# ffreyer/MonteCarlo.jl

Measured on AMD Instinct MI355X. Metric: DQMC sweeps/sec, 16x16 Hubbard beta=8 dtau=0.1; achieved % fp64 MFMA roofline, higher is better.
Workload: dtype f64

## Files before the change

### include/dqmc_hip.h

```cpp
#ifndef DQMC_HIP_H
#define DQMC_HIP_H
#include <stddef.h>
#include <stdint.h>

#ifdef __cplusplus
extern "C" {
#endif

typedef struct dqmc_handle dqmc_handle;

typedef enum {
    DQMC_OK = 0,
    DQMC_ERR_INVALID = -1,
    DQMC_ERR_HIP = -2,
    DQMC_ERR_NO_DEVICE = -3,
    DQMC_ERR_STATE = -4,
    DQMC_ERR_RNG = -5
} dqmc_status;

enum { DQMC_ATTRACTIVE = 0, DQMC_REPULSIVE = 1 };

typedef struct {
    int32_t n_sites;
    int32_t model_kind;
    int32_t slices;
    int32_t safe_mult;
    int32_t n_walkers;
    int32_t device_id;
    int32_t check_propagation_error;
    int32_t check_sign_problem;
    double delta_tau;
    double U;
    const double *eT;
    const double *eTinv;
    const double *eT2;
    const double *eTinv2;
} dqmc_params;

typedef struct {
    double max, min, sum;
    int64_t count;
} dqmc_magstats;

typedef struct {
    int64_t prop_local, acc_local;
    dqmc_magstats imaginary_probability;
    dqmc_magstats negative_probability;
    dqmc_magstats propagation_error;
} dqmc_stats;

int dqmc_create(const dqmc_params *p, dqmc_handle **out);
int dqmc_destroy(dqmc_handle *h);
const char *dqmc_last_error(const dqmc_handle *h);
int dqmc_device_count(void);

int dqmc_set_conf(dqmc_handle *h, int32_t walker, const int8_t *conf);
int dqmc_get_conf(dqmc_handle *h, int32_t walker, int8_t *conf);
int dqmc_get_conf_bits(dqmc_handle *h, int32_t walker, uint64_t *chunks);
int dqmc_set_conf_bits(dqmc_handle *h, int32_t walker, const uint64_t *chunks);
int dqmc_set_uniforms(dqmc_handle *h, int32_t walker, const double *u, size_t n);
int dqmc_seed(dqmc_handle *h, int32_t walker, uint64_t seed);
int dqmc_uniforms_used(dqmc_handle *h, int32_t walker, uint64_t *used);
int dqmc_get_state(dqmc_handle *h, int32_t *current_slice, int32_t *direction);

int dqmc_prepare(dqmc_handle *h);
int dqmc_build_stack(dqmc_handle *h);
int dqmc_propagate(dqmc_handle *h);
int dqmc_sweep_spatial(dqmc_handle *h);
int dqmc_update(dqmc_handle *h);
int dqmc_sweep(dqmc_handle *h, int32_t n_sweeps);
int dqmc_update_until_measure(dqmc_handle *h, int32_t *n_updates);
int dqmc_synchronize(dqmc_handle *h);

int dqmc_get_greens_eff(dqmc_handle *h, int32_t walker, double *out);
int dqmc_set_greens_eff(dqmc_handle *h, int32_t walker, const double *in);
int dqmc_get_greens(dqmc_handle *h, int32_t walker, double *out);
int dqmc_calculate_greens_at(dqmc_handle *h, int32_t walker, int32_t slice, double *out);
int dqmc_replay_greens(dqmc_handle *h, int32_t slice);
int dqmc_wrap_greens(dqmc_handle *h, int32_t slice, int32_t direction);

int dqmc_get_stats(dqmc_handle *h, int32_t walker, dqmc_stats *out);

int dqmc_accumulate_greens(dqmc_handle *h);
int dqmc_accumulator_size(dqmc_handle *h, size_t *n_doubles);
int dqmc_reset_accumulators(dqmc_handle *h);
int dqmc_get_accumulators(dqmc_handle *h, double *host_out);
int dqmc_export_accumulators(dqmc_handle *h, void *device_out);

int dqmc_set_pair_directions(dqmc_handle *h, const int32_t *dir_of, int32_t n_dirs);
int dqmc_accumulate_correlations(dqmc_handle *h);
int dqmc_correlations_size(dqmc_handle *h, size_t *n_doubles);
int dqmc_get_correlations(dqmc_handle *h, double *host_out);
int dqmc_export_correlations(dqmc_handle *h, void *device_out);

int dqmc_set_local_targets(dqmc_handle *h, const int32_t *trg_of, int32_t K);
int dqmc_accumulate_pairing(dqmc_handle *h);
int dqmc_pairing_size(dqmc_handle *h, size_t *n_doubles);
int dqmc_get_pairing(dqmc_handle *h, double *host_out);
int dqmc_export_pairing(dqmc_handle *h, void *device_out);

int dqmc_ut_build_stack(dqmc_handle *h);
int dqmc_ut_get_stack(dqmc_handle *h, int32_t w, int32_t which, int32_t idx, double *U, double *D, double *T);
int dqmc_ut_greens(dqmc_handle *h, int32_t slice1, int32_t slice2, int32_t effective);
int dqmc_ut_get(dqmc_handle *h, int32_t w, int32_t which, double *host_out);
int dqmc_ut_export(dqmc_handle *h, int32_t which, void *device_out );
int dqmc_greens_iterator_begin(dqmc_handle *h, int32_t l, int32_t recalculate);
int dqmc_greens_iterator_next(dqmc_handle *h, int32_t *k);
int dqmc_combined_iterator_begin(dqmc_handle *h, int32_t recalculate);
int dqmc_combined_iterator_next(dqmc_handle *h, int32_t *l);

int dqmc_accumulate_susceptibilities(dqmc_handle *h, int32_t recalculate);
int dqmc_susceptibilities_size(dqmc_handle *h, size_t *n_doubles);
int dqmc_get_susceptibilities(dqmc_handle *h, double *host_out);
int dqmc_export_susceptibilities(dqmc_handle *h, void *device_out);

int dqmc_set_current_targets(dqmc_handle *h, const int32_t *trg_of, int32_t K, const double *T);
int dqmc_current_targets_fast_path(dqmc_handle *h, int32_t *fast);

enum { DQMC_BIN_GREENS = 0, DQMC_BIN_CORRELATIONS = 1, DQMC_BIN_PAIRING = 2, DQMC_BIN_SUSCEPTIBILITIES = 3,
       DQMC_BIN_USER = 4 };
int dqmc_binner_enable(dqmc_handle *h, int32_t which, int64_t capacity);
int dqmc_binner_size(dqmc_handle *h, int32_t which, size_t *n_elements, int32_t *n_levels, int64_t *n_pushed);
int dqmc_binner_reliable_level(dqmc_handle *h, int32_t which, int32_t *level);
int dqmc_binner_get_level(dqmc_handle *h, int32_t which, int32_t walker, int32_t level,
                          double *x_sum, double *x2_sum, int64_t *count);
int dqmc_binner_finish(dqmc_handle *h, int32_t which, int32_t level,
                       double *mean, double *std_error, double *std_error_walkers, double *tau);
int dqmc_binner_export_moments(dqmc_handle *h, int32_t which, int32_t level, void *device_out);
int dqmc_binner_user_create(dqmc_handle *h, int64_t n_elements, int64_t capacity);
int dqmc_binner_user_push(dqmc_handle *h, const double *device_samples);

typedef struct dqmc_comm dqmc_comm;
int dqmc_comm_unique_id(void *id128);
int dqmc_comm_init(const void *id128, int32_t nranks, int32_t rank, int32_t device_id, dqmc_comm **out);
int dqmc_comm_destroy(dqmc_comm *c);
int dqmc_reduce(dqmc_handle *h, dqmc_comm *comm);
int dqmc_reduce_size(dqmc_handle *h, size_t *n_doubles );
int dqmc_reduce_export(dqmc_handle *h, double *host_out);
int dqmc_reduce_import(dqmc_handle *h, const double *host_in);
enum { DQMC_RED_GREENS = 0, DQMC_RED_CORRELATIONS = 1, DQMC_RED_PAIRING = 2, DQMC_RED_SUSCEPTIBILITIES = 3 };
int dqmc_get_reduced(dqmc_handle *h, int32_t which, double *host_out);
int dqmc_get_reduced_stats(dqmc_handle *h, dqmc_stats *out);

int dqmc_vmul(int32_t device_id, int32_t n, int32_t batch, int32_t transa, int32_t transb,
              const double *A, const double *B, double *C);
int dqmc_udt_pivot(int32_t device_id, int32_t n, int32_t batch, double *U, double *D, double *T,
                   int64_t *pivot, int32_t apply_pivot);
int dqmc_rdivp(int32_t device_id, int32_t n, int32_t batch, double *A, const double *T,
               const int64_t *pivot);
int dqmc_calculate_greens(int32_t device_id, int32_t n, int32_t batch, const double *Ul,
                          const double *Dl, const double *Tl, const double *Ur, const double *Dr,
                          const double *Tr, double *G);

int dqmc_set_checkerboard(dqmc_handle *h, int32_t kmax, int32_t n_mats, const double *vals, const int32_t *cols,
                          const double *mu, const double *mu_inv, const int32_t *seqs, const int32_t *lens);

int dqmc_qr_fallbacks(dqmc_handle *h, int64_t *count);
int dqmc_kron_hopping(dqmc_handle *h, int32_t *on);
int dqmc_set_triangular_factors(dqmc_handle *h, const double *f);
int dqmc_udt_one_launch_sites(dqmc_handle *h, int32_t *mask);
int dqmc_device_errors(dqmc_handle *h, int32_t *word);
const char *dqmc_build_commit(void);
const char *dqmc_build_source_hash(void);

typedef struct dqmc_mc_handle dqmc_mc_handle;

typedef struct {
    int32_t n_sites;
    int32_t z;
    int32_t n_walkers;
    int32_t device_id;
    int32_t n_bonds;
    int32_t series_capacity;
    const int64_t *neighs;
    const int64_t *bonds;
} dqmc_mc_params;

typedef struct {
    int64_t energy;
    int64_t magnetization;
    double sum_E, sum_E2, sum_absM, sum_M2;
    int64_t n_meas;
    int64_t prop_local, acc_local;
    uint64_t uniforms_used;
    int64_t n_series;
} dqmc_mc_stats;

int dqmc_mc_create(const dqmc_mc_params *p, dqmc_mc_handle **out);
int dqmc_mc_destroy(dqmc_mc_handle *h);
const char *dqmc_mc_last_error(const dqmc_mc_handle *h);
int dqmc_mc_set_beta(dqmc_mc_handle *h, int32_t walker, double beta);
int dqmc_mc_seed(dqmc_mc_handle *h, int32_t walker, uint64_t seed);
int dqmc_mc_rand_conf(dqmc_mc_handle *h, int32_t walker);
int dqmc_mc_set_conf(dqmc_mc_handle *h, int32_t walker, const int8_t *conf);
int dqmc_mc_get_conf(dqmc_mc_handle *h, int32_t walker, int8_t *conf);
int dqmc_mc_get_conf_bits(dqmc_mc_handle *h, int32_t walker, uint64_t *chunks);
int dqmc_mc_sweep(dqmc_mc_handle *h, int32_t n_sweeps, int64_t first_sweep_index, int64_t thermalization,
                  int32_t measure_rate);
int dqmc_mc_get_stats(dqmc_mc_handle *h, int32_t walker, dqmc_mc_stats *out);
int dqmc_mc_get_series(dqmc_mc_handle *h, int32_t walker, int32_t *energy, int32_t *abs_magnetization,
                       int64_t *n_recorded);
int dqmc_mc_reset_accumulators(dqmc_mc_handle *h);
int dqmc_mc_set_global_rate(dqmc_mc_handle *h, int32_t rate);
int dqmc_mc_global_move(dqmc_mc_handle *h, int32_t walker);
typedef struct {
    int64_t prop_global, acc_global, sum_cluster_size;
    uint64_t moves_drawn;
} dqmc_mc_global_stats;
int dqmc_mc_get_global_stats(dqmc_mc_handle *h, int32_t walker, dqmc_mc_global_stats *out);
int dqmc_mc_synchronize(dqmc_mc_handle *h);

int dqmc_mc_binner_enable(dqmc_mc_handle *h, int64_t capacity);
int dqmc_mc_binner_size(dqmc_mc_handle *h, int32_t *n_levels, int64_t *n_pushed);
int dqmc_mc_binner_reliable_level(dqmc_mc_handle *h, int32_t *level);
int dqmc_mc_binner_get_level(dqmc_mc_handle *h, int32_t walker, int32_t level,
                             double x_sum[4], double x2_sum[4], double xy_sum[2], int64_t *count);
typedef struct {
    double mean[4];
    double varN[4];
    double varN0[4];
    double tau[4];
    double covN[2];
    int64_t count;
    int32_t level;
} dqmc_mc_binned;
int dqmc_mc_binner_finish(dqmc_mc_handle *h, int32_t walker, int32_t level, dqmc_mc_binned *out);

enum { DQMC_K_GEMM = 0, DQMC_K_QR = 1, DQMC_K_TRSM = 2, DQMC_K_SWEEP = 3, DQMC_K_MISC = 4, DQMC_K_FLUSH = 5,
       DQMC_K_COUNT = 6 };
int dqmc_timing_enable(dqmc_handle *h, int32_t on);
int dqmc_timing_get(dqmc_handle *h, double *ms , int64_t *launches );
int dqmc_mfma_f64_peak(int32_t device_id, int32_t iters, double *tflops);

#ifdef __cplusplus
}
#endif
#endif
```

### montecarlo.jl_amd/_lib.py

```python
import ctypes as C
import os

_HERE = os.path.dirname(os.path.abspath(__file__))
LIB_PATH = os.environ.get("DQMC_HIP_LIB") or os.path.join(_HERE, "libdqmc_hip.so")
HEADER_PATH = os.path.join(os.path.dirname(_HERE), "include", "dqmc_hip.h")

OK, ERR_INVALID, ERR_HIP, ERR_NO_DEVICE, ERR_STATE, ERR_RNG = 0, -1, -2, -3, -4, -5
ATTRACTIVE, REPULSIVE = 0, 1
BIN_SECTIONS = ("greens", "correlations", "pairing", "susceptibilities", "user")
K_FAMILIES = ("gemm", "qr", "trsm", "sweep", "misc", "flush")


class DQMCError(RuntimeError):
    def __init__(self, code, msg):
        super().__init__("libdqmc_hip error %d: %s" % (code, msg))
        self.code = code


class Params(C.Structure):
    _fields_ = [
        ("n_sites", C.c_int32), ("model_kind", C.c_int32), ("slices", C.c_int32), ("safe_mult", C.c_int32),
        ("n_walkers", C.c_int32), ("device_id", C.c_int32), ("check_propagation_error", C.c_int32),
        ("check_sign_problem", C.c_int32), ("delta_tau", C.c_double), ("U", C.c_double),
        ("eT", C.POINTER(C.c_double)), ("eTinv", C.POINTER(C.c_double)), ("eT2", C.POINTER(C.c_double)),
        ("eTinv2", C.POINTER(C.c_double)),
    ]


class MagStats(C.Structure):
    _fields_ = [("max", C.c_double), ("min", C.c_double), ("sum", C.c_double), ("count", C.c_int64)]


class Stats(C.Structure):
    _fields_ = [("prop_local", C.c_int64), ("acc_local", C.c_int64), ("imaginary_probability", MagStats),
                ("negative_probability", MagStats), ("propagation_error", MagStats)]


class McParams(C.Structure):
    _fields_ = [("n_sites", C.c_int32), ("z", C.c_int32), ("n_walkers", C.c_int32), ("device_id", C.c_int32),
                ("n_bonds", C.c_int32), ("series_capacity", C.c_int32), ("neighs", C.POINTER(C.c_int64)),
                ("bonds", C.POINTER(C.c_int64))]


class McStats(C.Structure):
    _fields_ = [("energy", C.c_int64), ("magnetization", C.c_int64), ("sum_E", C.c_double), ("sum_E2", C.c_double),
                ("sum_absM", C.c_double), ("sum_M2", C.c_double), ("n_meas", C.c_int64), ("prop_local", C.c_int64),
                ("acc_local", C.c_int64), ("uniforms_used", C.c_uint64), ("n_series", C.c_int64)]


class McGlobalStats(C.Structure):
    _fields_ = [("prop_global", C.c_int64), ("acc_global", C.c_int64), ("sum_cluster_size", C.c_int64),
                ("moves_drawn", C.c_uint64)]


class McBinned(C.Structure):
    _fields_ = [("mean", C.c_double * 4), ("varN", C.c_double * 4), ("varN0", C.c_double * 4), ("tau", C.c_double * 4),
                ("covN", C.c_double * 2), ("count", C.c_int64), ("level", C.c_int32)]


_dp = C.POINTER(C.c_double)
_i64p = C.POINTER(C.c_int64)
_H = C.c_void_p

SIGNATURES = {
    "dqmc_create": (C.c_int, [C.POINTER(Params), C.POINTER(_H)]),
    "dqmc_destroy": (C.c_int, [_H]),
    "dqmc_last_error": (C.c_char_p, [_H]),
    "dqmc_device_count": (C.c_int, []),
    "dqmc_set_conf": (C.c_int, [_H, C.c_int32, C.c_void_p]),
    "dqmc_get_conf": (C.c_int, [_H, C.c_int32, C.c_void_p]),
    "dqmc_get_conf_bits": (C.c_int, [_H, C.c_int32, C.POINTER(C.c_uint64)]),
    "dqmc_set_conf_bits": (C.c_int, [_H, C.c_int32, C.POINTER(C.c_uint64)]),
    "dqmc_set_uniforms": (C.c_int, [_H, C.c_int32, _dp, C.c_size_t]),
    "dqmc_seed": (C.c_int, [_H, C.c_int32, C.c_uint64]),
    "dqmc_uniforms_used": (C.c_int, [_H, C.c_int32, C.POINTER(C.c_uint64)]),
    "dqmc_get_state": (C.c_int, [_H, C.POINTER(C.c_int32), C.POINTER(C.c_int32)]),
    "dqmc_prepare": (C.c_int, [_H]),
    "dqmc_build_stack": (C.c_int, [_H]),
    "dqmc_propagate": (C.c_int, [_H]),
    "dqmc_sweep_spatial": (C.c_int, [_H]),
    "dqmc_update": (C.c_int, [_H]),
    "dqmc_sweep": (C.c_int, [_H, C.c_int32]),
    "dqmc_update_until_measure": (C.c_int, [_H, C.POINTER(C.c_int32)]),
    "dqmc_synchronize": (C.c_int, [_H]),
    "dqmc_get_greens_eff": (C.c_int, [_H, C.c_int32, _dp]),
    "dqmc_set_greens_eff": (C.c_int, [_H, C.c_int32, _dp]),
    "dqmc_get_greens": (C.c_int, [_H, C.c_int32, _dp]),
    "dqmc_calculate_greens_at": (C.c_int, [_H, C.c_int32, C.c_int32, _dp]),
    "dqmc_replay_greens": (C.c_int, [_H, C.c_int32]),
    "dqmc_wrap_greens": (C.c_int, [_H, C.c_int32, C.c_int32]),
    "dqmc_get_stats": (C.c_int, [_H, C.c_int32, C.POINTER(Stats)]),
    "dqmc_accumulate_greens": (C.c_int, [_H]),
    "dqmc_accumulator_size": (C.c_int, [_H, C.POINTER(C.c_size_t)]),
    "dqmc_reset_accumulators": (C.c_int, [_H]),
    "dqmc_get_accumulators": (C.c_int, [_H, _dp]),
    "dqmc_export_accumulators": (C.c_int, [_H, C.c_void_p]),
    "dqmc_set_pair_directions": (C.c_int, [_H, C.POINTER(C.c_int32), C.c_int32]),
    "dqmc_accumulate_correlations": (C.c_int, [_H]),
    "dqmc_correlations_size": (C.c_int, [_H, C.POINTER(C.c_size_t)]),
    "dqmc_get_correlations": (C.c_int, [_H, _dp]),
    "dqmc_export_correlations": (C.c_int, [_H, C.c_void_p]),
    "dqmc_set_local_targets": (C.c_int, [_H, C.POINTER(C.c_int32), C.c_int32]),
    "dqmc_accumulate_pairing": (C.c_int, [_H]),
    "dqmc_pairing_size": (C.c_int, [_H, C.POINTER(C.c_size_t)]),
    "dqmc_get_pairing": (C.c_int, [_H, _dp]),
    "dqmc_export_pairing": (C.c_int, [_H, C.c_void_p]),
    "dqmc_ut_build_stack": (C.c_int, [_H]),
    "dqmc_ut_get_stack": (C.c_int, [_H, C.c_int32, C.c_int32, C.c_int32, _dp, _dp, _dp]),
    "dqmc_ut_greens": (C.c_int, [_H, C.c_int32, C.c_int32, C.c_int32]),
    "dqmc_ut_get": (C.c_int, [_H, C.c_int32, C.c_int32, _dp]),
    "dqmc_ut_export": (C.c_int, [_H, C.c_int32, C.c_void_p]),
    "dqmc_greens_iterator_begin": (C.c_int, [_H, C.c_int32, C.c_int32]),
    "dqmc_greens_iterator_next": (C.c_int, [_H, C.POINTER(C.c_int32)]),
    "dqmc_combined_iterator_begin": (C.c_int, [_H, C.c_int32]),
    "dqmc_combined_iterator_next": (C.c_int, [_H, C.POINTER(C.c_int32)]),
    "dqmc_accumulate_susceptibilities": (C.c_int, [_H, C.c_int32]),
    "dqmc_set_current_targets": (C.c_int, [_H, C.POINTER(C.c_int32), C.c_int32, C.POINTER(C.c_double)]),
    "dqmc_current_targets_fast_path": (C.c_int, [_H, C.POINTER(C.c_int32)]),
    "dqmc_susceptibilities_size": (C.c_int, [_H, C.POINTER(C.c_size_t)]),
    "dqmc_get_susceptibilities": (C.c_int, [_H, _dp]),
    "dqmc_export_susceptibilities": (C.c_int, [_H, C.c_void_p]),
    "dqmc_binner_enable": (C.c_int, [_H, C.c_int32, C.c_int64]),
    "dqmc_binner_size": (C.c_int, [_H, C.c_int32, C.POINTER(C.c_size_t), C.POINTER(C.c_int32), _i64p]),
    "dqmc_binner_reliable_level": (C.c_int, [_H, C.c_int32, C.POINTER(C.c_int32)]),
    "dqmc_binner_get_level": (C.c_int, [_H, C.c_int32, C.c_int32, C.c_int32, _dp, _dp, _i64p]),
    "dqmc_binner_finish": (C.c_int, [_H, C.c_int32, C.c_int32, _dp, _dp, _dp, _dp]),
    "dqmc_binner_export_moments": (C.c_int, [_H, C.c_int32, C.c_int32, C.c_void_p]),
    "dqmc_binner_user_create": (C.c_int, [_H, C.c_int64, C.c_int64]),
    "dqmc_binner_user_push": (C.c_int, [_H, C.c_void_p]),
    "dqmc_comm_unique_id": (C.c_int, [C.c_void_p]),
    "dqmc_comm_init": (C.c_int, [C.c_void_p, C.c_int32, C.c_int32, C.c_int32, C.POINTER(_H)]),
    "dqmc_comm_destroy": (C.c_int, [_H]),
    "dqmc_reduce": (C.c_int, [_H, _H]),
    "dqmc_reduce_size": (C.c_int, [_H, C.POINTER(C.c_size_t)]),
    "dqmc_reduce_export": (C.c_int, [_H, _dp]),
    "dqmc_reduce_import": (C.c_int, [_H, _dp]),
    "dqmc_get_reduced": (C.c_int, [_H, C.c_int32, _dp]),
    "dqmc_get_reduced_stats": (C.c_int, [_H, C.POINTER(Stats)]),
    "dqmc_vmul": (C.c_int, [C.c_int32, C.c_int32, C.c_int32, C.c_int32, C.c_int32, _dp, _dp, _dp]),
    "dqmc_udt_pivot": (C.c_int, [C.c_int32, C.c_int32, C.c_int32, _dp, _dp, _dp, _i64p, C.c_int32]),
    "dqmc_rdivp": (C.c_int, [C.c_int32, C.c_int32, C.c_int32, _dp, _dp, _i64p]),
    "dqmc_calculate_greens": (C.c_int, [C.c_int32, C.c_int32, C.c_int32, _dp, _dp, _dp, _dp, _dp, _dp, _dp]),
    "dqmc_set_checkerboard": (C.c_int, [_H, C.c_int32, C.c_int32, _dp, C.POINTER(C.c_int32), _dp, _dp,
                              C.POINTER(C.c_int32), C.POINTER(C.c_int32)]),
    "dqmc_qr_fallbacks": (C.c_int, [_H, C.POINTER(C.c_int64)]),
    "dqmc_kron_hopping": (C.c_int, [_H, C.POINTER(C.c_int32)]),
    "dqmc_set_triangular_factors": (C.c_int, [_H, _dp]),
    "dqmc_device_errors": (C.c_int, [_H, C.POINTER(C.c_int32)]),
    "dqmc_udt_one_launch_sites": (C.c_int, [_H, C.POINTER(C.c_int32)]),
    "dqmc_build_commit": (C.c_char_p, []),
    "dqmc_build_source_hash": (C.c_char_p, []),
    "dqmc_mc_create": (C.c_int, [C.POINTER(McParams), C.POINTER(_H)]),
    "dqmc_mc_destroy": (C.c_int, [_H]),
    "dqmc_mc_last_error": (C.c_char_p, [_H]),
    "dqmc_mc_set_beta": (C.c_int, [_H, C.c_int32, C.c_double]),
    "dqmc_mc_seed": (C.c_int, [_H, C.c_int32, C.c_uint64]),
    "dqmc_mc_rand_conf": (C.c_int, [_H, C.c_int32]),
    "dqmc_mc_set_conf": (C.c_int, [_H, C.c_int32, C.c_void_p]),
    "dqmc_mc_get_conf": (C.c_int, [_H, C.c_int32, C.c_void_p]),
    "dqmc_mc_get_conf_bits": (C.c_int, [_H, C.c_int32, C.POINTER(C.c_uint64)]),
    "dqmc_mc_sweep": (C.c_int, [_H, C.c_int32, C.c_int64, C.c_int64, C.c_int32]),
    "dqmc_mc_get_stats": (C.c_int, [_H, C.c_int32, C.POINTER(McStats)]),
    "dqmc_mc_get_series": (C.c_int, [_H, C.c_int32, C.POINTER(C.c_int32), C.POINTER(C.c_int32),
                           C.POINTER(C.c_int64)]),
    "dqmc_mc_reset_accumulators": (C.c_int, [_H]),
    "dqmc_mc_set_global_rate": (C.c_int, [_H, C.c_int32]),
    "dqmc_mc_global_move": (C.c_int, [_H, C.c_int32]),
    "dqmc_mc_get_global_stats": (C.c_int, [_H, C.c_int32, C.POINTER(McGlobalStats)]),
    "dqmc_mc_synchronize": (C.c_int, [_H]),
    "dqmc_mc_binner_enable": (C.c_int, [_H, C.c_int64]),
    "dqmc_mc_binner_size": (C.c_int, [_H, C.POINTER(C.c_int32), _i64p]),
    "dqmc_mc_binner_reliable_level": (C.c_int, [_H, C.POINTER(C.c_int32)]),
    "dqmc_mc_binner_get_level": (C.c_int, [_H, C.c_int32, C.c_int32, _dp, _dp, _dp, _i64p]),
    "dqmc_mc_binner_finish": (C.c_int, [_H, C.c_int32, C.c_int32, C.POINTER(McBinned)]),
    "dqmc_timing_enable": (C.c_int, [_H, C.c_int32]),
    "dqmc_timing_get": (C.c_int, [_H, _dp, _i64p]),
    "dqmc_mfma_f64_peak": (C.c_int, [C.c_int32, C.c_int32, _dp]),
}

_lib = None


def lib():
    global _lib
    if _lib is None:
        if not os.path.exists(LIB_PATH):
            raise ImportError(
                "libdqmc_hip.so not found at %s — build it with __graft_entry__.build() "
                "(hipcc --offload-arch=gfx950); there is no CPU fallback." % LIB_PATH)
        L = C.CDLL(LIB_PATH)
        for name, (res, args) in SIGNATURES.items():
            f = getattr(L, name)
            f.restype = res
            f.argtypes = args
        _lib = L
    return _lib


def check(rc, handle=None):
    if rc != 0:
        msg = lib().dqmc_last_error(handle)
        raise DQMCError(rc, msg.decode() if msg else "")


def dptr(a):
    return a.ctypes.data_as(_dp)


def i64ptr(a):
    return a.ctypes.data_as(_i64p)
```

### montecarlo.jl_amd/csrc/engine.cpp

```cpp
#include <hip/hip_runtime.h>

#include <algorithm>
#include <cmath>
#include <cstdio>
#include <cstdlib>
#include <cstring>
#include <string>
#include <vector>

#include "../../include/dqmc_hip.h"
#include "kernels.h"
#include <rccl/rccl.h>

using namespace dqmc;

struct dqmc_comm {
    ncclComm_t comm = nullptr;
    int nranks = 1, rank = 0, device = 0;
};

static thread_local std::string g_create_error;

struct UTStack;

struct dqmc_handle {
    dqmc_params p{};
    int n = 0, nb = 1, N = 0, M = 0, s = 0, K = 0, W = 0, units = 0;
    long nn = 0;
    double lambda = 0, epl = 0, eml = 0;
    SweepConsts sc{};
    hipStream_t stream = nullptr;
    KernelSwitches sw;
    double *eT = nullptr, *eTinv = nullptr, *eT2 = nullptr, *eTinv2 = nullptr;
    double *eT2T = nullptr;
    bool slab = false;
    bool kron = false, tri = false;
    double *kron_f = nullptr;
    int kron_fa = 0, kron_fb = 0;
    int8_t *conf = nullptr;
    double *u_stack = nullptr, *t_stack = nullptr, *d_stack = nullptr;
    std::vector<double *> su, sd, st;
    double *Ul = nullptr, *Ur = nullptr, *Tl = nullptr, *Tr = nullptr, *greens = nullptr, *greens_temp = nullptr;
    double *tmp1 = nullptr, *tmp2 = nullptr, *bufA = nullptr, *bufB = nullptr;
    struct QrSet {
        double *V = nullptr, *W = nullptr, *S = nullptr, *tau = nullptr, *winv = nullptr, *ts = nullptr;
        int *pivot = nullptr;
    } qs[1];
    double *&qrV = qs[0].V, *&qrW = qs[0].W, *&qrS = qs[0].S, *&trsm_w = qs[0].winv, *&trsm_s = qs[0].ts, *&tau = qs[0].tau;
    int *&pivot = qs[0].pivot;
    double *Dl = nullptr, *Dr = nullptr;
    hipStream_t cur = nullptr;
    double *greens_alt = nullptr, *lu_img = nullptr;
    bool sweep_fused = true;
    struct PendingFlush {
        const double *G = nullptr;
        const double *img = nullptr;
        int site0 = 0;
    } pf;
    unsigned *wrap_cnt = nullptr;
    unsigned wrap_launches = 0;
    int wrap_blocks[2] = {0, 0};
    WalkerRng *rng = nullptr;
    DevStats *stats = nullptr;
    unsigned long long *pc_scratch = nullptr;
    std::vector<double *> uniforms;
    double *acc = nullptr;
    size_t acc_n = 0;
    int n_dirs = 0;
    int *dir_ptr = nullptr, *pair_src = nullptr, *pair_trg = nullptr;
    double *corr_per_walker = nullptr, *corr_acc = nullptr;
    int K_loc = 0;
    int *trg_of = nullptr;
    size_t pc_n = 0;
    double *pc_per_walker = nullptr, *pc_acc = nullptr;
    int K_cc = 0;
    std::vector<int> cc_trg_h;
    std::vector<double> cc_T;
    CCPlan cc;
    size_t corr_n = 0;
    int current_slice = 0, direction = 0;
    bool prepared = false;
    long long conf_version = 0;
    UTStack *ut = nullptr;
    std::string err;
    bool timing = false;
    struct Ev { hipEvent_t a, b; int fam; };
    std::vector<Ev> pending;
    std::vector<hipEvent_t> pool;
    double fam_ms[DQMC_K_COUNT] = {0};
    long long fam_n[DQMC_K_COUNT] = {0};
    std::vector<void *> allocs;
    QrCoopWorkspace qr_ws;
    int qrb_sites = 0;
    struct {
        bool on = false;
        int kmax = 0, n_mats = 0;
        double *vals = nullptr, *mu = nullptr, *mu_inv = nullptr;
        int *cols = nullptr;
        int seq[7][32];
        int len[7] = {0, 0, 0, 0, 0, 0, 0};
    } cb;
    double *red_buf = nullptr;
    size_t red_cap = 0;
    dqmc_stats red_stats{};
    bool red_valid = false;
    size_t red_sizes[4] = {0, 0, 0, 0};
    struct Binner {
        bool on = false;
        int E = 0, L = 0;
        int64_t cap = 0, T = 0;
        double *xs = nullptr, *x2 = nullptr, *c = nullptr, *out = nullptr;
    } bin[5];
};

#define HIPCHK(expr)                                                                                   \
    do {                                                                                               \
        hipError_t e_ = (expr);                                                                        \
        if (e_ != hipSuccess) {                                                                        \
            h->err = std::string(#expr) + ": " + hipGetErrorString(e_);                                \
            return DQMC_ERR_HIP;                                                                       \
        }                                                                                              \
    } while (0)
#define CHK(expr)                \
    do {                         \
        int rc_ = (expr);        \
        if (rc_ != 0) return rc_; \
    } while (0)

static int fail(dqmc_handle *h, int code, const std::string &msg)
{
    if (h) h->err = msg;
    else g_create_error = msg;
    return code;
}

template <typename T>
static int dalloc(dqmc_handle *h, T **p, size_t count, bool zero = true)
{
    void *q = nullptr;
    HIPCHK(hipMalloc(&q, (count ? count : 1) * sizeof(T)));
    h->allocs.push_back(q);
    if (zero) HIPCHK(hipMemsetAsync(q, 0, (count ? count : 1) * sizeof(T), h->stream));
    *p = (T *)q;
    return 0;
}

static int timing_drain(dqmc_handle *h)
{
    if (h->pending.empty()) return 0;
    HIPCHK(hipStreamSynchronize(h->stream));
    for (auto &e : h->pending) {
        float ms = 0.f;
        HIPCHK(hipEventElapsedTime(&ms, e.a, e.b));
        h->fam_ms[e.fam] += ms;
        h->fam_n[e.fam] += 1;
        h->pool.push_back(e.a);
        h->pool.push_back(e.b);
    }
    h->pending.clear();
    return 0;
}
struct Timed {
    dqmc_handle *h;
    int fam;
    hipEvent_t a = nullptr, b = nullptr;
    Timed(dqmc_handle *h_, int fam_) : h(h_), fam(fam_)
    {
        if (!h->timing) return;
        auto get = [&]() {
            hipEvent_t e;
            if (!h->pool.empty()) { e = h->pool.back(); h->pool.pop_back(); }
            else (void)hipEventCreate(&e);
            return e;
        };
        a = get();
        b = get();
        (void)hipEventRecord(a, h->cur);
    }
    ~Timed()
    {
        if (!h->timing) return;
        (void)hipEventRecord(b, h->cur);
        h->pending.push_back({a, b, fam});
        if (h->pending.size() >= 2048) (void)timing_drain(h);
    }
};

static GemmArgs gemm_base(dqmc_handle *h, MatRef A, int tA, MatRef B, int tB, double *C)
{
    GemmArgs g{};
    g.M = g.N = g.K = h->n;
    g.n_units = h->units;
    g.nb = h->nb;
    g.A = A;
    g.B = B;
    g.C = C;
    g.strideC = h->nn;
    g.ldc = h->n;
    g.transA = tA;
    g.transB = tB;
    g.kscale = g.colscale = g.rowscale = g.adddiag = vs_none();
    g.row_first = 0;
    g.alpha = 1.0;
    g.ident = 0.0;
    g.beta = 0;
    g.tri = 0;
// ... 616 lines not shown
        g.rowscale = vs_conf(h, l, -1);
        CHK(run_gemm(h, g));
        g = gemm_base(h, U_(h, h->tmp1), 0, C_(h, h->eT2), 0, gf);
        g.colscale = vs_conf(h, l, +1);
        CHK(run_gemm(h, g));
    } else {
        const int l = curr_slice;
        GemmArgs g = gemm_base(h, C_(h, h->eT2), 0, U_(h, gf), 0, h->tmp1);
        g.kscale = vs_conf(h, l, +1);
        CHK(run_gemm(h, g));
        g = gemm_base(h, U_(h, h->tmp1), 0, C_(h, h->eTinv2), 0, gf);
        g.kscale = vs_conf(h, l, -1);
        CHK(run_gemm(h, g));
    }
    return 0;
}

static int reset_slot(dqmc_handle *h, int slot)
{
    const int sp = h->K + 1;
    CHK(set_identity(h, uslot(h, sp)));
    CHK(set_ones(h, dslot(h, sp)));
    CHK(set_identity(h, tslot(h, sp)));
    slot_swap_spare(h, slot);
    return 0;
}
static int prop_check(dqmc_handle *h)
{
    Timed t(h, DQMC_K_MISC);
    HIPCHK(launch_prop_check(h->n, h->nb, h->W, h->greens_temp, h->greens, h->nn, h->stats, h->pc_scratch, h->cur));
    return 0;
}

static int init_stack(dqmc_handle *h)
{
    CHK(set_identity(h, h->Ul)); CHK(set_identity(h, h->Ur));
    CHK(set_identity(h, h->Tl)); CHK(set_identity(h, h->Tr));
    CHK(set_ones(h, h->Dl)); CHK(set_ones(h, h->Dr));
    h->current_slice = 0;
    h->direction = 0;
    return 0;
}
static int build_stack(dqmc_handle *h)
{
    CHK(reset_slot(h, 0));
    for (int i = 1; i <= h->K; ++i) CHK(add_slice_sequence_left(h, i));
    h->current_slice = h->M + 1;
    h->direction = -1;
    return 0;
}

static int propagate(dqmc_handle *h)
{
    const int M = h->M, s = h->s;
    if (h->direction == 1) {
        if (h->current_slice % s == 0) {
            h->current_slice += 1;
            if (h->current_slice == 1) {
                const Udt R = slot_ref(h, 0);
                CHK(reset_slot(h, 0));
                discard_pending_flush(h);
                CHK(calculate_greens_src(h, h->greens, slot_ref(h, 0), R));
            } else if (1 < h->current_slice && h->current_slice <= M) {
                const int idx = (h->current_slice - 1) / s;
                const Udt R = slot_ref(h, idx);
                const bool wt = h->p.check_propagation_error != 0, wt_slab = wt && oop_wrap(h);
                CHK(add_slice_sequence_left(h, idx, wt_slab));
                const Udt L = slot_ref(h, idx);
                if (wt && !wt_slab) {
                    CHK(materialize_pending_flush(h));
                    CHK(copy_mat(h, h->greens_temp, h->greens));
                    CHK(wrap_greens(h, &h->greens_temp, h->current_slice - 1, 1));
                }
                if (wt_slab) {
                    std::swap(h->greens, h->greens_alt);
                    CHK(calculate_greens_src(h, h->greens, L, R));
                    CHK(prop_check(h));
                    return 0;
                }
                discard_pending_flush(h);
                CHK(calculate_greens_src(h, h->greens, L, R));
                if (h->p.check_propagation_error) CHK(prop_check(h));
            } else {
                CHK(add_slice_sequence_left(h, h->K));
                h->direction = -1;
                h->current_slice = M + 1;
                CHK(propagate(h));
            }
        } else {
            CHK(wrap_greens(h, &h->greens, h->current_slice, 1));
            h->current_slice += 1;
        }
    } else {
        if ((h->current_slice - 1) % s == 0) {
            h->current_slice -= 1;
            if (h->current_slice == M) {
                const Udt L = slot_ref(h, h->K);
                CHK(reset_slot(h, h->K));
                discard_pending_flush(h);
                CHK(calculate_greens_src(h, h->greens, L, slot_ref(h, h->K)));
                CHK(wrap_greens(h, &h->greens, h->current_slice + 1, -1));
            } else if (0 < h->current_slice && h->current_slice < M) {
                const int idx = h->current_slice / s + 1;
                const Udt L = slot_ref(h, idx - 1);
                CHK(add_slice_sequence_right(h, idx));
                const Udt R = slot_ref(h, idx - 1);
                if (h->p.check_propagation_error) {
                    CHK(materialize_pending_flush(h));
                    std::swap(h->greens_temp, h->greens);
                }
                discard_pending_flush(h);
                CHK(calculate_greens_src(h, h->greens, L, R));
                if (h->p.check_propagation_error) CHK(prop_check(h));
                CHK(wrap_greens(h, &h->greens, h->current_slice + 1, -1));
            } else {
                CHK(add_slice_sequence_right(h, 1));
                h->direction = 1;
                h->current_slice = 0;
                CHK(propagate(h));
            }
        } else {
            CHK(wrap_greens(h, &h->greens, h->current_slice, -1));
            h->current_slice -= 1;
        }
    }
    return 0;
}

static int sweep_spatial_launches(dqmc_handle *h);
static int sweep_spatial(dqmc_handle *h)
{
    const int l = h->current_slice;
    if (l < 1 || l > h->M) return fail(h, DQMC_ERR_STATE, "sweep_spatial: current_slice outside 1..slices");
    CHK(sweep_spatial_launches(h));
    return 0;
}
static int sweep_spatial_launches(dqmc_handle *h)
{
    const int l = h->current_slice;
    int8_t *cslice = h->conf + (long)(l - 1) * h->N;
    h->conf_version++;
    CHK(materialize_pending_flush(h));
    double *cur = h->greens, *alt = h->greens_alt;
    const size_t istr = (size_t)h->units * sweep_lu_image_doubles();

    const long cstr = (long)h->N * h->M;
    hipEvent_t a, b;
    if (h->sweep_fused && h->n % 64 == 0 && h->N >= 128) {
        const int nc = h->N / 64;
        timing_events(h, &a, &b);
        HIPCHK(launch_sweep_lu(h->n, h->nb, h->W, cur, h->nn, cslice, cstr, 0, 64, h->lu_img, h->sc, h->rng, h->stats,
                               h->p.check_sign_problem, h->qr_ws.errflag, h->cur, a, b));
        CHK(timing_push(h, a, b, DQMC_K_SWEEP));
        for (int c = 1; c < nc; ++c) {
            timing_events(h, &a, &b);
            HIPCHK(launch_sweep_fused(h->n, h->nb, h->W, cur, alt, h->nn, cslice, cstr, 64 * c, 64 * (c - 1),
                                      h->lu_img + (size_t)(c & 1) * istr, h->lu_img + (size_t)((c - 1) & 1) * istr, h->sc,
                                      h->rng, h->stats, h->p.check_sign_problem, h->qr_ws.errflag, h->cur, a, b));
            CHK(timing_push(h, a, b, DQMC_K_SWEEP));
            std::swap(cur, alt);
        }
        const double *img_last = h->lu_img + (size_t)((nc - 1) & 1) * istr;
        if (fold_wrap_flush(h)) {
            h->pf = dqmc_handle::PendingFlush{cur, img_last, 64 * (nc - 1)};
        } else {
            timing_events(h, &a, &b);
            HIPCHK(launch_sweep_flush_lu(h->n, h->units, cur, alt, h->nn, 64 * (nc - 1), 64, img_last, h->sw, h->cur, a, b));
            CHK(timing_push(h, a, b, DQMC_K_FLUSH));
            std::swap(cur, alt);
        }
        if (cur != h->greens) std::swap(h->greens, h->greens_alt);
        return 0;
    }
    for (int site0 = 0; site0 < h->N; site0 += 64) {
        const int ns = std::min(64, h->N - site0);
        timing_events(h, &a, &b);
        HIPCHK(launch_sweep_lu(h->n, h->nb, h->W, cur, h->nn, cslice, cstr, site0, ns, h->lu_img, h->sc,
                               h->rng, h->stats, h->p.check_sign_problem, h->qr_ws.errflag, h->cur, a, b));
        CHK(timing_push(h, a, b, DQMC_K_SWEEP));
        timing_events(h, &a, &b);
        HIPCHK(launch_sweep_flush_lu(h->n, h->units, cur, alt, h->nn, site0, ns, h->lu_img, h->sw, h->cur, a, b));
        CHK(timing_push(h, a, b, DQMC_K_FLUSH));
        std::swap(cur, alt);
    }
    if (cur != h->greens) std::swap(h->greens, h->greens_alt);
    return 0;
}

extern "C" {

const char *dqmc_last_error(const dqmc_handle *h) { return h ? h->err.c_str() : g_create_error.c_str(); }

int dqmc_device_count(void)
{
    int c = 0;
    if (hipGetDeviceCount(&c) != hipSuccess) return 0;
    return c;
}

int dqmc_create(const dqmc_params *p, dqmc_handle **out)
{
    if (!p || !out) return fail(nullptr, DQMC_ERR_INVALID, "dqmc_create: null argument");
    *out = nullptr;
    if (p->n_sites < 1 || p->slices < 1 || p->safe_mult < 1 || p->n_walkers < 1)
        return fail(nullptr, DQMC_ERR_INVALID, "dqmc_create: n_sites, slices, safe_mult, n_walkers must be >= 1");
    if (p->slices % p->safe_mult != 0)
        return fail(nullptr, DQMC_ERR_INVALID, "dqmc_create: slices must be divisible by safe_mult");
    if (p->model_kind != DQMC_ATTRACTIVE && p->model_kind != DQMC_REPULSIVE)
        return fail(nullptr, DQMC_ERR_INVALID, "dqmc_create: unknown model_kind");
    if (!p->eT || !p->eTinv || !p->eT2 || !p->eTinv2)
        return fail(nullptr, DQMC_ERR_INVALID, "dqmc_create: hopping exponentials missing");
    if (!(p->U >= 0.0)) return fail(nullptr, DQMC_ERR_INVALID, "dqmc_create: U must be positive");
    const int nb = p->model_kind == DQMC_REPULSIVE ? 2 : 1;
    if (p->n_sites > 1024) return fail(nullptr, DQMC_ERR_INVALID, "dqmc_create: n_sites exceeds 1024 (unsupported)");
    int ndev = 0;
    if (hipGetDeviceCount(&ndev) != hipSuccess || ndev == 0)
        return fail(nullptr, DQMC_ERR_NO_DEVICE, "dqmc_create: no HIP device visible");
    if (p->device_id < 0 || p->device_id >= ndev)
        return fail(nullptr, DQMC_ERR_INVALID, "dqmc_create: device_id out of range");

    dqmc_handle *h = new dqmc_handle();
    read_kernel_switches(h);
    h->p = *p;
    h->p.eT = h->p.eTinv = h->p.eT2 = h->p.eTinv2 = nullptr;
    h->N = h->n = p->n_sites;
    h->nb = nb;
    h->M = p->slices;
    h->s = p->safe_mult;
    h->K = h->M / h->s;
    h->W = p->n_walkers;
    h->units = h->W * h->nb;
    h->nn = (long)h->n * h->n;
    h->sweep_fused = false;
    if (!h->sw.sweep_split && h->n % 64 == 0) {
        hipDeviceProp_t prop;
        if (hipGetDeviceProperties(&prop, p->device_id) == hipSuccess) {
            const int ncp = (h->n % 256 == 0) ? 2 : 1, nt = (h->n % 128 == 0) ? 8 : 4;
            const int flush_blocks = ((h->units + 7) / 8) * 8 * (h->n / 64) * (h->n / (16 * nt * ncp));
            h->sweep_fused = h->W + flush_blocks <= prop.multiProcessorCount;
        }
    }
    h->lambda = std::acosh(std::exp(0.5 * p->U * p->delta_tau));
    h->epl = std::exp(h->lambda);
    h->eml = std::exp(-h->lambda);
    for (int ci = 0; ci < 2; ++ci) {
        const double c = ci ? 1.0 : -1.0;
        const double dE = -2.0 * h->lambda * c;
        h->sc.gamma[ci] = std::exp(dE) - 1.0;
        h->sc.ebos[ci] = std::exp(-dE);
        h->sc.dup[ci] = std::exp(dE) - 1.0;
        h->sc.ddn[ci] = std::exp(-dE) - 1.0;
    }
    auto bail = [&](int rc) {
        g_create_error = h->err;
        dqmc_destroy(h);
        return rc;
    };
#define CCHK(expr)                     \
    do {                               \
        int rc__ = (expr);             \
        if (rc__ != 0) return bail(rc__); \
    } while (0)
#define CHIP(expr)                                                        \
    do {                                                                  \
        hipError_t e__ = (expr);                                          \
        if (e__ != hipSuccess) {                                          \
            h->err = std::string(#expr) + ": " + hipGetErrorString(e__);  \
            return bail(DQMC_ERR_HIP);                                    \
        }                                                                 \
    } while (0)
    CHIP(hipSetDevice(p->device_id));
    CHIP(hipStreamCreate(&h->stream));
    h->cur = h->stream;
    const size_t cn = (size_t)nb * h->nn, un = (size_t)h->units * h->nn, uv = (size_t)h->units * h->n;
    CCHK(dalloc(h, &h->eT, cn)); CCHK(dalloc(h, &h->eTinv, cn));
    CCHK(dalloc(h, &h->eT2, cn)); CCHK(dalloc(h, &h->eTinv2, cn));
    CHIP(hipMemcpy(h->eT, p->eT, cn * sizeof(double), hipMemcpyHostToDevice));
    CHIP(hipMemcpy(h->eTinv, p->eTinv, cn * sizeof(double), hipMemcpyHostToDevice));
    CHIP(hipMemcpy(h->eT2, p->eT2, cn * sizeof(double), hipMemcpyHostToDevice));
    CHIP(hipMemcpy(h->eTinv2, p->eTinv2, cn * sizeof(double), hipMemcpyHostToDevice));
    if (h->n == 256 && !h->sw.no_slab) {
        std::vector<double> tr(cn);
        for (int b = 0; b < nb; ++b)
            for (int j = 0; j < h->n; ++j)
                for (int i = 0; i < h->n; ++i) tr[(size_t)b * h->nn + j + (size_t)h->n * i] = p->eT2[(size_t)b * h->nn + i + (size_t)h->n * j];
        CCHK(dalloc(h, &h->eT2T, cn));
        CHIP(hipMemcpy(h->eT2T, tr.data(), cn * sizeof(double), hipMemcpyHostToDevice));
        h->slab = true;
    }
    if (h->slab && !h->sw.no_kron) {
        std::vector<double> f((size_t)4 * 2 * nb * 256);
        bool ok = true;
        for (int m = 0; m < 2 && ok; ++m)
            for (int b = 0; b < nb && ok; ++b) {
                double *fx = f.data() + ((size_t)m * 2 * nb + b) * 256, *fy = fx + (size_t)nb * 256;
                double *tx = f.data() + ((size_t)(m + 2) * 2 * nb + b) * 256, *ty = tx + (size_t)nb * 256;
                ok = kron_factor((m ? p->eTinv2 : p->eT2) + (size_t)b * h->nn, fx, fy);
                for (int j = 0; j < 16; ++j)
                    for (int i = 0; i < 16; ++i) {
                        tx[i + 16 * j] = fx[j + 16 * i];
                        ty[i + 16 * j] = fy[j + 16 * i];
                    }
            }
        if (ok) {
            CCHK(dalloc(h, &h->kron_f, f.size()));
            CHIP(hipMemcpy(h->kron_f, f.data(), f.size() * sizeof(double), hipMemcpyHostToDevice));
            h->kron = true;
            h->kron_fa = h->kron_fb = 256;
        }
    }
    if (h->n == 512 && !h->sw.no_kron) {
        const size_t per = (size_t)nb * (4096 + 256);
        std::vector<double> f(4 * per);
        double fx[64], fy[64], fz[64];
        bool ok = true;
        for (int m = 0; m < 2 && ok; ++m)
// ... 648 lines not shown
int dqmc_comm_destroy(dqmc_comm *c)
{
    if (!c) return DQMC_OK;
    if (c->comm) (void)ncclCommDestroy(c->comm);
    delete c;
    return DQMC_OK;
}
int dqmc_reduce_size(dqmc_handle *h, size_t *n_doubles)
{
    if (!h || !n_doubles) return DQMC_ERR_INVALID;
    *n_doubles = red_nsum(h) + 4;
    return DQMC_OK;
}
int dqmc_reduce(dqmc_handle *h, dqmc_comm *comm)
{
    ENTER(h);
    CHK(red_pack(h));
    if (comm && comm->comm) {
        if (comm->device != h->p.device_id) return fail(h, DQMC_ERR_INVALID, "dqmc_reduce: communicator bound to another device");
        const size_t nsum = red_nsum(h);
        ncclResult_t r = ncclGroupStart();
        if (r == ncclSuccess) r = ncclAllReduce(h->red_buf, h->red_buf, nsum, ncclDouble, ncclSum, comm->comm, h->stream);
        if (r == ncclSuccess) r = ncclAllReduce(h->red_buf + nsum, h->red_buf + nsum, 2, ncclDouble, ncclMax, comm->comm, h->stream);
        if (r == ncclSuccess) r = ncclAllReduce(h->red_buf + nsum + 2, h->red_buf + nsum + 2, 2, ncclDouble, ncclMin, comm->comm, h->stream);
        const ncclResult_t r2 = ncclGroupEnd();
        if (r != ncclSuccess || r2 != ncclSuccess)
            return fail(h, DQMC_ERR_HIP, std::string("ncclAllReduce: ") + ncclGetErrorString(r != ncclSuccess ? r : r2));
    }
    CHK(red_unpack(h));
    return DQMC_OK;
}
int dqmc_reduce_export(dqmc_handle *h, double *host_out)
{
    ENTER(h);
    CHK(red_pack(h));
    HIPCHK(hipMemcpy(host_out, h->red_buf, (red_nsum(h) + 4) * sizeof(double), hipMemcpyDeviceToHost));
    return DQMC_OK;
}
int dqmc_reduce_import(dqmc_handle *h, const double *host_in)
{
    ENTER(h);
    if (h->red_cap < red_nsum(h) + 4) return fail(h, DQMC_ERR_STATE, "call dqmc_reduce_export first");
    HIPCHK(hipStreamSynchronize(h->stream));
    HIPCHK(hipMemcpy(h->red_buf, host_in, (red_nsum(h) + 4) * sizeof(double), hipMemcpyHostToDevice));
    CHK(red_unpack(h));
    return DQMC_OK;
}
int dqmc_get_reduced(dqmc_handle *h, int32_t which, double *host_out)
{
    ENTER(h);
    if (!host_out || which < 0 || which > 3) return fail(h, DQMC_ERR_INVALID, "dqmc_get_reduced: bad arguments");
    if (!h->red_valid) return fail(h, DQMC_ERR_STATE, "call dqmc_reduce first");
    const size_t sizes[4] = {h->acc_n, h->corr_n, h->pc_n, h->ut ? h->ut->sus_n : 0};
    size_t off = 0;
    for (int i = 0; i < which; ++i) off += sizes[i];
    if (sizes[which] == 0) return fail(h, DQMC_ERR_STATE, "dqmc_get_reduced: this accumulator is not configured");
    for (int i = 0; i < 4; ++i)
        if (sizes[i] != h->red_sizes[i])
            return fail(h, DQMC_ERR_STATE, "accumulators were reconfigured after the last reduction: call dqmc_reduce again");
    if (h->red_cap < red_nsum(h) + 4) return fail(h, DQMC_ERR_STATE, "call dqmc_reduce first");
    HIPCHK(hipStreamSynchronize(h->stream));
    HIPCHK(hipMemcpy(host_out, h->red_buf + off, sizes[which] * sizeof(double), hipMemcpyDeviceToHost));
    return DQMC_OK;
}
int dqmc_get_reduced_stats(dqmc_handle *h, dqmc_stats *out)
{
    if (!h || !out) return DQMC_ERR_INVALID;
    if (!h->red_valid) return fail(h, DQMC_ERR_STATE, "call dqmc_reduce first");
    *out = h->red_stats;
    return DQMC_OK;
}


int dqmc_set_triangular_factors(dqmc_handle *h, const double *f)
{
    ENTER(h);
    if (!f) return fail(h, DQMC_ERR_INVALID, "dqmc_set_triangular_factors: null factors");
    if (h->n != 256) return fail(h, DQMC_ERR_INVALID, "dqmc_set_triangular_factors: n_sites must be 256");
    if (h->prepared) return fail(h, DQMC_ERR_STATE, "dqmc_set_triangular_factors: call before dqmc_prepare");
    if (!h->slab || h->cb.on || h->sw.no_kron || h->kron) return DQMC_OK;
    const int nb = h->nb;
    std::vector<double> E((size_t)2 * nb * h->nn);
    HIPCHK(hipStreamSynchronize(h->stream));
    HIPCHK(hipMemcpy(E.data(), h->eT2, sizeof(double) * nb * h->nn, hipMemcpyDeviceToHost));
    HIPCHK(hipMemcpy(E.data() + (size_t)nb * h->nn, h->eTinv2, sizeof(double) * nb * h->nn, hipMemcpyDeviceToHost));
    std::vector<double> img((size_t)4 * 3 * nb * 256);
    for (int b = 0; b < nb; ++b)
        for (int m = 0; m < 2; ++m) {
            const double *fb = f + (size_t)b * 1536 + (size_t)m * 768;
            if (!tri_factor_ok(E.data() + ((size_t)m * nb + b) * h->nn, fb, fb + 256, fb + 512))
                return fail(h, DQMC_ERR_INVALID, "dqmc_set_triangular_factors: the factors do not reproduce eT2 / eTinv2 of block " +
                                                     std::to_string(b) + " within 256 ulp");
            for (int k = 0; k < 3; ++k) {
                double *o = img.data() + (((size_t)m * 3 + k) * nb + b) * 256, *ot = o + (size_t)2 * 3 * nb * 256;
                for (int j = 0; j < 16; ++j)
                    for (int i = 0; i < 16; ++i) {
                        o[i + 16 * j] = fb[256 * k + i + 16 * j];
                        ot[i + 16 * j] = fb[256 * k + j + 16 * i];
                    }
            }
        }
    CHK(dalloc(h, &h->kron_f, img.size()));
    HIPCHK(hipMemcpy(h->kron_f, img.data(), img.size() * sizeof(double), hipMemcpyHostToDevice));
    h->kron_fa = 256;
    h->kron_fb = 512;
    h->tri = h->kron = true;
    return DQMC_OK;
}

int dqmc_set_checkerboard(dqmc_handle *h, int32_t kmax, int32_t n_mats, const double *vals, const int32_t *cols,
                          const double *mu, const double *mu_inv, const int32_t *seqs ,
                          const int32_t *lens )
{
    ENTER(h);
    if (kmax < 1 || kmax > 64 || n_mats < 1 || !vals || !cols || !mu || !mu_inv || !seqs || !lens)
        return fail(h, DQMC_ERR_INVALID, "dqmc_set_checkerboard: bad arguments");
    const size_t cnt = (size_t)n_mats * h->n * kmax;
    for (size_t i = 0; i < cnt; ++i)
        if (cols[i] < 0 || cols[i] >= h->n) return fail(h, DQMC_ERR_INVALID, "dqmc_set_checkerboard: column index out of range");
    for (int q = 0; q < 7; ++q) {
        if (lens[q] < 0 || lens[q] > 32) return fail(h, DQMC_ERR_INVALID, "dqmc_set_checkerboard: sequence too long");
        for (int i = 0; i < lens[q]; ++i)
            if (seqs[q * 32 + i] < 0 || seqs[q * 32 + i] >= n_mats)
                return fail(h, DQMC_ERR_INVALID, "dqmc_set_checkerboard: factor index out of range");
    }
    HIPCHK(hipStreamSynchronize(h->stream));
    CHK(dalloc(h, &h->cb.vals, cnt));
    CHK(dalloc(h, &h->cb.cols, cnt));
    CHK(dalloc(h, &h->cb.mu, (size_t)h->nb * h->n));
    CHK(dalloc(h, &h->cb.mu_inv, (size_t)h->nb * h->n));
    HIPCHK(hipMemcpy(h->cb.vals, vals, cnt * sizeof(double), hipMemcpyHostToDevice));
    HIPCHK(hipMemcpy(h->cb.cols, cols, cnt * sizeof(int), hipMemcpyHostToDevice));
    HIPCHK(hipMemcpy(h->cb.mu, mu, (size_t)h->nb * h->n * sizeof(double), hipMemcpyHostToDevice));
    HIPCHK(hipMemcpy(h->cb.mu_inv, mu_inv, (size_t)h->nb * h->n * sizeof(double), hipMemcpyHostToDevice));
    h->cb.kmax = kmax; h->cb.n_mats = n_mats;
    for (int q = 0; q < 7; ++q) {
        h->cb.len[q] = lens[q];
        for (int i = 0; i < lens[q]; ++i) h->cb.seq[q][i] = seqs[q * 32 + i];
    }
    h->cb.on = true;
    return DQMC_OK;
}

int dqmc_device_errors(dqmc_handle *h, int32_t *word)
{
    ENTER(h);
    if (!word) return DQMC_ERR_INVALID;
    *word = 0;
    if (!h->qr_ws.errflag) return DQMC_OK;
    HIPCHK(hipStreamSynchronize(h->stream));
    HIPCHK(hipMemcpy(word, h->qr_ws.errflag, sizeof(int), hipMemcpyDeviceToHost));
    return DQMC_OK;
}
int dqmc_udt_one_launch_sites(dqmc_handle *h, int32_t *mask)
{
    if (!h || !mask) return DQMC_ERR_INVALID;
    *mask = h->qrb_sites;
    return DQMC_OK;
}

int dqmc_kron_hopping(dqmc_handle *h, int32_t *on)
{
    ENTER(h);
    if (!on) return DQMC_ERR_INVALID;
    *on = use_kron(h) ? 1 : 0;
    return DQMC_OK;
}

int dqmc_qr_fallbacks(dqmc_handle *h, int64_t *count)
{
    ENTER(h);
    if (!count) return DQMC_ERR_INVALID;
    *count = 0;
    if (!h->qr_ws.fb) return DQMC_OK;
    int fb[2] = {0, 0};
    HIPCHK(hipStreamSynchronize(h->stream));
    HIPCHK(hipMemcpy(fb, h->qr_ws.fb, sizeof(fb), hipMemcpyDeviceToHost));
    *count = fb[1];
    return DQMC_OK;
}

int dqmc_timing_enable(dqmc_handle *h, int32_t on)
{
    ENTER(h);
    CHK(timing_drain(h));
    h->timing = on != 0;
    for (int i = 0; i < DQMC_K_COUNT; ++i) { h->fam_ms[i] = 0; h->fam_n[i] = 0; }
    return DQMC_OK;
}
int dqmc_timing_get(dqmc_handle *h, double *ms, int64_t *launches)
{
    ENTER(h);
    CHK(timing_drain(h));
    for (int i = 0; i < DQMC_K_COUNT; ++i) {
        if (ms) ms[i] = h->fam_ms[i];
        if (launches) launches[i] = h->fam_n[i];
    }
    return DQMC_OK;
}

namespace {
struct Scratch {
    dqmc_handle h;
    int ok = 0;
};
static int scratch_init(dqmc_handle *h, int device_id, int n, int batch)
{
    int ndev = 0;
    if (hipGetDeviceCount(&ndev) != hipSuccess || ndev == 0) return fail(nullptr, DQMC_ERR_NO_DEVICE, "no HIP device visible");
    if (device_id < 0 || device_id >= ndev) return fail(nullptr, DQMC_ERR_INVALID, "device_id out of range");
    if (n < 1 || n > 1024 || batch < 1) return fail(nullptr, DQMC_ERR_INVALID, "n must be 1..1024 and batch >= 1");
    read_kernel_switches(h);
    h->p.device_id = device_id;
    h->n = h->N = n;
    h->nb = 1;
    h->W = h->units = batch;
    h->nn = (long)n * n;
    HIPCHK(hipSetDevice(device_id));
    HIPCHK(hipStreamCreate(&h->stream));
    h->cur = h->stream;
    return 0;
}
static void scratch_free(dqmc_handle *h)
{
    if (h->stream) (void)hipStreamSynchronize(h->stream);
    for (void *q : h->allocs) (void)hipFree(q);
    h->allocs.clear();
    if (h->stream) (void)hipStreamDestroy(h->stream);
    h->stream = nullptr;
}
}

#define SCHK(expr)                                   \
    do {                                             \
        int rc_ = (expr);                            \
        if (rc_ != 0) {                              \
            g_create_error = h->err.empty() ? g_create_error : h->err; \
            scratch_free(h);                         \
            return rc_;                              \
        }                                            \
    } while (0)
#define SHIP(expr)                                                       \
    do {                                                                 \
        hipError_t e_ = (expr);                                          \
        if (e_ != hipSuccess) {                                          \
            g_create_error = std::string(#expr) + ": " + hipGetErrorString(e_); \
            scratch_free(h);                                             \
            return DQMC_ERR_HIP;                                         \
        }                                                                \
    } while (0)

int dqmc_vmul(int32_t device_id, int32_t n, int32_t batch, int32_t ta, int32_t tb, const double *A, const double *B,
              double *C)
{
    dqmc_handle hh; dqmc_handle *h = &hh;
    SCHK(scratch_init(h, device_id, n, batch));
    const size_t un = (size_t)batch * h->nn;
    double *dA, *dB, *dC;
    SCHK(dalloc(h, &dA, un, false)); SCHK(dalloc(h, &dB, un, false)); SCHK(dalloc(h, &dC, un));
    SHIP(hipMemcpy(dA, A, un * sizeof(double), hipMemcpyHostToDevice));
    SHIP(hipMemcpy(dB, B, un * sizeof(double), hipMemcpyHostToDevice));
    SCHK(run_gemm(h, gemm_base(h, U_(h, dA), ta != 0, U_(h, dB), tb != 0, dC)));
    SHIP(hipStreamSynchronize(h->stream));
    SHIP(hipMemcpy(C, dC, un * sizeof(double), hipMemcpyDeviceToHost));
    scratch_free(h);
    return DQMC_OK;
}

static int scratch_udt_bufs(dqmc_handle *h)
{
    const size_t un = (size_t)h->units * h->nn, uv = (size_t)h->units * h->n;
    CHK(dalloc(h, &h->qrV, un)); CHK(dalloc(h, &h->qrW, un)); CHK(dalloc(h, &h->qrS, un));
    CHK(dalloc(h, &h->tau, uv)); CHK(dalloc(h, &h->pivot, uv));
    CHK(dalloc(h, &h->trsm_w, (size_t)h->units * ((h->n + 15) / 16) * 256));
    CHK(alloc_qr_workspace(h));
    return 0;
}

int dqmc_udt_pivot(int32_t device_id, int32_t n, int32_t batch, double *U, double *D, double *T, int64_t *pivot,
                   int32_t apply)
{
    dqmc_handle hh; dqmc_handle *h = &hh;
    SCHK(scratch_init(h, device_id, n, batch));
    const size_t un = (size_t)batch * h->nn, uv = (size_t)batch * n;
    double *dU, *dD, *dT, *dTo;
    SCHK(dalloc(h, &dU, un)); SCHK(dalloc(h, &dD, uv)); SCHK(dalloc(h, &dT, un, false)); SCHK(dalloc(h, &dTo, un));
    SCHK(scratch_udt_bufs(h));
    SHIP(hipMemcpy(dT, T, un * sizeof(double), hipMemcpyHostToDevice));
    SCHK(udt(h, dT, dU, dD, dTo, apply != 0));
    SHIP(hipStreamSynchronize(h->stream));
    SCHK(check_qr_workspace(h));
    SHIP(hipMemcpy(U, dU, un * sizeof(double), hipMemcpyDeviceToHost));
    SHIP(hipMemcpy(D, dD, uv * sizeof(double), hipMemcpyDeviceToHost));
    SHIP(hipMemcpy(T, (apply || udt_is_fused(h, 0)) ? dTo : dT, un * sizeof(double), hipMemcpyDeviceToHost));
    std::vector<int> piv(uv);
    SHIP(hipMemcpy(piv.data(), h->pivot, uv * sizeof(int), hipMemcpyDeviceToHost));
    for (size_t i = 0; i < uv; ++i) pivot[i] = (int64_t)piv[i] + 1;
    scratch_free(h);
    return DQMC_OK;
}

int dqmc_rdivp(int32_t device_id, int32_t n, int32_t batch, double *A, const double *T, const int64_t *pivot)
{
    dqmc_handle hh; dqmc_handle *h = &hh;
    SCHK(scratch_init(h, device_id, n, batch));
    const size_t un = (size_t)batch * h->nn, uv = (size_t)batch * n;
// ... 70 lines not shown
```

### montecarlo.jl_amd/csrc/kernels.h

```cpp
#pragma once
#include <hip/hip_runtime.h>
#include <stdint.h>

namespace dqmc {

struct VecSrc {
    int mode;
    const double *d;
    long stride;
    const int8_t *conf;
    long conf_stride;
    double cpos[2], cneg[2];
};
static inline VecSrc vs_none() { VecSrc v = {}; v.mode = 0; return v; }
static inline VecSrc vs_arr(const double *d, long stride) { VecSrc v = {}; v.mode = 1; v.d = d; v.stride = stride; return v; }
static inline VecSrc vs_inv(const double *d, long stride) { VecSrc v = {}; v.mode = 3; v.d = d; v.stride = stride; return v; }
static inline VecSrc vs_min1(const double *d, long stride) { VecSrc v = {}; v.mode = 4; v.d = d; v.stride = stride; return v; }
static inline VecSrc vs_maxinv(const double *d, long stride) { VecSrc v = {}; v.mode = 5; v.d = d; v.stride = stride; return v; }
#ifdef __HIPCC__
__device__ __forceinline__ double vs_get(const VecSrc &v, int unit, int nb, int i)
{
    if (v.mode == 1) return v.d[(long)unit * v.stride + i];
    if (v.mode == 3) return 1.0 / v.d[(long)unit * v.stride + i];
    if (v.mode == 2) {
// ... 44 lines not shown
    long conf_stride;
    double epl, eml;
};
hipError_t launch_slab_chain(const SlabArgs &a, hipStream_t s, hipEvent_t start = nullptr, hipEvent_t stop = nullptr);
struct KronStep {
    const double *ax, *ay;
    const int8_t *pre_conf; int pre_sign;
    const int8_t *post_conf; int post_sign;
};
struct KronArgs {
    int n_units, nb, nsteps;
    KronStep st[SLAB_MAX_STEPS];
    const double *X0; long x_su;
    double *out; long out_su;
    const double *col_d; long col_stride;
    int transpose_out;
    long conf_stride;
    double epl, eml;
    const double *pf_img; long pf_img_su;
    int pf_site0;
    double *wrap_out;
    unsigned *wrap_cnt; unsigned wrap_target;
    int *errflag;
};
hipError_t launch_kron_chain(const KronArgs &a, hipStream_t s, hipEvent_t start = nullptr, hipEvent_t stop = nullptr);
constexpr int KR_CNT_STRIDE = 32;
inline int kron_wrap_grid(int n_units) { return (n_units + 7) / 8 * 8 * 16; }
int kron_wrap_blocks_per_cu(bool pending);
hipError_t launch_kron_wrap(const KronArgs &a, hipStream_t s, hipEvent_t start = nullptr, hipEvent_t stop = nullptr);
hipError_t launch_kron3_chain(const KronArgs &a, hipStream_t s, hipEvent_t start = nullptr, hipEvent_t stop = nullptr);
hipError_t launch_tri_chain(const KronArgs &a, hipStream_t s, hipEvent_t start = nullptr, hipEvent_t stop = nullptr);

struct KernelSwitches {
    bool qr_noblocked = false;
    int qrb_sites = 7;
    bool qr_tail = true;
    bool qr_sc1 = false;
    bool qr_nocoop = false;
    int qr_force_timeout = 0;
    bool qr_nopanel = false;
    bool trsm_simple = false;
    bool sweep_split = false;
    bool flush_ncp2 = false;
    bool no_slab = false;
    bool no_kron = false;
    bool no_wrap_flush = false;
    bool wrap_two_launch = false;
};

constexpr int QR_COOP_SLOT = 528;
constexpr int QR_COOP_SLOTS_PER_UNIT = 16;
struct QrCoopWorkspace {
    double *mailbox = nullptr;
    int *errflag = nullptr;
    int *fb = nullptr;
    unsigned long long epoch = 0;
    int max_blocks = 0;
    bool tail = true;
    int force_sc1 = 0;
    int no_coop = 0;
    bool no_panel = false;
    int force_timeout = 0;
    double *mailbox2 = nullptr;
    int blk_max_blocks = 0;
};
hipError_t launch_udt_blocked(int n_units, const double *A, long strideA, double *U, long strideU, double *D, long strideD,
                              double *T, long strideT, int *pivot, QrCoopWorkspace *ws, int apply_pivot, hipStream_t s,
                              const double *B = nullptr, long strideB = 0);
size_t qrb_mailbox_bytes(int n_units);
int qrb_blocks_per_cu();
hipError_t launch_qr_pivot(int n, int n_units, double *A, long strideA, double *tau, int *pivot,
                           QrCoopWorkspace *ws, double *W, long strideW, const double **factored, hipStream_t s,
                           double *X = nullptr, long strideX = 0);
int qr_coop_blocks_per_cu();

hipError_t launch_udt_finish(int n, int n_units, double *A, long strideA, const double *F, long strideF,
                             const int *pivot, double *D, long strideD, double *V, long strideV, double *Tout,
                             long strideT, int apply_pivot, hipStream_t s);

hipError_t launch_trsm_right_upper(int n, int n_units, const double *A, long strideA, const double *T,
                                   long strideT, const int *pivot, const double *dmul, long strideV,
                                   double *Out, long strideOut, double *winv, const KernelSwitches &sw,
                                   hipStream_t s, double *scratch = nullptr);

struct SweepConsts {
    double gamma[2], ebos[2], dup[2], ddn[2];
};
struct WalkerRng {
    unsigned long long seed;
    unsigned long long draw;
    const double *uniforms;
    unsigned long long n_uniforms;
    int exhausted;
};
struct DevMagStats { double max, min, sum; long long count; };
struct DevStats {
    long long prop_local, acc_local;
    DevMagStats negative_probability, propagation_error;
};
#ifdef __HIPCC__
__device__ __forceinline__ double philox_uniform(unsigned long long seed, unsigned long long index)
{
    unsigned int c0 = (unsigned int)index, c1 = (unsigned int)(index >> 32), c2 = 0u, c3 = 0u;
    unsigned int k0 = (unsigned int)seed, k1 = (unsigned int)(seed >> 32);
#pragma unroll
    for (int r = 0; r < 10; ++r) {
        const unsigned long long p0 = (unsigned long long)0xD2511F53u * c0;
        const unsigned long long p1 = (unsigned long long)0xCD9E8D57u * c2;
        const unsigned int n0 = (unsigned int)(p1 >> 32) ^ c1 ^ k0;
        const unsigned int n1 = (unsigned int)p1;
        const unsigned int n2 = (unsigned int)(p0 >> 32) ^ c3 ^ k1;
        const unsigned int n3 = (unsigned int)p0;
        c0 = n0; c1 = n1; c2 = n2; c3 = n3;
        k0 += 0x9E3779B9u;
        k1 += 0xBB67AE85u;
    }
    const unsigned long long hi = c0 >> 5, lo = c1 >> 6;
    return (double)((hi << 26) | lo) * (1.0 / 9007199254740992.0);
}

__device__ __forceinline__ double philox4_uniform(unsigned long long seed, unsigned int c0, unsigned int c1,
                                                  unsigned int c2, unsigned int c3)
{
    unsigned int k0 = (unsigned int)seed, k1 = (unsigned int)(seed >> 32);
#pragma unroll
    for (int r = 0; r < 10; ++r) {
        const unsigned long long p0 = (unsigned long long)0xD2511F53u * c0;
        const unsigned long long p1 = (unsigned long long)0xCD9E8D57u * c2;
        const unsigned int n0 = (unsigned int)(p1 >> 32) ^ c1 ^ k0;
        const unsigned int n1 = (unsigned int)p1;
        const unsigned int n2 = (unsigned int)(p0 >> 32) ^ c3 ^ k1;
        const unsigned int n3 = (unsigned int)p0;
        c0 = n0; c1 = n1; c2 = n2; c3 = n3;
        k0 += 0x9E3779B9u;
        k1 += 0xBB67AE85u;
    }
    const unsigned long long hi = c0 >> 5, lo = c1 >> 6;
    return (double)((hi << 26) | lo) * (1.0 / 9007199254740992.0);
}

__device__ __forceinline__ void magstats_push(DevMagStats &s, double value)
{
    const double v = log10(fabs(value));
    s.max = fmax(s.max, v);
    s.min = fmin(s.min, v);
    s.sum += v;
    s.count += 1;
}
#endif
size_t sweep_lu_image_doubles();
constexpr int LU_TILE = 256;
constexpr int LU_OFF_U = 0, LU_OFF_L = 6 * LU_TILE, LU_OFF_PT = 12 * LU_TILE, LU_OFF_Q = 16 * LU_TILE;
constexpr int LU_IMG = 20 * LU_TILE;
constexpr int LU_STRIDE = LU_IMG + 64;
__host__ __device__ constexpr int lu_pair(int K, int J)
{
    return K == 0 ? J - 1 : (K == 1 ? J + 1 : 5);
}
hipError_t launch_sweep_lu(int n, int nb, int n_walkers, const double *G, long strideG, int8_t *conf_slice,
                           long conf_stride, int site0, int nsites, double *img, SweepConsts sc, WalkerRng *rng,
                           DevStats *stats, int check_sign, int *errflag, hipStream_t s,
                           hipEvent_t start = nullptr, hipEvent_t stop = nullptr);
hipError_t launch_sweep_fused(int n, int nb, int n_walkers, const double *Gin, double *Gout, long strideG,
                              int8_t *conf_slice, long conf_stride, int site0, int site0p, double *img,
                              const double *imgp, SweepConsts sc, WalkerRng *rng, DevStats *stats, int check_sign,
                              int *errflag, hipStream_t s, hipEvent_t start = nullptr, hipEvent_t stop = nullptr);

hipError_t launch_sweep_flush_lu(int n, int n_units, const double *Gin, double *Gout, long strideG, int site0,
                                 int nsites, const double *img, const KernelSwitches &sw, hipStream_t s,
                                 hipEvent_t start = nullptr, hipEvent_t stop = nullptr);

struct CbArgs {
    int n, nb, side, kmax, seq_len;
    int seq[32];
    const double *vals;
    const int *cols;
    const double *X;
    double *O;
    long strideX;
    const int8_t *conf;
    long conf_stride;
    double epl, eml;
    int pre_conf, post_conf;
    const double *pre_vec, *post_vec;
    const double *qscale;
    long qstride;
};
hipError_t launch_cb_apply(const CbArgs &a, int n_units, hipStream_t s, hipEvent_t start = nullptr,
                           hipEvent_t stop = nullptr);

hipError_t launch_set_identity(int n, int count, double *A, long stride, hipStream_t s);
hipError_t launch_fill(double *p, size_t n, double v, hipStream_t s);
hipError_t launch_set_diag(int n, int nb, int units, double *A, long stride, VecSrc d, hipStream_t s);
hipError_t launch_mat_add(double *A, const double *B, size_t count, hipStream_t s);
hipError_t launch_sub_identity(int n, int units, double *O, const double *A, long stride, hipStream_t s);
hipError_t launch_vec_map(int n, int nb, int units, double *dst, long stride, VecSrc src, hipStream_t s);
hipError_t launch_scale_mat(int n, int nb, int units, double *O, const double *A, long stride, VecSrc row, VecSrc col,
                            int row_first, hipStream_t s);
hipError_t launch_prop_check(int n, int nb, int n_walkers, const double *A, const double *B,
                             long stride_unit, DevStats *stats, unsigned long long *scratch, hipStream_t s);
hipError_t launch_accumulate(int n, int nb, int n_walkers, const double *G, long stride_unit,
                             double *acc, hipStream_t s);
hipError_t launch_mfma_peak(int iters, int blocks, double *sink, hipStream_t s);
hipError_t launch_correlations(int n, int nb, int model, int n_walkers, const double *G, long stride_unit,
                               const int *dir_ptr, const int *pair_src, const int *pair_trg, int n_dirs,
                               double *per_walker, double *acc, hipStream_t s);
hipError_t launch_pairing(int n, int nb, int n_walkers, const double *G, long stride_unit, const int *dir_ptr,
                          const int *pair_src, const int *pair_trg, int n_dirs, int K, const int *trg_of,
                          double *per_walker, double *acc, hipStream_t s);
hipError_t launch_sus_slice(int n, int nb, int model, int n_walkers, const double *G00, const double *G0l,
                            const double *Gl0, const double *Gll, long stride_unit, const int *dir_ptr,
                            const int *pair_src, const int *pair_trg, int n_dirs, int K, const int *trg_of,
                            double *per_walker, long per_stride, hipStream_t s);
hipError_t launch_sus_reduce(int n_walkers, long total, double factor, const double *per_walker, double *acc,
                             hipStream_t s);
constexpr int CC_KMAX = 8;
struct CCPlan {
    int K = 0;
    const int *trg = nullptr;
    const double *tst = nullptr, *tts = nullptr;
    double *bsum = nullptr;
    bool fast = false;
    int C = 0, umax = 0, nchunks = 0, chunks_per_wg = 0, n_wg = 0, threads = 0;
    size_t lds_bytes = 0;
    const int *dsel = nullptr, *rows = nullptr, *ucnt = nullptr, *slot = nullptr;
    double *partial = nullptr;
};
hipError_t launch_cc_b(int n, int nb, int n_walkers, int K, double afac, const double *G00, long stride_unit,
                       const int *trg, const double *tst, const double *tts, double *bsum, hipStream_t s);
hipError_t launch_cc_slice(const CCPlan &p, int n, int nb, int n_walkers, double afac, double xfac,
                           const double *G0l, const double *Gl0, const double *Gll, long stride_unit,
                           const int *dir_ptr, const int *pair_src, const int *pair_trg, int n_dirs,
                           double *per_walker, long per_stride, long offset, hipStream_t s);
enum { BIN_SRC_PLAIN = 0, BIN_SRC_GREENS = 1, BIN_SRC_CORR = 2 };
struct BinPush {
    int mode = BIN_SRC_PLAIN;
    const double *src = nullptr, *G = nullptr;
    long stride_unit = 0;
    int n = 0, nb = 1, model = 0, n_dirs = 0;
    double scale = 1.0;
};
hipError_t launch_binner_push(const BinPush &p, int W, int E, int L, int lmax, double *xs, double *x2, double *c,
                              hipStream_t s);
hipError_t launch_binner_finish(int W, int E, long T, int level, const double *xs, const double *x2, double *out,
                                hipStream_t s);
hipError_t launch_conf_pack(const int8_t *conf, size_t n_elem, unsigned long long *chunks, hipStream_t s);
hipError_t launch_conf_unpack(const unsigned long long *chunks, size_t n_elem, int8_t *conf, hipStream_t s);

}
```

### montecarlo.jl_amd/csrc/kron.hip

```cpp
#include "kernels.h"
#include <hip/hip_ext.h>

namespace dqmc {

typedef double d4k __attribute__((ext_vector_type(4)));
#define KR_MFMA(a, b, c) __builtin_amdgcn_mfma_f64_16x16x4f64((a), (b), (c), 0, 0, 0)

constexpr int KR_N = 256;
constexpr int KR_NC = 4;
constexpr int KR_COLS = 4 * KR_NC;
constexpr int KR_TLD = 17;
constexpr int KR_SLD = 18;
constexpr int KR_LDS_T = 4 * KR_NC * 16 * KR_TLD;
constexpr int KR_LDS_S = KR_N * KR_SLD;
constexpr int KR_LDS = KR_LDS_T > KR_LDS_S ? KR_LDS_T : KR_LDS_S;
constexpr int KR_PF_TS = 16 * 17;
constexpr int KR_PF_IMG = 0, KR_PF_X = 20 * KR_PF_TS, KR_PF_R0 = KR_PF_X + 64, KR_PF_RLD = 65;
constexpr int KR_PF_D = KR_LDS_T, KR_PF_DLD = 257;
constexpr int KR_LDS_PF = KR_PF_D + KR_COLS * KR_PF_DLD;
static_assert(KR_PF_R0 + KR_COLS * KR_PF_RLD <= KR_LDS_PF && KR_LDS <= KR_LDS_PF, "pending-chunk LDS layout");

#define KR_GLOBAL __attribute__((address_space(1)))
typedef const KR_GLOBAL double *kr_gcdp;
typedef double kr_d2 __attribute__((ext_vector_type(2)));
typedef const KR_GLOBAL kr_d2 *kr_gcd2p;
typedef unsigned kr_u4 __attribute__((ext_vector_type(4)));

__device__ __forceinline__ double kr_conf(int8_t c, int sign, bool bn, double epl, double eml)
{
    return (((c > 0) == (sign > 0)) != bn) ? epl : eml;
}

#ifdef KR_STAMPS
__device__ long long *kr_stamp_ptr = nullptr;
#define KR_STAMP(k)                                                                                   \
    do {                                                                                              \
        if (PF && threadIdx.x == 0 && kr_stamp_ptr)                                                   \
            kr_stamp_ptr[16 * blockIdx.x + (k)] = (long long)__builtin_amdgcn_s_memtime();            \
    } while (0)
#define KR_STAMP_RT(k)                                                                                \
    do {                                                                                              \
        if (PF && threadIdx.x == 0 && kr_stamp_ptr)                                                   \
            kr_stamp_ptr[16 * blockIdx.x + (k)] = (long long)__builtin_amdgcn_s_memrealtime();        \
    } while (0)
extern "C" int dqmc_debug_kr_stamps(void *devptr)
{
    return (int)hipMemcpyToSymbol(HIP_SYMBOL(kr_stamp_ptr), &devptr, sizeof(void *));
}
#else
#define KR_STAMP(k) do { } while (0)
#define KR_STAMP_RT(k) do { } while (0)
#endif
template <bool PF>
__device__ __forceinline__ void kr_apply_pending(const KronArgs &a, int unit, int c0, d4k (&v)[KR_NC], double *lds)
{
    const int tid = threadIdx.x, lane = tid & 63, w = tid >> 6, g = lane >> 4, ci = lane & 15;
    const int site0 = a.pf_site0;
    const kr_gcdp img = (kr_gcdp)(a.pf_img + (long)unit * a.pf_img_su);
    const kr_gcdp G = (kr_gcdp)(a.X0 + (long)unit * a.x_su);
    double *limg = lds + KR_PF_IMG, *lx = lds + KR_PF_X, *lr = lds + KR_PF_R0, *ld = lds + KR_PF_D;
    constexpr int NI = LU_IMG / 2 / 256;
    static_assert(NI * 512 == LU_IMG, "image staging");
    kr_d2 iv[NI];
#pragma unroll
    for (int i = 0; i < NI; ++i) iv[i] = reinterpret_cast<kr_gcd2p>(img)[tid + 256 * i];
    const double xin = img[LU_IMG + (tid & 63)];
#pragma unroll
    for (int i = 0; i < NI; ++i) {
        const int p = 2 * (tid + 256 * i), tl = p >> 8, r = (p >> 6) & 3, ln = p & 63;
        double *d = limg + tl * KR_PF_TS + (4 * r + (ln >> 4)) * 17 + (ln & 15);
        d[0] = iv[i].x;
        d[1] = iv[i].y;
    }
    if (tid < 64) lx[tid] = xin;
    {
        const int rr = site0 >> 6;
#pragma unroll
        for (int t = 0; t < KR_NC; ++t) {
            const double r0 = rr == 0 ? v[t][0] : (rr == 1 ? v[t][1] : (rr == 2 ? v[t][2] : v[t][3]));
            lr[(KR_NC * w + t) * KR_PF_RLD + ci + 16 * g] = r0;
        }
    }
    __syncthreads();
    KR_STAMP(2);
    auto A = [&](int tl, int q) { return limg[tl * KR_PF_TS + ci * 17 + 4 * q + g]; };
    auto xr = [&](int J, int r) { return lx[16 * J + 4 * r + g]; };
    constexpr int TU = LU_OFF_U / LU_TILE, TL = LU_OFF_L / LU_TILE, TP = LU_OFF_PT / LU_TILE, TQ = LU_OFF_Q / LU_TILE;
    const kr_gcdp gc = G + 64 * w + ci + (long)KR_N * (site0 + g);
    double ca[2][4][4];
    auto fetch = [&](int J, double (&c)[4][4]) {
#pragma unroll
        for (int q = 0; q < 4; ++q)
#pragma unroll
            for (int mm = 0; mm < 4; ++mm) c[mm][q] = gc[16 * mm + (long)KR_N * (16 * J + 4 * q)];
    };
    fetch(0, ca[0]);
#ifdef KR_PROBE_PRODUCTS
    d4k rh[4];
    {
        double *lw = lr + KR_COLS * KR_PF_RLD, *lh = lr;
        static_assert(KR_PF_R0 + 2 * KR_COLS * KR_PF_RLD <= KR_LDS_PF, "probe LDS");
        d4k pa[4];
#pragma unroll
        for (int J = 0; J < 4; ++J) {
            pa[J] = (d4k){0.0, 0.0, 0.0, 0.0};
            if (J <= w)
#pragma unroll
                for (int q = 0; q < 4; ++q) pa[J] = KR_MFMA(A(TL + J, q), lr[ci * KR_PF_RLD + 16 * J + 4 * q + g], pa[J]);
        }
#pragma unroll
        for (int r = 0; r < 4; ++r)
            lw[ci * KR_PF_RLD + 16 * w + 4 * r + g] = (pa[0][r] + pa[1][r] + pa[2][r] + pa[3][r]) * xr(w, r);
        __syncthreads();
#pragma unroll
        for (int J = 0; J < 4; ++J) {
            pa[J] = (d4k){0.0, 0.0, 0.0, 0.0};
            if (J >= w)
#pragma unroll
                for (int q = 0; q < 4; ++q) pa[J] = KR_MFMA(A(TU + J, q), lw[ci * KR_PF_RLD + 16 * J + 4 * q + g], pa[J]);
        }
#pragma unroll
        for (int r = 0; r < 4; ++r) lh[ci * KR_PF_RLD + 16 * w + 4 * r + g] = pa[0][r] + pa[1][r] + pa[2][r] + pa[3][r];
        __syncthreads();
#pragma unroll
        for (int J = 0; J < 4; ++J)
#pragma unroll
            for (int q = 0; q < 4; ++q) rh[J][q] = lh[ci * KR_PF_RLD + 16 * J + 4 * q + g];
    }
#else
    d4k xv[4], rh[4];
#pragma unroll
    for (int J = 0; J < 4; ++J) {
        d4k acc;
#pragma unroll
        for (int r = 0; r < 4; ++r) acc[r] = lr[ci * KR_PF_RLD + 16 * J + 4 * r + g];
#pragma unroll
        for (int K = 0; K < J; ++K)
#pragma unroll
            for (int q = 0; q < 4; ++q) acc = KR_MFMA(A(TL + lu_pair(K, J), q), xv[K][q], acc);
        d4k z = (d4k){0.0, 0.0, 0.0, 0.0};
#pragma unroll
        for (int q = 0; q < 4; ++q) z = KR_MFMA(A(TQ + J, q), acc[q], z);
#pragma unroll
        for (int r = 0; r < 4; ++r) xv[J][r] = z[r] * xr(J, r);
    }
#pragma unroll
    for (int J = 3; J >= 0; --J) {
        d4k acc = (d4k){0.0, 0.0, 0.0, 0.0};
#pragma unroll
        for (int K = J + 1; K < 4; ++K)
#pragma unroll
            for (int q = 0; q < 4; ++q) acc = KR_MFMA(A(TU + lu_pair(J, K), q), rh[K][q], acc);
#pragma unroll
        for (int r = 0; r < 4; ++r) acc[r] = xv[J][r] + xr(J, r) * acc[r];
        d4k o = (d4k){0.0, 0.0, 0.0, 0.0};
#pragma unroll
        for (int q = 0; q < 4; ++q) o = KR_MFMA(A(TP + J, q), acc[q], o);
        rh[J] = o;
    }
#endif
    KR_STAMP(3);
    d4k dm[4];
#pragma unroll
    for (int mm = 0; mm < 4; ++mm) dm[mm] = (d4k){0.0, 0.0, 0.0, 0.0};
#pragma unroll
    for (int J = 0; J < 4; ++J) {
        if (J < 3) fetch(J + 1, ca[(J + 1) & 1]);
        __builtin_amdgcn_sched_barrier(0);
#pragma unroll
        for (int q = 0; q < 4; ++q)
#pragma unroll
            for (int mm = 0; mm < 4; ++mm) {
                const int i = 16 * (4 * w + mm) + ci, s = 16 * J + 4 * q + g;
                const double c = ca[J & 1][mm][q] - (i == site0 + s ? 1.0 : 0.0);
                dm[mm] = KR_MFMA(c, rh[J][q], dm[mm]);
            }
        __builtin_amdgcn_sched_barrier(0);
    }
    KR_STAMP(4);
    __syncthreads();
#pragma unroll
    for (int mm = 0; mm < 4; ++mm)
#pragma unroll
        for (int r = 0; r < 4; ++r) ld[ci * KR_PF_DLD + 16 * (4 * w + mm) + 4 * r + g] = dm[mm][r];
    __syncthreads();
#pragma unroll
    for (int t = 0; t < KR_NC; ++t)
#pragma unroll
        for (int r = 0; r < 4; ++r) v[t][r] += ld[(KR_NC * w + t) * KR_PF_DLD + ci + 16 * (g + 4 * r)];
}

template <bool PF, bool WT>
__device__ __forceinline__ void kr_chain(const KronArgs &a, const KronStep *steps, int nsteps, const double *x0u, double *ou,
                                         int unit, int c0, double *lds)
{
    const int wk = a.nb == 2 ? unit >> 1 : unit, blk = a.nb == 2 ? unit & 1 : 0;
    const bool bn = blk != 0;
    const int tid = threadIdx.x, lane = tid & 63, w = tid >> 6, g = lane >> 4, ci = lane & 15;
    const long conf_off = (long)wk * a.conf_stride;
    double *tile = lds + w * (KR_NC * 16 * KR_TLD);

    d4k v[KR_NC];
    {
        const double *x0 = x0u + (long)KR_N * (c0 + KR_NC * w) + ci + 16 * g;
#pragma unroll
        for (int t = 0; t < KR_NC; ++t)
#pragma unroll
            for (int r = 0; r < 4; ++r) v[t][r] = x0[KR_N * t + 64 * r];
    }
    auto idx = [&](int par, int r) { return par ? (g + 4 * r) + 16 * ci : ci + 16 * (g + 4 * r); };
    struct Ops {
        double av[4], bv[4];
        int8_t cpre[4], cpost[4];
    };
    auto request = [&](int s, Ops &o) {
        const KronStep &st = steps[s];
        const int par = s & 1;
        const double *fx = st.ax + KR_N * blk, *fy = st.ay + KR_N * blk;
        const double *fa = par ? fx : fy, *fb = par ? fy : fx;
#pragma unroll
        for (int q = 0; q < 4; ++q) {
            o.av[q] = fa[ci + 16 * (4 * q + g)];
            o.bv[q] = fb[ci + 16 * (4 * q + g)];
        }
        const int8_t *dummy = reinterpret_cast<const int8_t *>(x0u);
        const int8_t *pre = st.pre_conf ? st.pre_conf + conf_off : dummy, *post = st.post_conf ? st.post_conf + conf_off : dummy;
#pragma unroll
        for (int r = 0; r < 4; ++r) {
            o.cpre[r] = pre[st.pre_conf ? idx(par, r) : 0];
            o.cpost[r] = post[st.post_conf ? idx(par ^ 1, r) : 0];
        }
    };
    Ops cur, nxt;
    request(0, cur);
    double cs[KR_NC];
    {
        const double *cd = a.col_d ? a.col_d + (long)unit * a.col_stride + c0 + KR_NC * w : x0u;
#pragma unroll
        for (int t = 0; t < KR_NC; ++t) cs[t] = cd[t];
    }
    if constexpr (PF) kr_apply_pending<PF>(a, unit, c0, v, lds);
    KR_STAMP(5);

    for (int s = 0; s < nsteps; ++s) {
        const KronStep &st = steps[s];
        if (st.pre_conf) {
#pragma unroll
            for (int r = 0; r < 4; ++r) {
                const double f = kr_conf(cur.cpre[r], st.pre_sign, bn, a.epl, a.eml);
#pragma unroll
                for (int t = 0; t < KR_NC; ++t) v[t][r] *= f;
            }
        }
#pragma unroll
        for (int t = 0; t < KR_NC; ++t) {
            d4k p = (d4k){0.0, 0.0, 0.0, 0.0};
#pragma unroll
            for (int q = 0; q < 4; ++q) p = KR_MFMA(cur.av[q], v[t][q], p);
#pragma unroll
            for (int r = 0; r < 4; ++r) tile[t * 16 * KR_TLD + (g + 4 * r) * KR_TLD + ci] = p[r];
        }
        request(min(s + 1, nsteps - 1), nxt);
        __syncthreads();
#pragma unroll
        for (int t = 0; t < KR_NC; ++t) {
            d4k q4 = (d4k){0.0, 0.0, 0.0, 0.0};
#pragma unroll
            for (int q = 0; q < 4; ++q) q4 = KR_MFMA(cur.bv[q], tile[t * 16 * KR_TLD + ci * KR_TLD + 4 * q + g], q4);
            v[t] = q4;
        }
        __syncthreads();
        if (st.post_conf) {
#pragma unroll
            for (int r = 0; r < 4; ++r) {
                const double f = kr_conf(cur.cpost[r], st.post_sign, bn, a.epl, a.eml);
#pragma unroll
                for (int t = 0; t < KR_NC; ++t) v[t][r] *= f;
            }
        }
        cur = nxt;
    }
    KR_STAMP(6);
    const int par = nsteps & 1;
#pragma unroll
    for (int t = 0; t < KR_NC; ++t) {
        const int cl = KR_NC * w + t;
#pragma unroll
        for (int r = 0; r < 4; ++r) {
            const int i = idx(par, r);
            lds[a.transpose_out ? i * KR_SLD + cl : cl * KR_N + i] = a.col_d ? v[t][r] * cs[t] : v[t][r];
        }
    }
    __syncthreads();
    double *o = ou;
    if constexpr (WT) {
        const __amdgpu_buffer_rsrc_t rs = __builtin_amdgcn_make_buffer_rsrc(o, 0, KR_N * KR_N * (int)sizeof(double), 0x00020000);
#pragma unroll
        for (int k = 0; k < 8; ++k) {
            const int e = 2 * (tid + 256 * k), i = e >> 4, cl = e & 15;
            __builtin_amdgcn_raw_buffer_store_b128(*reinterpret_cast<const kr_u4 *>(lds + i * KR_SLD + cl), rs,
                                                   (c0 + KR_N * i + cl) * (int)sizeof(double), 0, 16 );
        }
    } else if (a.transpose_out) {
#pragma unroll
        for (int k = 0; k < 8; ++k) {
            const int e = 2 * (tid + 256 * k), i = e >> 4, cl = e & 15;
            *reinterpret_cast<double2 *>(o + c0 + (long)KR_N * i + cl) = *reinterpret_cast<const double2 *>(lds + i * KR_SLD + cl);
        }
    } else {
#pragma unroll
        for (int k = 0; k < 8; ++k) {
            const int e = 2 * (tid + 256 * k);
            *reinterpret_cast<double2 *>(o + (long)KR_N * c0 + e) = *reinterpret_cast<const double2 *>(lds + e);
// ... 115 lines not shown
```

### montecarlo.jl_amd/csrc/sweep_lu.hip

```cpp
#include "kernels.h"
#include <hip/hip_ext.h>
#include <cstdlib>

namespace dqmc {

typedef double d4 __attribute__((ext_vector_type(4)));

size_t sweep_lu_image_doubles() { return LU_STRIDE; }

__device__ __forceinline__ double readlane_d(double v, int lane)
{
    const unsigned long long u = (unsigned long long)__double_as_longlong(v);
    const unsigned lo = (unsigned)__builtin_amdgcn_readlane((int)(u & 0xffffffffull), lane);
    const unsigned hi = (unsigned)__builtin_amdgcn_readlane((int)(u >> 32), lane);
    return __longlong_as_double((long long)(((unsigned long long)hi << 32) | lo));
}
#define MFMA(a, b, c) __builtin_amdgcn_mfma_f64_16x16x4f64((a), (b), (c), 0, 0, 0)
#define DQMC_GLOBAL __attribute__((address_space(1)))
typedef const DQMC_GLOBAL double *gcdp;
typedef DQMC_GLOBAL double *gdp;
typedef double d2v __attribute__((ext_vector_type(2)));
typedef const DQMC_GLOBAL d2v *gcd2p;


constexpr int LU4_SPIN = 1 << 21;
template <int NB>
struct Lu4Smem {
    double2 aST[NB][64][64];
    double xs[NB][64];
    double strip[12][NB][2][64];
    double negv[64];
    int step[64];
    int sflag[12];
    unsigned acc16[4], neg16[4];
    int ndraw[4], exh[4];
    int abort;
};
__host__ __device__ constexpr int lu4_strip_idx(int I0, int r0, int I) { return I0 == 0 ? r0 * 2 + (I - 1) : 8 + r0; }

#define LU4_ORDER() asm volatile("" ::: "memory")

__device__ __forceinline__ int lu4_wait(int *flag, int *abortf)
{
    int v = 0;
    for (int it = 0; it < LU4_SPIN; ++it) {
        v = __builtin_amdgcn_readfirstlane(__hip_atomic_load(flag, __ATOMIC_RELAXED, __HIP_MEMORY_SCOPE_WORKGROUP));
        if (v) break;
        if ((it & 63) == 63 &&
            __builtin_amdgcn_readfirstlane(__hip_atomic_load(abortf, __ATOMIC_RELAXED, __HIP_MEMORY_SCOPE_WORKGROUP)))
            return -1;
        __builtin_amdgcn_s_sleep(1);
    }
    if (!v) {
        __hip_atomic_store(abortf, 1, __ATOMIC_RELAXED, __HIP_MEMORY_SCOPE_WORKGROUP);
        return -1;
    }
    LU4_ORDER();
    return v;
}
__device__ __forceinline__ double lu4_rcp(double r)
{
    double y = __builtin_amdgcn_rcp(r);
    double e = __builtin_fma(-r, y, 1.0);
    y = __builtin_fma(y, e, y);
    e = __builtin_fma(-r, y, 1.0);
    return __builtin_fma(y, e, y);
}

extern __shared__ __attribute__((aligned(16))) double lu4_lds[];
#ifdef LU4_STAMPS
__device__ long long *lu4_stamp_ptr = nullptr;
#define LU4_STAMP(idx)                                                                       \
    do {                                                                                     \
        if ((LU4_STAMPS != 2 || (idx) >= 320) && w == 0 && (threadIdx.x & 63) == 0 && lu4_stamp_ptr)            \
            lu4_stamp_ptr[(idx)] = (long long)__builtin_amdgcn_s_memtime();                  \
    } while (0)
#else
#define LU4_STAMP(idx) do { } while (0)
#endif
#ifdef LU4_STAMPS
#ifndef FL_STAMP_BID
#define FL_STAMP_BID 1200
#endif
#define FL_STAMP(k)                                                                                    \
    do {                                                                                               \
        if (bid == FL_STAMP_BID && threadIdx.x == 0 && lu4_stamp_ptr)                                 \
            lu4_stamp_ptr[480 + (k)] = (long long)__builtin_amdgcn_s_memtime();                       \
    } while (0)
#else
#define FL_STAMP(k) do { } while (0)
#endif
template <int NB, bool FULL, bool PRO, int J>
__device__ __noinline__ void lu4_wave(int n, const double *__restrict__ Gall, long strideG, int w, int site0,
                                      int nsites, double *__restrict__ img_all, const SweepConsts &sc,
                                      unsigned long long cbits_v, double uvec, int check_sign, int site0p,
                                      const double *__restrict__ imgp_all)
{
    Lu4Smem<NB> &sm = *reinterpret_cast<Lu4Smem<NB> *>(lu4_lds);
    const int lane = threadIdx.x & 63, g = lane >> 4, ci = lane & 15;
    const unsigned long long cbits =
        ((unsigned long long)(unsigned)__builtin_amdgcn_readfirstlane((int)(cbits_v >> 32)) << 32) |
        (unsigned)__builtin_amdgcn_readfirstlane((int)(cbits_v & 0xffffffffull));
    d4 S[NB][J + 1], ST[NB][J + 1];
#pragma unroll
    for (int b = 0; b < NB; ++b) {
        const gcdp G = (gcdp)(Gall + (long)(w * NB + b) * strideG + (long)site0 * n + site0);
#pragma unroll
        for (int I = 0; I <= J; ++I)
#pragma unroll
            for (int r = 0; r < 4; ++r) {
                const int rho = 16 * I + 4 * r + g, kap = 16 * J + ci;
                if (FULL) {
                    S[b][I][r] = G[rho + (long)n * kap];
                    ST[b][I][r] = G[kap + (long)n * rho];
                } else {
                    const bool ok = rho < nsites && kap < nsites;
                    const int rc = min(rho, nsites - 1), kc = min(kap, nsites - 1);
                    const double a = G[rc + (long)n * kc], c = G[kc + (long)n * rc];
                    S[b][I][r] = ok ? a : 0.0;
                    ST[b][I][r] = ok ? c : 0.0;
                }
            }
    }
    if (PRO) {
        LU4_STAMP(400 + 8 * J + 0);
        constexpr bool EARLY = (NB == 1) && (sizeof(Lu4Smem<NB>) + LU_STRIDE * sizeof(double) <= 150 * 1024);
        double *xtra = lu4_lds + (sizeof(Lu4Smem<NB>) + 15) / 16 * 2 + LU_STRIDE;
        double *Rl = EARLY ? reinterpret_cast<double *>(&sm.aST[0][31][0]) : reinterpret_cast<double *>(&sm.aST[0][0][0]);
        double *ttx = EARLY ? xtra : Rl + 64 * 66;
        double *tt0 = xtra + 1536;
        int *pflag = reinterpret_cast<int *>(xtra + 1536 + 1024);
        const int tid = threadIdx.x;
#pragma unroll 1
        for (int b = 0; b < NB; ++b) {
            const gcdp Gin = (gcdp)(Gall + (long)(w * NB + b) * strideG);
            const gcdp imgp = (gcdp)(imgp_all + (long)(w * NB + b) * LU_STRIDE);
            const int t = site0 + 16 * J + ci;
            d4 az[4];
#pragma unroll
            for (int Jb = 0; Jb < 4; ++Jb)
#pragma unroll
                for (int r = 0; r < 4; ++r) az[Jb][r] = Gin[t + (long)n * (site0p + 16 * Jb + 4 * r + g)];
            d2v r0v[8];
            {
                const int tl = tid >> 2, s0 = (tid & 3) * 16;
                const gcd2p q = reinterpret_cast<gcd2p>(Gin + (long)n * (site0 + tl) + site0p + s0);
#pragma unroll
                for (int i = 0; i < 8; ++i) r0v[i] = q[i];
            }
            constexpr bool STAGE = sizeof(Lu4Smem<NB>) + LU_STRIDE * sizeof(double) <= 150 * 1024;
            double *imgl = lu4_lds + (sizeof(Lu4Smem<NB>) + 15) / 16 * 2;
            double opU[STAGE ? 1 : 6][4], opL[STAGE ? 1 : 6][4], opP[STAGE ? 1 : 4][4], opQ[STAGE ? 1 : 4][4], xr[4][4];
            if (STAGE) {
                constexpr int NI = (LU_STRIDE / 2 + 255) / 256;
                const gcd2p src = reinterpret_cast<gcd2p>(imgp);
                d2v *dst = reinterpret_cast<d2v *>(imgl);
                d2v iv[NI];
#pragma unroll
                for (int i = 0; i < NI; ++i) iv[i] = src[min(tid + 256 * i, LU_STRIDE / 2 - 1)];
#pragma unroll
                for (int i = 0; i < NI; ++i)
                    if (tid + 256 * i < LU_STRIDE / 2) dst[tid + 256 * i] = iv[i];
            } else {
#pragma unroll
                for (int pr = 0; pr < (STAGE ? 0 : 6); ++pr)
#pragma unroll
                    for (int q = 0; q < 4; ++q) {
                        opU[pr][q] = imgp[LU_OFF_U + pr * LU_TILE + q * 64 + lane];
                        opL[pr][q] = imgp[LU_OFF_L + pr * LU_TILE + q * 64 + lane];
                    }
#pragma unroll
                for (int Jb = 0; Jb < (STAGE ? 0 : 4); ++Jb)
#pragma unroll
                    for (int q = 0; q < 4; ++q) {
                        opP[Jb][q] = imgp[LU_OFF_PT + Jb * LU_TILE + q * 64 + lane];
                        opQ[Jb][q] = imgp[LU_OFF_Q + Jb * LU_TILE + q * 64 + lane];
                    }
            }
            {
                const int tl = tid >> 2, s0 = (tid & 3) * 16;
                d2v *d = reinterpret_cast<d2v *>(Rl + tl * 66 + s0);
#pragma unroll
                for (int i = 0; i < 8; ++i) d[i] = r0v[i];
            }
            if (STAGE) __syncthreads();
#pragma unroll
            for (int Jb = 0; Jb < 4; ++Jb)
#pragma unroll
                for (int q = 0; q < 4; ++q) xr[Jb][q] = STAGE ? imgl[LU_IMG + 16 * Jb + 4 * q + g] : imgp[LU_IMG + 16 * Jb + 4 * q + g];
#define PRO_U(pr, q) (STAGE ? imgl[LU_OFF_U + (pr) * LU_TILE + (q) * 64 + lane] : opU[STAGE ? 0 : (pr)][q])
#define PRO_L(pr, q) (STAGE ? imgl[LU_OFF_L + (pr) * LU_TILE + (q) * 64 + lane] : opL[STAGE ? 0 : (pr)][q])
#define PRO_P(jb, q) (STAGE ? imgl[LU_OFF_PT + (jb) * LU_TILE + (q) * 64 + lane] : opP[STAGE ? 0 : (jb)][q])
#define PRO_Q(jb, q) (STAGE ? imgl[LU_OFF_Q + (jb) * LU_TILE + (q) * 64 + lane] : opQ[STAGE ? 0 : (jb)][q])
            d4 xz[4], tt[4];
#if defined(LU4_STAMPS) && LU4_STAMPS != 2
            LU4_STAMP(400 + 8 * J + 1);
            asm volatile("s_waitcnt vmcnt(0)" ::: "memory");
            LU4_STAMP(400 + 8 * J + 2);
#endif
#pragma unroll
            for (int Jb = 0; Jb < 4; ++Jb) {
#pragma unroll
                for (int K = 0; K < Jb; ++K)
#pragma unroll
                    for (int q = 0; q < 4; ++q) az[Jb] = MFMA(PRO_U(lu_pair(K, Jb), q), xz[K][q], az[Jb]);
                d4 z = {0.0, 0.0, 0.0, 0.0};
#pragma unroll
                for (int q = 0; q < 4; ++q) z = MFMA(PRO_P(Jb, q), az[Jb][q], z);
#pragma unroll
                for (int r = 0; r < 4; ++r) xz[Jb][r] = z[r] * xr[Jb][r];
            }
#pragma unroll
            for (int Jb = 3; Jb >= 0; --Jb) {
                d4 a = {0.0, 0.0, 0.0, 0.0};
#pragma unroll
                for (int K = Jb + 1; K < 4; ++K)
#pragma unroll
                    for (int q = 0; q < 4; ++q) a = MFMA(PRO_L(lu_pair(Jb, K), q), tt[K][q], a);
#pragma unroll
                for (int r = 0; r < 4; ++r) a[r] = xz[Jb][r] + xr[Jb][r] * a[r];
                d4 o = {0.0, 0.0, 0.0, 0.0};
#pragma unroll
                for (int q = 0; q < 4; ++q) o = MFMA(PRO_Q(Jb, q), a[q], o);
                tt[Jb] = o;
            }
#undef PRO_U
#undef PRO_L
#undef PRO_P
#undef PRO_Q
            LU4_STAMP(400 + 8 * J + 3);
            if (EARLY) {
                double *dlt = ttx;
                if (J == 0) {
#pragma unroll
                    for (int K = 0; K < 4; ++K)
#pragma unroll
                        for (int q = 0; q < 4; ++q) tt0[(K * 4 + q) * 64 + lane] = tt[K][q];
                    LU4_ORDER();
                    __hip_atomic_store(&pflag[0], 1, __ATOMIC_RELAXED, __HIP_MEMORY_SCOPE_WORKGROUP);
#pragma unroll
                    for (int K = 0; K < 4; ++K)
#pragma unroll
                        for (int q = 0; q < 4; ++q) {
                            const int sk = 16 * K + 4 * q + g;
                            ST[b][0] = MFMA(Rl[ci * 66 + sk], tt[K][q], ST[b][0]);
                            S[b][0] = MFMA(tt[K][q], Rl[ci * 66 + sk], S[b][0]);
                        }
                } else {
#pragma unroll
                    for (int K = 0; K < 4; ++K)
#pragma unroll
                        for (int q = 0; q < 4; ++q) {
                            const int sk = 16 * K + 4 * q + g;
#pragma unroll
                            for (int I = 0; I <= J; ++I) ST[b][I] = MFMA(Rl[(16 * I + ci) * 66 + sk], tt[K][q], ST[b][I]);
                            S[b][J] = MFMA(tt[K][q], Rl[(16 * J + ci) * 66 + sk], S[b][J]);
                        }
#pragma unroll
                    for (int Jc = J + 1; Jc < 4; ++Jc) {
                        d4 dl = {0.0, 0.0, 0.0, 0.0};
#pragma unroll
                        for (int K = 0; K < 4; ++K)
#pragma unroll
                            for (int q = 0; q < 4; ++q) dl = MFMA(tt[K][q], Rl[(16 * Jc + ci) * 66 + 16 * K + 4 * q + g], dl);
#pragma unroll
                        for (int r = 0; r < 4; ++r) dlt[(lu_pair(J, Jc) * 4 + r) * 64 + lane] = dl[r];
                    }
                    LU4_ORDER();
                    __hip_atomic_store(&pflag[J], 1, __ATOMIC_RELAXED, __HIP_MEMORY_SCOPE_WORKGROUP);
                    if (lu4_wait(&pflag[0], &sm.abort) > 0) {
#pragma unroll
                        for (int K = 0; K < 4; ++K)
#pragma unroll
                            for (int q = 0; q < 4; ++q)
                                S[b][0] = MFMA(tt0[(K * 4 + q) * 64 + lane], Rl[(16 * J + ci) * 66 + 16 * K + 4 * q + g], S[b][0]);
                    }
#pragma unroll
                    for (int I = 1; I < J; ++I)
                        if (lu4_wait(&pflag[I], &sm.abort) > 0) {
#pragma unroll
                            for (int r = 0; r < 4; ++r) S[b][I][r] += dlt[(lu_pair(I, J) * 4 + r) * 64 + lane];
                        }
                    LU4_ORDER();
                    __hip_atomic_store(&pflag[4 + J], 1, __ATOMIC_RELAXED, __HIP_MEMORY_SCOPE_WORKGROUP);
                }
                continue;
            }
            if (!STAGE) __syncthreads();
            LU4_STAMP(400 + 8 * J + 4);
            double *dlt = ttx;
#pragma unroll
            for (int K = 0; K < 4; ++K)
#pragma unroll
                for (int q = 0; q < 4; ++q) {
                    const int sk = 16 * K + 4 * q + g;
#pragma unroll
                    for (int I = 0; I <= J; ++I)
                        ST[b][I] = MFMA(Rl[(16 * I + ci) * 66 + sk], tt[K][q], ST[b][I]);
                    S[b][J] = MFMA(tt[K][q], Rl[(16 * J + ci) * 66 + sk], S[b][J]);
                }
#pragma unroll
            for (int Jc = J + 1; Jc < 4; ++Jc) {
                d4 dl = {0.0, 0.0, 0.0, 0.0};
#pragma unroll
                for (int K = 0; K < 4; ++K)
#pragma unroll
                    for (int q = 0; q < 4; ++q) dl = MFMA(tt[K][q], Rl[(16 * Jc + ci) * 66 + 16 * K + 4 * q + g], dl);
#pragma unroll
                for (int r = 0; r < 4; ++r) dlt[(lu_pair(J, Jc) * 4 + r) * 64 + lane] = dl[r];
            }
            __syncthreads();
#pragma unroll
            for (int I = 0; I < J; ++I)
#pragma unroll
                for (int r = 0; r < 4; ++r) S[b][I][r] += dlt[(lu_pair(I, J) * 4 + r) * 64 + lane];
            __syncthreads();
        }
        LU4_STAMP(320 + 8 * J + 7);
    }
    LU4_STAMP(320 + 8 * J + 0);
#if defined(LU4_STAMPS) && LU4_STAMPS != 2
    asm volatile("s_waitcnt vmcnt(0)" ::: "memory");
    LU4_STAMP(320 + 8 * J + 1);
#endif
    auto sgpr = [](double v) {
        const unsigned long long u = (unsigned long long)__double_as_longlong(v);
        const unsigned lo = (unsigned)__builtin_amdgcn_readfirstlane((int)(u & 0xffffffffull));
        const unsigned hi = (unsigned)__builtin_amdgcn_readfirstlane((int)(u >> 32));
        return __longlong_as_double((long long)(((unsigned long long)hi << 32) | lo));
    };
    const double g0 = sgpr(sc.gamma[0]), g1 = sgpr(sc.gamma[1]), e0 = sgpr(sc.ebos[0]), e1 = sgpr(sc.ebos[1]);
    const double du0 = sgpr(sc.dup[0]), du1 = sgpr(sc.dup[1]), dd0 = sgpr(sc.ddn[0]), dd1 = sgpr(sc.ddn[1]);
    int lastflag = 0;

#pragma unroll
    for (int I0 = 0; I0 < 4; ++I0) {
        if (!FULL && 16 * I0 >= nsites) break;
        const bool PIV = (I0 == J), HLP = (J > I0), PTQ = (J == (I0 == 0 ? 3 : (I0 == 3 ? 1 : 0)));
        if (!PIV && !HLP && !PTQ) continue;
        d4 PT[NB], Q[NB];
        if (PTQ) {
#pragma unroll
            for (int b = 0; b < NB; ++b)
#pragma unroll
                for (int r = 0; r < 4; ++r) PT[b][r] = Q[b][r] = (4 * r + g == ci) ? 1.0 : 0.0;
        }
        int ndraw = (lastflag >> 3) & 0xfff, exhausted = (lastflag >> 2) & 1;
        unsigned accb = 0, negb = 0;
        double negv = 0.0;
        int pf_v = 0;
        double2 pf_pay[NB];
        double pf_xh[NB];
#pragma unroll
        for (int b = 0; b < NB; ++b) { pf_pay[b] = make_double2(0.0, 0.0); pf_xh[b] = 0.0; }
        double dcur[NB];
        if (PIV) {
            if (PRO && NB == 1 && I0 >= 1 && sizeof(Lu4Smem<NB>) + LU_STRIDE * sizeof(double) <= 150 * 1024) {
                int *pflag = reinterpret_cast<int *>(lu4_lds + (sizeof(Lu4Smem<NB>) + 15) / 16 * 2 + LU_STRIDE + 1536 + 1024);
                (void)lu4_wait(&pflag[5], &sm.abort);
                (void)lu4_wait(&pflag[6], &sm.abort);
                (void)lu4_wait(&pflag[7], &sm.abort);
            }
#pragma unroll
            for (int b = 0; b < NB; ++b) dcur[b] = readlane_d(S[b][J][0], 0);
        }
#pragma unroll
        for (int r0 = 0; r0 < 4; ++r0) {
            double xv4[NB];
#pragma unroll
            for (int b = 0; b < NB; ++b) xv4[b] = 0.0;
            unsigned panel_acc = 0;
#pragma unroll
            for (int ks = 0; ks < 4; ++ks) {
                const int c = 4 * r0 + ks, s = 16 * I0 + c;
                if (!FULL && s >= nsites) continue;
                if (PIV) {
                    LU4_STAMP(s);
                    const int spin = (int)((cbits >> s) & 1ull);
                    double det, p, xb[NB];
                    if (NB == 1) {
                        const double gamma = spin ? g1 : g0;
                        const double r = 1.0 + gamma * (1.0 - dcur[0]);
                        det = r * r;
                        p = (spin ? e1 : e0) * det;
                        xb[0] = gamma * lu4_rcp(r);
                    } else {
                        const double D0 = spin ? du1 : du0, D1 = spin ? dd1 : dd0;
                        const double R0 = 1.0 + D0 * (1.0 - dcur[0]), R1 = 1.0 + D1 * (1.0 - dcur[NB - 1]);
                        det = R0 * R1;
                        p = det;
                        const double inv_div = lu4_rcp(det);
                        xb[0] = (R1 * inv_div) * D0;
                        xb[NB - 1] = (R0 * inv_div) * D1;
                        if (check_sign && det < 0.0) {
                            negb |= 1u << c;
                            negv = lane == s ? det : negv;
                        }
                    }
                    bool acc;
                    if (p > 1.0) acc = true;
                    else {
                        const double u = readlane_d(uvec, ndraw);
                        ++ndraw;
                        if (u == 2.0) exhausted = 1;
                        acc = u < p;
                    }
                    const int word = (ndraw << 3) | (exhausted << 2);
                    const bool more = c < 15 && (FULL || s + 1 < nsites);
                    constexpr int dummy = 0;
                    (void)dummy;
                    const int c1 = c + 1, l1 = 16 * (c1 & 3) + c1;
                    {
                        const bool accu = __builtin_amdgcn_readfirstlane((int)acc) != 0;
                        accb |= (accu ? 1u : 0u) << c;
                        const bool lm2 = g == ks && ci > c;
#pragma unroll
                        for (int b = 0; b < NB; ++b) {
                            const double x = accu ? xb[b] : 0.0;
                            const double mS = lm2 ? S[b][J][r0] : 0.0, mT = lm2 ? ST[b][J][r0] : 0.0;
                            const double aS = x * mT, aT = x * mS;
                            if (more) {
                                const double qs = readlane_d(mT * mS, 16 * ks + c1);
                                dcur[b] = __builtin_fma(x, qs, readlane_d(S[b][J][c1 >> 2], l1));
                            }
                            S[b][J] = MFMA(aS, mS, S[b][J]);
                            sm.aST[b][s][lane] = make_double2(aS, aT);
                            sm.xs[b][s] = x;
                            ST[b][J] = MFMA(aT, mT, ST[b][J]);
                        }
                        LU4_ORDER();
                        __hip_atomic_store(&sm.step[s], word | (accu ? 2 : 1), __ATOMIC_RELAXED, __HIP_MEMORY_SCOPE_WORKGROUP);
                    }
                    lastflag = word;
                } else {
                    int v = c > 0 ? __builtin_amdgcn_readfirstlane(pf_v) : 0;
                    double2 pay[NB];
                    double xh[NB];
#pragma unroll
                    for (int b = 0; b < NB; ++b) { pay[b] = pf_pay[b]; xh[b] = pf_xh[b]; }
                    for (int it = 0; v == 0 && it < LU4_SPIN; ++it) {
                        const int vr = __hip_atomic_load(&sm.step[s], __ATOMIC_RELAXED, __HIP_MEMORY_SCOPE_WORKGROUP);
                        LU4_ORDER();
#pragma unroll
                        for (int b = 0; b < NB; ++b) {
                            pay[b] = sm.aST[b][s][lane];
                            xh[b] = sm.xs[b][s];
                        }
                        v = __builtin_amdgcn_readfirstlane(vr);
                        if (v) break;
                        if ((it & 63) == 63 && __builtin_amdgcn_readfirstlane(__hip_atomic_load(
                                                   &sm.abort, __ATOMIC_RELAXED, __HIP_MEMORY_SCOPE_WORKGROUP))) {
                            v = -1;
                            break;
                        }
                        __builtin_amdgcn_s_sleep(1);
                    }
                    if (v == 0) {
                        __hip_atomic_store(&sm.abort, 1, __ATOMIC_RELAXED, __HIP_MEMORY_SCOPE_WORKGROUP);
                        v = -1;
                    }
                    if (v > 0) lastflag = v;
                    if (c < 15 && (FULL || s + 1 < nsites)) {
                        pf_v = __hip_atomic_load(&sm.step[s + 1], __ATOMIC_RELAXED, __HIP_MEMORY_SCOPE_WORKGROUP);
                        LU4_ORDER();
#pragma unroll
                        for (int b = 0; b < NB; ++b) {
                            pf_pay[b] = sm.aST[b][s + 1][lane];
                            pf_xh[b] = sm.xs[b][s + 1];
                        }
                    }
                    LU4_STAMP(64 * (1 + J) + s);
                    if (v > 0 && (v & 3) == 2) {
                        panel_acc |= 1u << ks;
#pragma unroll
                        for (int b = 0; b < NB; ++b) {
                            const double aS = pay[b].x, aT = pay[b].y;
                            if (HLP) {
                                xv4[b] = g == ks ? xh[b] : xv4[b];
                                S[b][I0] = MFMA(aS, S[b][I0][r0], S[b][I0]);
                                ST[b][I0] = MFMA(aT, ST[b][I0][r0], ST[b][I0]);
                            }
                            if (PTQ) {
                                PT[b] = MFMA(aT, PT[b][r0], PT[b]);
                                Q[b] = MFMA(aS, Q[b][r0], Q[b]);
                            }
                        }
                    }
                }
            }
            if (HLP && panel_acc != 0) {
                if (J < 3) {
#pragma unroll
                    for (int b = 0; b < NB; ++b) {
                        sm.strip[lu4_strip_idx(I0, r0, J)][b][0][lane] = S[b][I0][r0];
                        sm.strip[lu4_strip_idx(I0, r0, J)][b][1][lane] = ST[b][I0][r0];
                    }
                    LU4_ORDER();
                    __hip_atomic_store(&sm.sflag[lu4_strip_idx(I0, r0, J)], 1, __ATOMIC_RELAXED, __HIP_MEMORY_SCOPE_WORKGROUP);
                }
#pragma unroll
                for (int b = 0; b < NB; ++b) {
                    S[b][J] = MFMA(xv4[b] * ST[b][I0][r0], S[b][I0][r0], S[b][J]);
                    ST[b][J] = MFMA(xv4[b] * S[b][I0][r0], ST[b][I0][r0], ST[b][J]);
                }
#pragma unroll
                for (int I = I0 + 1; I < J; ++I) {
                    const int ok = lu4_wait(&sm.sflag[lu4_strip_idx(I0, r0, I)], &sm.abort);
                    if (ok > 0) {
#pragma unroll
                        for (int b = 0; b < NB; ++b) {
                            const double rs = sm.strip[lu4_strip_idx(I0, r0, I)][b][0][lane];
                            const double rt = sm.strip[lu4_strip_idx(I0, r0, I)][b][1][lane];
                            S[b][I] = MFMA(xv4[b] * rt, S[b][I0][r0], S[b][I]);
                            ST[b][I] = MFMA(xv4[b] * rs, ST[b][I0][r0], ST[b][I]);
                        }
                    }
                }
            }
        }
        LU4_STAMP(320 + 8 * J + 2 + I0);
#pragma unroll
        for (int b = 0; b < NB; ++b) {
            const gdp img = (gdp)(img_all + (long)(w * NB + b) * LU_STRIDE);
#pragma unroll
            for (int r = 0; r < 4; ++r) {
                const int tpos = (ci >> 2) * 64 + 16 * (ci & 3) + 4 * r + g;
                if (HLP) {
                    img[LU_OFF_U + lu_pair(I0, J) * LU_TILE + r * 64 + lane] = S[b][I0][r];
                    img[LU_OFF_L + lu_pair(I0, J) * LU_TILE + tpos] = ST[b][I0][r];
                }
                if (PTQ) {
                    img[LU_OFF_PT + I0 * LU_TILE + tpos] = PT[b][r];
                    img[LU_OFF_Q + I0 * LU_TILE + r * 64 + lane] = Q[b][r];
                }
            }
            if (PIV && (lane >> 4) == I0) img[LU_IMG + lane] = sm.xs[b][lane];
        }
        if (PIV) {
            if (lane == 0) {
                sm.acc16[I0] = accb;
                sm.neg16[I0] = negb;
                sm.ndraw[I0] = ndraw;
                sm.exh[I0] = exhausted;
            }
            if (NB == 2 && (lane >> 4) == I0) sm.negv[lane] = negv;
        }
    }
    LU4_STAMP(320 + 8 * J + 6);
}

template <int NB, bool FULL, bool PRO>
__device__ __forceinline__ void lu4_block(int w, int n, const double *__restrict__ Gall, long strideG,
                                          int8_t *__restrict__ conf_slice, long conf_stride, int site0, int nsites,
                                          double *__restrict__ img_all, const SweepConsts &sc, WalkerRng *rngs,
                                          DevStats *stats, int check_sign, int *errflag, int site0p,
                                          const double *__restrict__ imgp_all)
{
    Lu4Smem<NB> &sm = *reinterpret_cast<Lu4Smem<NB> *>(lu4_lds);
    const int tid = threadIdx.x, lane = tid & 63, wave = tid >> 6;
    int8_t *__restrict__ cw = conf_slice + (long)w * conf_stride;
    const int myc = (FULL || lane < nsites) ? (int)cw[site0 + (FULL ? lane : min(lane, nsites - 1))] : 1;
    const unsigned long long cbits = __ballot(myc > 0);
    const WalkerRng rs = rngs[w];
    double uvec;
    {
        const unsigned long long d = rs.draw + (unsigned long long)lane;
        uvec = rs.uniforms ? (d < rs.n_uniforms ? rs.uniforms[d] : 2.0) : philox_uniform(rs.seed, d);
    }
    if (tid < 64) {
        sm.step[tid] = 0;
        for (int b = 0; b < NB; ++b) sm.xs[b][tid] = 0.0;
    }
    if (tid < 12) sm.sflag[tid] = 0;
#ifdef LU4_STAMPS
    if (w == 0 && tid == 0 && lu4_stamp_ptr) lu4_stamp_ptr[360] = (long long)__builtin_amdgcn_s_memtime();
#endif
    if (tid < 4) { sm.acc16[tid] = 0u; sm.neg16[tid] = 0u; sm.ndraw[tid] = 0; sm.exh[tid] = 0; }
    if (tid == 0) sm.abort = 0;
    if (PRO && NB == 1 && tid < 8)
        reinterpret_cast<int *>(lu4_lds + (sizeof(Lu4Smem<NB>) + 15) / 16 * 2 + LU_STRIDE + 1536 + 1024)[tid] = 0;
    __syncthreads();
    const int wv = __builtin_amdgcn_readfirstlane(wave);
    if (wv == 0) lu4_wave<NB, FULL, PRO, 0>(n, Gall, strideG, w, site0, nsites, img_all, sc, cbits, uvec, check_sign, site0p, imgp_all);
    else if (wv == 1) lu4_wave<NB, FULL, PRO, 1>(n, Gall, strideG, w, site0, nsites, img_all, sc, cbits, uvec, check_sign, site0p, imgp_all);
    else if (wv == 2) lu4_wave<NB, FULL, PRO, 2>(n, Gall, strideG, w, site0, nsites, img_all, sc, cbits, uvec, check_sign, site0p, imgp_all);
    else lu4_wave<NB, FULL, PRO, 3>(n, Gall, strideG, w, site0, nsites, img_all, sc, cbits, uvec, check_sign, site0p, imgp_all);
    __syncthreads();
    const int nblk = (nsites + 15) / 16;
    if (!FULL) {
        const int I0 = wv, g = lane >> 4, ci = lane & 15;
        if (I0 >= nblk)
            for (int b = 0; b < NB; ++b) {
                const gdp img = (gdp)(img_all + (long)(w * NB + b) * LU_STRIDE);
                for (int r = 0; r < 4; ++r) {
                    const double idv = (4 * r + g == ci) ? 1.0 : 0.0;
                    for (int Jc = I0 + 1; Jc < 4; ++Jc) {
                        img[LU_OFF_U + lu_pair(I0, Jc) * LU_TILE + r * 64 + lane] = 0.0;
                        img[LU_OFF_L + lu_pair(I0, Jc) * LU_TILE + r * 64 + lane] = 0.0;
                    }
                    img[LU_OFF_PT + I0 * LU_TILE + r * 64 + lane] = idv;
                    img[LU_OFF_Q + I0 * LU_TILE + r * 64 + lane] = idv;
                }
                if (lane < 16) img[LU_IMG + 16 * I0 + lane] = 0.0;
            }
    }
    if (wv == 0) {
        const unsigned long long accbits = (unsigned long long)sm.acc16[0] | ((unsigned long long)sm.acc16[1] << 16) |
                                           ((unsigned long long)sm.acc16[2] << 32) | ((unsigned long long)sm.acc16[3] << 48);
        if (lane < nsites && ((accbits >> lane) & 1ull)) cw[site0 + lane] = (int8_t)(-myc);
        if (lane == 0) {
            rngs[w].draw = rs.draw + (unsigned long long)sm.ndraw[nblk - 1];
            if (sm.exh[nblk - 1]) rngs[w].exhausted = 1;
            stats[w].prop_local += nsites;
            stats[w].acc_local += __popcll(accbits);
            if (sm.abort) atomicOr(errflag, 2);
#ifdef LU4_STAMPS
            if (w == 0 && lu4_stamp_ptr) lu4_stamp_ptr[361] = (long long)__builtin_amdgcn_s_memtime();
#endif
            if (NB == 2)
                for (int s = 0; s < nsites; ++s)
                    if ((sm.neg16[s >> 4] >> (s & 15)) & 1u) magstats_push(stats[w].negative_probability, sm.negv[s]);
        }
    }
}

template <int NB, bool FULL>
__global__ __launch_bounds__(256) void sweep_lu4_kernel(int n, const double *__restrict__ Gall, long strideG,
                                                       int8_t *__restrict__ conf_slice, long conf_stride, int site0,
                                                       int nsites, double *__restrict__ img_all, SweepConsts sc,
                                                       WalkerRng *rngs, DevStats *stats, int check_sign, int *errflag)
{
    lu4_block<NB, FULL, false>(blockIdx.x, n, Gall, strideG, conf_slice, conf_stride, site0, nsites, img_all, sc, rngs,
                               stats, check_sign, errflag, 0, nullptr);
}

hipError_t launch_sweep_lu(int n, int nb, int n_walkers, const double *G, long strideG, int8_t *conf_slice,
                           long conf_stride, int site0, int nsites, double *img, SweepConsts sc, WalkerRng *rng,
                           DevStats *stats, int check_sign, int *errflag, hipStream_t s, hipEvent_t start,
                           hipEvent_t stop)
{
    if (nsites < 1 || nsites > 64 || site0 < 0 || site0 + nsites > n || nb < 1 || nb > 2) return hipErrorInvalidValue;
    const bool full = nsites == 64;
    int dev = 0;
    (void)hipGetDevice(&dev);
    static unsigned attr_mask = 0;
    if (!(attr_mask & (1u << dev))) {
        (void)hipFuncSetAttribute((const void *)sweep_lu4_kernel<1, true>, hipFuncAttributeMaxDynamicSharedMemorySize, (int)sizeof(Lu4Smem<1>));
        (void)hipFuncSetAttribute((const void *)sweep_lu4_kernel<1, false>, hipFuncAttributeMaxDynamicSharedMemorySize, (int)sizeof(Lu4Smem<1>));
        (void)hipFuncSetAttribute((const void *)sweep_lu4_kernel<2, true>, hipFuncAttributeMaxDynamicSharedMemorySize, (int)sizeof(Lu4Smem<2>));
        (void)hipFuncSetAttribute((const void *)sweep_lu4_kernel<2, false>, hipFuncAttributeMaxDynamicSharedMemorySize, (int)sizeof(Lu4Smem<2>));
        attr_mask |= 1u << dev;
    }
    dim3 grid(n_walkers), block(256);
#define LU4_LAUNCH(NBV, FL)                                                                                          \
    hipExtLaunchKernelGGL((sweep_lu4_kernel<NBV, FL>), grid, block, sizeof(Lu4Smem<NBV>), s, start, stop, 0, n, G, strideG, \
                          conf_slice, conf_stride, site0, nsites, img, sc, rng, stats, check_sign, errflag)
    if (nb == 1) { if (full) LU4_LAUNCH(1, true); else LU4_LAUNCH(1, false); }
    else { if (full) LU4_LAUNCH(2, true); else LU4_LAUNCH(2, false); }
#undef LU4_LAUNCH
    return hipGetLastError();
}

constexpr int FL_LDR = 66;
template <bool FULL, int NT, int NCP = 1>
__device__ __forceinline__ void flush_lu_body(int bid, int n, int n_units, const double *__restrict__ Gin_all,
                                              double *__restrict__ Gout_all, long strideG, int site0, int nsites,
                                              const double *__restrict__ img_all, int tiles_m, int tiles_n,
                                              int ncp_rt = 1)
{
    const int ncp = NCP > 0 ? NCP : ncp_rt;
    double *fsm = lu4_lds;
    double *img = fsm;
    double *xs = fsm + LU_IMG;
    double *Rl = fsm + LU_STRIDE;
    const int xcd = bid & 7, seq = bid >> 3;
    const int T = tiles_m * tiles_n;
    const int unit = (seq / T) * 8 + xcd;
    if (unit >= n_units) return;
    const int tile = seq % T;
    const int m0 = (tile % tiles_m) * 64, n00 = (tile / tiles_m) * (16 * NT * ncp);
    int n0 = n00;
    const gcdp Gin = (gcdp)(Gin_all + (long)unit * strideG);
    const gdp Gout = (gdp)(Gout_all + (long)unit * strideG);
    const int tid = threadIdx.x, lane = tid & 63, wave = tid >> 6, g = lane >> 4, ci = lane & 15;
    const int t = m0 + 16 * wave + ci;
    const int tq = FULL ? t : min(t, n - 1);

    FL_STAMP(0);
    d4 acc[NT];
#pragma unroll
    for (int jt = 0; jt < NT; ++jt)
#pragma unroll
        for (int r = 0; r < 4; ++r) {
            const int tp = n0 + 16 * jt + 4 * r + g;
            acc[jt][r] = Gin[tq + (long)n * (FULL ? tp : min(tp, n - 1))];
        }
    d4 az[4];
#pragma unroll
    for (int J = 0; J < 4; ++J)
#pragma unroll
        for (int r = 0; r < 4; ++r) {
            const int s = 16 * J + 4 * r + g;
            const int col = site0 + (FULL ? s : min(s, nsites - 1));
            double v = Gin[tq + (long)n * col];
            if (!FULL && (s >= nsites || t >= n)) v = 0.0;
            az[J][r] = v - ((t == site0 + s) ? 1.0 : 0.0);
        }
    {
        const gcd2p src = reinterpret_cast<gcd2p>((gcdp)(img_all + (long)unit * LU_STRIDE));
        d2v *dst = reinterpret_cast<d2v *>(img);
        for (int i = tid; i < LU_STRIDE / 2; i += 256) dst[i] = src[i];
    }
#pragma unroll
    for (int pass = 0; pass < NT / 4; ++pass) {
        const int tl = pass * 64 + (tid >> 2), tp = n0 + tl, s0 = (tid & 3) * 16;
        double *d = Rl + tl * FL_LDR + s0;
        if (FULL) {
            d2v rv[8];
#pragma unroll
            for (int i = 0; i < 8; ++i) {
                const int pc = i * 256 + tid, col = pass * 64 + (pc >> 5), w2 = 2 * (pc & 31);
                rv[i] = *reinterpret_cast<gcd2p>(Gin + (long)n * (n0 + col) + site0 + w2);
            }
#pragma unroll
            for (int i = 0; i < 8; ++i) {
                const int pc = i * 256 + tid, col = pass * 64 + (pc >> 5), w2 = 2 * (pc & 31);
                *reinterpret_cast<d2v *>(Rl + col * FL_LDR + w2) = rv[i];
            }
        } else {
            for (int i = 0; i < 16; ++i)
                d[i] = (tp < n && s0 + i < nsites) ? Gin[(long)n * tp + site0 + s0 + i] : 0.0;
        }
    }
    __syncthreads();
    FL_STAMP(1);

    d4 xz[4];
#pragma unroll
    for (int J = 0; J < 4; ++J) {
#pragma unroll
        for (int K = 0; K < J; ++K)
#pragma unroll
            for (int q = 0; q < 4; ++q)
                az[J] = MFMA(img[LU_OFF_U + lu_pair(K, J) * LU_TILE + q * 64 + lane], xz[K][q], az[J]);
        d4 z = {0.0, 0.0, 0.0, 0.0};
#pragma unroll
        for (int q = 0; q < 4; ++q) z = MFMA(img[LU_OFF_PT + J * LU_TILE + q * 64 + lane], az[J][q], z);
#pragma unroll
        for (int r = 0; r < 4; ++r) xz[J][r] = z[r] * xs[16 * J + 4 * r + g];
    }
    d4 tt[4];
#pragma unroll
    for (int J = 3; J >= 0; --J) {
        d4 a = {0.0, 0.0, 0.0, 0.0};
#pragma unroll
        for (int K = J + 1; K < 4; ++K)
#pragma unroll
            for (int q = 0; q < 4; ++q)
                a = MFMA(img[LU_OFF_L + lu_pair(J, K) * LU_TILE + q * 64 + lane], tt[K][q], a);
#pragma unroll
        for (int r = 0; r < 4; ++r) a[r] = xz[J][r] + xs[16 * J + 4 * r + g] * a[r];
        d4 o = {0.0, 0.0, 0.0, 0.0};
#pragma unroll
        for (int q = 0; q < 4; ++q) o = MFMA(img[LU_OFF_Q + J * LU_TILE + q * 64 + lane], a[q], o);
        tt[J] = o;
    }
    if constexpr (NCP == 0 && FULL && NT == 4) {
        const int rb_off[2] = {(int)(Rl - fsm), 0};
        FL_STAMP(2);
        __syncthreads();
        FL_STAMP(3);
        for (int cp = 0; cp < ncp; ++cp) {
            const bool more = cp + 1 < ncp;
            const int n1 = n00 + (more ? cp + 1 : cp) * 64;
            d4 nxt[NT];
            double r0n[16];
#pragma unroll
            for (int jt = 0; jt < NT; ++jt)
#pragma unroll
                for (int r = 0; r < 4; ++r) nxt[jt][r] = Gin[t + (long)n * (n1 + 16 * jt + 4 * r + g)];
#pragma unroll
            for (int i = 0; i < 8; ++i) {
                const int pc = i * 256 + tid;
                const d2v v = *reinterpret_cast<gcd2p>(Gin + (long)n * (n1 + (pc >> 5)) + site0 + 2 * (pc & 31));
                r0n[2 * i] = v.x;
                r0n[2 * i + 1] = v.y;
            }
            const double *Rc = fsm + rb_off[cp & 1];
#pragma unroll
            for (int K = 0; K < 4; ++K)
#pragma unroll
                for (int q = 0; q < 4; ++q) {
                    const int sk = 16 * K + 4 * q + g;
#pragma unroll
                    for (int jt = 0; jt < NT; ++jt) acc[jt] = MFMA(Rc[(16 * jt + ci) * FL_LDR + sk], tt[K][q], acc[jt]);
                }
            n0 = n00 + cp * 64;
#pragma unroll
            for (int jt = 0; jt < NT; ++jt)
#pragma unroll
                for (int r = 0; r < 4; ++r) Gout[t + (long)n * (n0 + 16 * jt + 4 * r + g)] = acc[jt][r];
            if (more) {
                double *nb = fsm + rb_off[(cp + 1) & 1];
#pragma unroll
                for (int i = 0; i < 8; ++i) {
                    const int pc = i * 256 + tid;
                    *reinterpret_cast<double2 *>(nb + (pc >> 5) * FL_LDR + 2 * (pc & 31)) = make_double2(r0n[2 * i], r0n[2 * i + 1]);
                }
#pragma unroll
                for (int jt = 0; jt < NT; ++jt) acc[jt] = nxt[jt];
                __syncthreads();
            }
            FL_STAMP(4 + cp);
        }
        return;
    }
    for (int cp = 0; cp < ncp; ++cp) {
        if (cp > 0) {
            n0 = n00 + cp * 16 * NT;
#pragma unroll
            for (int jt = 0; jt < NT; ++jt)
#pragma unroll
                for (int r = 0; r < 4; ++r) {
                    const int tp = n0 + 16 * jt + 4 * r + g;
                    acc[jt][r] = Gin[tq + (long)n * (FULL ? tp : min(tp, n - 1))];
                }
            __syncthreads();
#pragma unroll
            for (int pass = 0; pass < NT / 4; ++pass) {
                const int tl = pass * 64 + (tid >> 2), tp = n0 + tl, s0 = (tid & 3) * 16;
                double *d = Rl + tl * FL_LDR + s0;
                if (FULL) {
                    d2v rv[8];
#pragma unroll
                    for (int i = 0; i < 8; ++i) {
                        const int pc = i * 256 + tid, col = pass * 64 + (pc >> 5), w2 = 2 * (pc & 31);
                        rv[i] = *reinterpret_cast<gcd2p>(Gin + (long)n * (n0 + col) + site0 + w2);
                    }
#pragma unroll
                    for (int i = 0; i < 8; ++i) {
                        const int pc = i * 256 + tid, col = pass * 64 + (pc >> 5), w2 = 2 * (pc & 31);
                        *reinterpret_cast<d2v *>(Rl + col * FL_LDR + w2) = rv[i];
                    }
                } else {
                    for (int i = 0; i < 16; ++i)
                        d[i] = (tp < n && s0 + i < nsites) ? Gin[(long)n * tp + site0 + s0 + i] : 0.0;
                }
            }
            __syncthreads();
        }
#pragma unroll
        for (int K = 0; K < 4; ++K)
#pragma unroll
            for (int q = 0; q < 4; ++q) {
                const int sk = 16 * K + 4 * q + g;
#pragma unroll
                for (int jt = 0; jt < NT; ++jt)
                    acc[jt] = MFMA(Rl[(16 * jt + ci) * FL_LDR + sk], tt[K][q], acc[jt]);
            }
#pragma unroll
        for (int jt = 0; jt < NT; ++jt)
#pragma unroll
            for (int r = 0; r < 4; ++r) {
                const int tp = n0 + 16 * jt + 4 * r + g;
                if (FULL || (t < n && tp < n)) Gout[t + (long)n * tp] = acc[jt][r];
            }
    }
}

template <bool FULL, int NT, int NCP = 1>
__global__ __launch_bounds__(256) void sweep_flush_lu_kernel(int n, int n_units, const double *__restrict__ Gin_all,
                                                            double *__restrict__ Gout_all, long strideG, int site0,
                                                            int nsites, const double *__restrict__ img_all,
                                                            int tiles_m, int tiles_n, int ncp_rt)
{
    flush_lu_body<FULL, NT, NCP>(blockIdx.x, n, n_units, Gin_all, Gout_all, strideG, site0, nsites, img_all, tiles_m, tiles_n,
                                 ncp_rt);
}

struct SweepFusedArgs {
    int n, n_walkers, n_units;
    const double *Gin;
    double *Gout;
    long strideG;
    int8_t *conf_slice;
    long conf_stride;
    int site0, site0p;
    double *img;
    const double *imgp;
    SweepConsts sc;
    WalkerRng *rngs;
    DevStats *stats;
    int check_sign;
    int *errflag;
    int tiles_m, tiles_n;
};
template <int NB, int NT, int NCP>
__global__ __launch_bounds__(256) void sweep_fused_kernel(SweepFusedArgs a)
{
    if ((int)blockIdx.x < a.n_walkers)
        lu4_block<NB, true, true>(blockIdx.x, a.n, a.Gin, a.strideG, a.conf_slice, a.conf_stride, a.site0, 64, a.img, a.sc,
                                  a.rngs, a.stats, a.check_sign, a.errflag, a.site0p, a.imgp);
    else
        flush_lu_body<true, NT, NCP>((int)blockIdx.x - a.n_walkers, a.n, a.n_units, a.Gin, a.Gout, a.strideG, a.site0p, 64,
                                     a.imgp, a.tiles_m, a.tiles_n);
}


hipError_t launch_sweep_flush_lu(int n, int n_units, const double *Gin, double *Gout, long strideG, int site0,
                                 int nsites, const double *img, const KernelSwitches &sw, hipStream_t s, hipEvent_t start,
                                 hipEvent_t stop)
{
    const bool wide = n % 128 == 0;
    const int nt = wide ? 8 : 4;
    const int tm = (n + 63) / 64, tn = (n + 16 * nt - 1) / (16 * nt);
    const int groups = (n_units + 7) / 8;
    const size_t lds = ((size_t)LU_STRIDE + 16 * nt * FL_LDR) * sizeof(double);
    const bool full = (n % 64 == 0) && nsites == 64;
    int dev = 0;
    (void)hipGetDevice(&dev);
    static unsigned attr_mask = 0;
    if (!(attr_mask & (1u << dev))) {
        const int big = (int)(((size_t)LU_STRIDE + 128 * FL_LDR) * sizeof(double));
        (void)hipFuncSetAttribute((const void *)sweep_flush_lu_kernel<true, 8>, hipFuncAttributeMaxDynamicSharedMemorySize, big);
        (void)hipFuncSetAttribute((const void *)sweep_flush_lu_kernel<false, 8>, hipFuncAttributeMaxDynamicSharedMemorySize, big);
        (void)hipFuncSetAttribute((const void *)sweep_flush_lu_kernel<true, 4>, hipFuncAttributeMaxDynamicSharedMemorySize, big);
        (void)hipFuncSetAttribute((const void *)sweep_flush_lu_kernel<false, 4>, hipFuncAttributeMaxDynamicSharedMemorySize, big);
        attr_mask |= 1u << dev;
    }
#define FL_LAUNCH(FU, NTV)                                                                                          \
    hipExtLaunchKernelGGL((sweep_flush_lu_kernel<FU, NTV>), dim3(groups * 8 * tm * tn), dim3(256), lds, s, start, stop, 0, \
                          n, n_units, Gin, Gout, strideG, site0, nsites, img, tm, tn, 1)
    static int n_cus[32] = {0};
    if (dev >= 0 && dev < 32 && n_cus[dev] == 0) {
        hipDeviceProp_t prop;
        n_cus[dev] = hipGetDeviceProperties(&prop, dev) == hipSuccess ? prop.multiProcessorCount : 256;
    }
    const bool ncp2 = sw.flush_ncp2 || (dev >= 0 && dev < 32 && groups * 8 * tm * tn > n_cus[dev]);
    if (ncp2 && full && (n + 63) / 64 > 1) {
        const int tn4 = (n + 63) / 64;
        const size_t lds4 = ((size_t)LU_STRIDE + 64 * FL_LDR) * sizeof(double);
        static unsigned m0 = 0;
        if (!(m0 & (1u << dev))) {
            (void)hipFuncSetAttribute((const void *)sweep_flush_lu_kernel<true, 4, 0>, hipFuncAttributeMaxDynamicSharedMemorySize,
                                      (int)(((size_t)LU_STRIDE + 128 * FL_LDR) * sizeof(double)));
            m0 |= 1u << dev;
        }
        hipExtLaunchKernelGGL((sweep_flush_lu_kernel<true, 4, 0>), dim3(groups * 8 * tm), dim3(256), lds4, s, start, stop, 0, n,
                              n_units, Gin, Gout, strideG, site0, nsites, img, tm, 1, tn4);
        return hipGetLastError();
    }
    if (wide) { if (full) FL_LAUNCH(true, 8); else FL_LAUNCH(false, 8); }
    else { if (full) FL_LAUNCH(true, 4); else FL_LAUNCH(false, 4); }
#undef FL_LAUNCH
    return hipGetLastError();
}

hipError_t launch_sweep_fused(int n, int nb, int n_walkers, const double *Gin, double *Gout, long strideG,
                              int8_t *conf_slice, long conf_stride, int site0, int site0p, double *img,
                              const double *imgp, SweepConsts sc, WalkerRng *rng, DevStats *stats, int check_sign,
                              int *errflag, hipStream_t s, hipEvent_t start, hipEvent_t stop)
{
    if (n % 64 != 0 || site0 % 64 != 0 || site0p % 64 != 0 || site0 + 64 > n || site0p + 64 > n || nb < 1 || nb > 2)
        return hipErrorInvalidValue;
    const int n_units = n_walkers * nb;
    const bool wide = n % 128 == 0;
    const int nt = wide ? 8 : 4;
    SweepFusedArgs a;
    a.n = n; a.n_walkers = n_walkers; a.n_units = n_units; a.Gin = Gin; a.Gout = Gout; a.strideG = strideG;
    a.conf_slice = conf_slice; a.conf_stride = conf_stride; a.site0 = site0; a.site0p = site0p; a.img = img; a.imgp = imgp;
    a.sc = sc; a.rngs = rng; a.stats = stats; a.check_sign = check_sign; a.errflag = errflag;
    const int ncp = (wide && n % 256 == 0) ? 2 : 1;
    a.tiles_m = n / 64; a.tiles_n = n / (16 * nt * ncp);
    const int groups = (n_units + 7) / 8;
    const int flush_blocks = groups * 8 * a.tiles_m * a.tiles_n;
    const size_t lds_flush = ((size_t)LU_STRIDE + 16 * nt * FL_LDR) * sizeof(double);
    const size_t lds_lu = nb == 1 ? sizeof(Lu4Smem<1>) : sizeof(Lu4Smem<2>);
    const size_t lds_pro = nb == 1 ? (sizeof(Lu4Smem<1>) + 15) / 16 * 16 + (LU_STRIDE + 1536 + 1024 + 8) * sizeof(double) : lds_lu;
    const size_t lds_e = lds_pro > lds_lu ? lds_pro : lds_lu;
    const size_t lds = lds_flush > lds_e ? lds_flush : lds_e;
    int dev = 0;
    (void)hipGetDevice(&dev);
    static unsigned attr_mask = 0;
    if (!(attr_mask & (1u << dev))) {
        (void)hipFuncSetAttribute((const void *)sweep_fused_kernel<1, 8, 1>, hipFuncAttributeMaxDynamicSharedMemorySize, 160 * 1024);
        (void)hipFuncSetAttribute((const void *)sweep_fused_kernel<1, 8, 2>, hipFuncAttributeMaxDynamicSharedMemorySize, 160 * 1024);
        (void)hipFuncSetAttribute((const void *)sweep_fused_kernel<1, 4, 1>, hipFuncAttributeMaxDynamicSharedMemorySize, 160 * 1024);
        (void)hipFuncSetAttribute((const void *)sweep_fused_kernel<2, 8, 1>, hipFuncAttributeMaxDynamicSharedMemorySize, 160 * 1024);
        (void)hipFuncSetAttribute((const void *)sweep_fused_kernel<2, 8, 2>, hipFuncAttributeMaxDynamicSharedMemorySize, 160 * 1024);
        (void)hipFuncSetAttribute((const void *)sweep_fused_kernel<2, 4, 1>, hipFuncAttributeMaxDynamicSharedMemorySize, 160 * 1024);
        attr_mask |= 1u << dev;
    }
    dim3 grid(n_walkers + flush_blocks), block(256);
#define FU_LAUNCH(NBV, NTV, NCPV) hipExtLaunchKernelGGL((sweep_fused_kernel<NBV, NTV, NCPV>), grid, block, lds, s, start, stop, 0, a)
    if (nb == 1) { if (ncp == 2) FU_LAUNCH(1, 8, 2); else if (wide) FU_LAUNCH(1, 8, 1); else FU_LAUNCH(1, 4, 1); }
    else { if (ncp == 2) FU_LAUNCH(2, 8, 2); else if (wide) FU_LAUNCH(2, 8, 1); else FU_LAUNCH(2, 4, 1); }
#undef FU_LAUNCH
    return hipGetLastError();
}

#ifdef LU4_STAMPS
extern "C" int dqmc_debug_lu4_stamps(void *devptr)
{
    return (int)hipMemcpyToSymbol(HIP_SYMBOL(lu4_stamp_ptr), &devptr, sizeof(void *));
}
#endif

}
```

### montecarlo.jl_amd/dqmc.py

```python
import ctypes as C
import time
from dataclasses import dataclass

import numpy as np

from . import _lib
from ._lib import check, dptr, i64ptr, lib
from .configurations import CompressedConf, ConfigRecorder
from .models import rand_conf


@dataclass
class DQMCParameters:
    thermalization: int = 100
    sweeps: int = 100
    check_sign_problem: bool = True
    check_propagation_error: bool = True
    safe_mult: int = 10
    delta_tau: float = 0.1
    beta: float = 1.0
    slices: int = 10
    measure_rate: int = 10

    @staticmethod
# ... 593 lines not shown
        res["n_walkers"] = raw["n_walkers"]
        return res

    def set_pair_directions(self, iterator):
        tab = np.asfortranarray(iterator.dir_of.astype(np.int32))
        self._ndirs = iterator.ndirections()
        self._c(lib().dqmc_set_pair_directions(self._h, tab.ctypes.data_as(C.POINTER(C.c_int32)), self._ndirs))

    def accumulate_correlations(self):
        self._c(lib().dqmc_accumulate_correlations(self._h))

    def correlations_raw(self):
        n = C.c_size_t()
        self._c(lib().dqmc_correlations_size(self._h, C.byref(n)))
        out = np.zeros(n.value)
        self._c(lib().dqmc_get_correlations(self._h, dptr(out)))
        return out

    def correlations(self):
        n = C.c_size_t()
        self._c(lib().dqmc_correlations_size(self._h, C.byref(n)))
        out = np.zeros(n.value)
        self._c(lib().dqmc_get_correlations(self._h, dptr(out)))
        nd, N, cnt = self._ndirs, self.N, out[-1]
        names = ["CDC", "SDCx", "SDCy", "SDCz"]
        res = {k: out[i * nd:(i + 1) * nd] / cnt for i, k in enumerate(names)}
        for i, k in enumerate(["Mx", "My", "Mz"]):
            res[k] = out[4 * nd + i * N:4 * nd + (i + 1) * N] / cnt
        res["count"] = cnt
        return res

    def set_local_targets(self, iterator):
        self.set_pair_directions(iterator.pairs_by_dir)
        tab = np.asfortranarray(iterator.trg_of.astype(np.int32))
        self._K = iterator.K
        self._c(lib().dqmc_set_local_targets(self._h, tab.ctypes.data_as(C.POINTER(C.c_int32)), self._K))

    def accumulate_pairing(self):
        self._c(lib().dqmc_accumulate_pairing(self._h))

    def pairing(self):
        n = C.c_size_t()
        self._c(lib().dqmc_pairing_size(self._h, C.byref(n)))
        out = np.zeros(n.value)
        self._c(lib().dqmc_get_pairing(self._h, dptr(out)))
        cnt = out[-1]
        return out[:-1].reshape((self._ndirs, self._K, self._K), order="F") / cnt, cnt

    def ut_build_stack(self):
        self._c(lib().dqmc_ut_build_stack(self._h))

    def ut_stack(self, which, idx, walker=0):
        sel = {"forward": 0, "backward": 1, "inverse": 2}[which]
        U = np.zeros(self.nb * self.N * self.N); T = np.zeros_like(U); D = np.zeros(self.nb * self.N)
        self._c(lib().dqmc_ut_get_stack(self._h, walker, sel, idx, dptr(U), dptr(D), dptr(T)))
        return self._blocks(U), [D[b * self.N:(b + 1) * self.N] for b in range(self.nb)], self._blocks(T)

    def _ut_result(self, which, walker):
        out = np.zeros(self.nb * self.N * self.N)
        self._c(lib().dqmc_ut_get(self._h, walker, which, dptr(out)))
        return self._blocks(out)

    def calculate_greens_kl(self, slice1, slice2, walker=0):
        self._c(lib().dqmc_ut_greens(self._h, slice1, slice2, 1))
        return self._ut_result(0, walker)

    def greens_kl(self, slice1, slice2, walker=None):
        self._c(lib().dqmc_ut_greens(self._h, slice1, slice2, 0))
        if walker is None:
            return [self._ut_result(0, w) for w in range(self.n_walkers)]
        return self._ut_result(0, walker)

    def greens_iterator(self, l=0, recalculate=None, walker=0):
        recalculate = 4 * self.p.safe_mult if recalculate is None else recalculate
        self._c(lib().dqmc_greens_iterator_begin(self._h, l, recalculate))
        yield self._ut_result(0, walker)
        k = C.c_int32()
        while True:
            self._c(lib().dqmc_greens_iterator_next(self._h, C.byref(k)))
            if k.value < 0:
                return
            yield self._ut_result(0, walker)

    def combined_greens_iterator(self, recalculate=None, walker=0):
        recalculate = 4 * self.p.safe_mult if recalculate is None else recalculate
        self._c(lib().dqmc_combined_iterator_begin(self._h, recalculate))
        l = C.c_int32()
        while True:
            self._c(lib().dqmc_combined_iterator_next(self._h, C.byref(l)))
            if l.value < 0:
                return
            yield tuple(self._ut_result(i, walker) for i in range(3))

    def accumulate_susceptibilities(self, recalculate=None):
        recalculate = 4 * self.p.safe_mult if recalculate is None else recalculate
        self._c(lib().dqmc_accumulate_susceptibilities(self._h, recalculate))

    def susceptibilities(self):
        n = C.c_size_t()
        self._c(lib().dqmc_susceptibilities_size(self._h, C.byref(n)))
        out = np.zeros(n.value)
        self._c(lib().dqmc_get_susceptibilities(self._h, dptr(out)))
        nd, cnt = self._ndirs, out[-1]
        res = {k: out[i * nd:(i + 1) * nd] / cnt for i, k in enumerate(["CDS", "SDSx", "SDSy", "SDSz"])}
        K = getattr(self, "_K", 0)
        if K:
            res["PS"] = out[4 * nd:4 * nd + nd * K * K].reshape((nd, K, K), order="F") / cnt
        Kcc = getattr(self, "_Kcc", 0)
        if Kcc:
            off = 4 * nd + nd * K * K
            res["CCS"] = out[off:off + nd * Kcc].reshape((nd, Kcc), order="F") / cnt
        res["count"] = cnt
        return res

    def set_current_targets(self, iterator, hopping=None):
        self.set_pair_directions(iterator.pairs_by_dir)
        blocks = self.model.hopping_matrix() if hopping is None else hopping
        if isinstance(blocks, np.ndarray) and blocks.ndim == 2:
            blocks = [blocks]
        if len(blocks) != self.nb or any(np.shape(b) != (self.N, self.N) for b in blocks):
            raise ValueError("hopping must be %d matrices of %d x %d" % (self.nb, self.N, self.N))
        self._cc_T = np.ascontiguousarray(np.concatenate([np.asarray(b, dtype=np.float64).reshape(-1, order="F")
                                                          for b in blocks]))
        tab = np.asfortranarray(iterator.trg_of.astype(np.int32))
        self._c(lib().dqmc_set_current_targets(self._h, tab.ctypes.data_as(C.POINTER(C.c_int32)), iterator.K,
                                               dptr(self._cc_T)))
        self._Kcc = iterator.K

    def current_targets_fast_path(self):
        f = C.c_int32()
        self._c(lib().dqmc_current_targets_fast_path(self._h, C.byref(f)))
        return bool(f.value)

    def qr_fallbacks(self):
        n = C.c_int64()
        self._c(lib().dqmc_qr_fallbacks(self._h, C.byref(n)))
        return n.value

    def kron_hopping(self):
        f = C.c_int32(0)
        self._c(lib().dqmc_kron_hopping(self._h, C.byref(f)))
        return bool(f.value)

    def udt_one_launch_sites(self):
        w = C.c_int32(0)
        self._c(lib().dqmc_udt_one_launch_sites(self._h, C.byref(w)))
        return int(w.value)

    def device_errors(self):
        w = C.c_int32(0)
        self._c(lib().dqmc_device_errors(self._h, C.byref(w)))
        return int(w.value)

    def timing_enable(self, on=True):
        self._c(lib().dqmc_timing_enable(self._h, int(on)))

    def timing(self):
        ms = np.zeros(len(_lib.K_FAMILIES))
        n = np.zeros(len(_lib.K_FAMILIES), dtype=np.int64)
        self._c(lib().dqmc_timing_get(self._h, dptr(ms), i64ptr(n)))
        return {k: (float(ms[i]), int(n[i])) for i, k in enumerate(_lib.K_FAMILIES)}


def finish_moments(buf):
    if hasattr(buf, "detach"):
        buf = buf.detach().cpu().numpy()
    buf = np.asarray(buf, dtype=np.float64)
    E, W = (buf.size - 1) // 4, buf[-1]
    if buf.ndim != 1 or buf.size != 4 * E + 1 or W < 1:
        raise ValueError("not a binner moment buffer")
    s1, s2, vl, v0 = (buf[i * E:(i + 1) * E] for i in range(4))
    with np.errstate(invalid="ignore", divide="ignore"):
        between = np.maximum(s2 - s1 * s1 / W, 0.0) / (W * (W - 1)) if W >= 2 else np.full(E, np.nan)
        return dict(mean=s1 / W, std_error=np.sqrt(np.where(vl < 0, 0.0, vl)) / W, std_error_walkers=np.sqrt(between),
                    tau=0.5 * (vl / v0 - 1.0), n_walkers=int(W))


def _batch(a):
    a = np.asarray(a, dtype=np.float64)
    if a.ndim == 2:
        a = a[None]
    return a


def _pack(mats):
    return np.ascontiguousarray(np.concatenate([m.reshape(-1, order="F") for m in mats]))


def _unpack(flat, batch, n):
    return np.stack([flat[i * n * n:(i + 1) * n * n].reshape((n, n), order="F") for i in range(batch)])


def vmul(A, B, transa=False, transb=False, device_id=0):
    A, B = _batch(A), _batch(B)
    batch, n = A.shape[0], A.shape[1]
    a, b = _pack(A), _pack(B)
    c = np.zeros_like(a)
    check(lib().dqmc_vmul(device_id, n, batch, int(transa), int(transb), dptr(a), dptr(b), dptr(c)))
    return _unpack(c, batch, n)


def udt_AVX_pivot(X, apply_pivot=True, device_id=0):
    X = _batch(X)
    batch, n = X.shape[0], X.shape[1]
    t = _pack(X)
    u = np.zeros_like(t)
    d = np.zeros(batch * n)
    piv = np.zeros(batch * n, dtype=np.int64)
    check(lib().dqmc_udt_pivot(device_id, n, batch, dptr(u), dptr(d), dptr(t), i64ptr(piv), int(apply_pivot)))
    return _unpack(u, batch, n), d.reshape(batch, n), _unpack(t, batch, n), piv.reshape(batch, n)


def rdivp(A, T, pivot, device_id=0):
    A, T = _batch(A), _batch(T)
    batch, n = A.shape[0], A.shape[1]
    a, t = _pack(A), _pack(T)
    piv = np.ascontiguousarray(np.asarray(pivot, dtype=np.int64).reshape(-1))
    check(lib().dqmc_rdivp(device_id, n, batch, dptr(a), dptr(t), i64ptr(piv)))
    return _unpack(a, batch, n)


def calculate_greens_AVX(Ul, Dl, Tl, Ur, Dr, Tr, device_id=0):
    Ul, Tl, Ur, Tr = _batch(Ul), _batch(Tl), _batch(Ur), _batch(Tr)
    batch, n = Ul.shape[0], Ul.shape[1]
    dl = np.ascontiguousarray(np.asarray(Dl, dtype=np.float64).reshape(-1))
    dr = np.ascontiguousarray(np.asarray(Dr, dtype=np.float64).reshape(-1))
    g = np.zeros(batch * n * n)
    check(lib().dqmc_calculate_greens(device_id, n, batch, dptr(_pack(Ul)), dptr(dl), dptr(_pack(Tl)),
                                      dptr(_pack(Ur)), dptr(dr), dptr(_pack(Tr)), dptr(g)))
    return _unpack(g, batch, n)


def mfma_f64_peak(iters=20000, device_id=0):
    t = C.c_double()
    check(lib().dqmc_mfma_f64_peak(device_id, iters, C.byref(t)))
    return t.value


def device_count():
    return lib().dqmc_device_count()
```

Measured before the change: 789.4.

## Build explicit block-LU inverse tiles in last fused chunk to speed pending flush

The final fused sweep chunk now optionally builds the off-diagonal blocks of the inverted U and L factors and stores them in an extended LU image. The pending-chunk flush in the Kronecker path then applies the inverse as independent block products instead of sequential forward and back triangular substitution. This shortens the dependent MFMA chain in the flush. The cost is extra MFMA work, a larger image stride and more LDS use in the last fused chunk. A debug accessor for reading the LU image back to the host is also added.

```diff
diff --git a/include/dqmc_hip.h b/include/dqmc_hip.h
--- a/include/dqmc_hip.h
+++ b/include/dqmc_hip.h
@@ -160,6 +160,8 @@
 int dqmc_set_triangular_factors(dqmc_handle *h, const double *f);
 int dqmc_udt_one_launch_sites(dqmc_handle *h, int32_t *mask);
 int dqmc_device_errors(dqmc_handle *h, int32_t *word);
+int64_t dqmc_lu_image_doubles(void);
+int dqmc_lu_image(dqmc_handle *h, int32_t unit, double *out, int64_t n_doubles, int32_t *has_inverse);
 const char *dqmc_build_commit(void);
 const char *dqmc_build_source_hash(void);
 
diff --git a/montecarlo.jl_amd/_lib.py b/montecarlo.jl_amd/_lib.py
--- a/montecarlo.jl_amd/_lib.py
+++ b/montecarlo.jl_amd/_lib.py
@@ -147,6 +147,8 @@
     "dqmc_kron_hopping": (C.c_int, [_H, C.POINTER(C.c_int32)]),
     "dqmc_set_triangular_factors": (C.c_int, [_H, _dp]),
     "dqmc_device_errors": (C.c_int, [_H, C.POINTER(C.c_int32)]),
+    "dqmc_lu_image_doubles": (C.c_int64, []),
+    "dqmc_lu_image": (C.c_int, [_H, C.c_int32, C.POINTER(C.c_double), C.c_int64, C.POINTER(C.c_int32)]),
     "dqmc_udt_one_launch_sites": (C.c_int, [_H, C.POINTER(C.c_int32)]),
     "dqmc_build_commit": (C.c_char_p, []),
     "dqmc_build_source_hash": (C.c_char_p, []),
diff --git a/montecarlo.jl_amd/csrc/engine.cpp b/montecarlo.jl_amd/csrc/engine.cpp
--- a/montecarlo.jl_amd/csrc/engine.cpp
+++ b/montecarlo.jl_amd/csrc/engine.cpp
@@ -52,6 +52,8 @@
     hipStream_t cur = nullptr;
     double *greens_alt = nullptr, *lu_img = nullptr;
     bool sweep_fused = true;
+    const double *last_img = nullptr;
+    bool last_img_inv = false;
     struct PendingFlush {
         const double *G = nullptr;
         const double *img = nullptr;
@@ -974,16 +976,20 @@
         HIPCHK(launch_sweep_lu(h->n, h->nb, h->W, cur, h->nn, cslice, cstr, 0, 64, h->lu_img, h->sc, h->rng, h->stats,
                                h->p.check_sign_problem, h->qr_ws.errflag, h->cur, a, b));
         CHK(timing_push(h, a, b, DQMC_K_SWEEP));
+        const bool fold = fold_wrap_flush(h);
         for (int c = 1; c < nc; ++c) {
             timing_events(h, &a, &b);
             HIPCHK(launch_sweep_fused(h->n, h->nb, h->W, cur, alt, h->nn, cslice, cstr, 64 * c, 64 * (c - 1),
                                       h->lu_img + (size_t)(c & 1) * istr, h->lu_img + (size_t)((c - 1) & 1) * istr, h->sc,
-                                      h->rng, h->stats, h->p.check_sign_problem, h->qr_ws.errflag, h->cur, a, b));
+                                      h->rng, h->stats, h->p.check_sign_problem, h->qr_ws.errflag,
+                                      (fold && c == nc - 1) ? 1 : 0, h->cur, a, b));
             CHK(timing_push(h, a, b, DQMC_K_SWEEP));
             std::swap(cur, alt);
         }
         const double *img_last = h->lu_img + (size_t)((nc - 1) & 1) * istr;
-        if (fold_wrap_flush(h)) {
+        h->last_img = img_last;
+        h->last_img_inv = fold;
+        if (fold) {
             h->pf = dqmc_handle::PendingFlush{cur, img_last, 64 * (nc - 1)};
         } else {
             timing_events(h, &a, &b);
@@ -1938,6 +1944,18 @@
     HIPCHK(hipMemcpy(word, h->qr_ws.errflag, sizeof(int), hipMemcpyDeviceToHost));
     return DQMC_OK;
 }
+int64_t dqmc_lu_image_doubles(void) { return (int64_t)sweep_lu_image_doubles(); }
+int dqmc_lu_image(dqmc_handle *h, int32_t unit, double *out, int64_t n_doubles, int32_t *has_inverse)
+{
+    ENTER(h);
+    const int64_t need = (int64_t)sweep_lu_image_doubles();
+    if (!out || !has_inverse || unit < 0 || unit >= h->units || n_doubles < need) return DQMC_ERR_INVALID;
+    if (!h->last_img) return fail(h, DQMC_ERR_STATE, "dqmc_lu_image: no fused sweep_spatial has run on this handle");
+    HIPCHK(hipStreamSynchronize(h->stream));
+    HIPCHK(hipMemcpy(out, h->last_img + (size_t)unit * need, (size_t)need * sizeof(double), hipMemcpyDeviceToHost));
+    *has_inverse = h->last_img_inv ? 1 : 0;
+    return DQMC_OK;
+}
 int dqmc_udt_one_launch_sites(dqmc_handle *h, int32_t *mask)
 {
     if (!h || !mask) return DQMC_ERR_INVALID;
diff --git a/montecarlo.jl_amd/csrc/kernels.h b/montecarlo.jl_amd/csrc/kernels.h
--- a/montecarlo.jl_amd/csrc/kernels.h
+++ b/montecarlo.jl_amd/csrc/kernels.h
@@ -220,7 +220,9 @@
 constexpr int LU_TILE = 256;
 constexpr int LU_OFF_U = 0, LU_OFF_L = 6 * LU_TILE, LU_OFF_PT = 12 * LU_TILE, LU_OFF_Q = 16 * LU_TILE;
 constexpr int LU_IMG = 20 * LU_TILE;
-constexpr int LU_STRIDE = LU_IMG + 64;
+constexpr int LU_SOLVE = LU_IMG + 64;
+constexpr int LU_OFF_AI = LU_SOLVE, LU_OFF_BI = LU_SOLVE + 6 * LU_TILE;
+constexpr int LU_STRIDE = LU_SOLVE + 12 * LU_TILE;
 __host__ __device__ constexpr int lu_pair(int K, int J)
 {
     return K == 0 ? J - 1 : (K == 1 ? J + 1 : 5);
@@ -232,7 +234,8 @@
 hipError_t launch_sweep_fused(int n, int nb, int n_walkers, const double *Gin, double *Gout, long strideG,
                               int8_t *conf_slice, long conf_stride, int site0, int site0p, double *img,
                               const double *imgp, SweepConsts sc, WalkerRng *rng, DevStats *stats, int check_sign,
-                              int *errflag, hipStream_t s, hipEvent_t start = nullptr, hipEvent_t stop = nullptr);
+                              int *errflag, int build_inv, hipStream_t s, hipEvent_t start = nullptr,
+                              hipEvent_t stop = nullptr);
 
 hipError_t launch_sweep_flush_lu(int n, int n_units, const double *Gin, double *Gout, long strideG, int site0,
                                  int nsites, const double *img, const KernelSwitches &sw, hipStream_t s,
diff --git a/montecarlo.jl_amd/csrc/kron.hip b/montecarlo.jl_amd/csrc/kron.hip
--- a/montecarlo.jl_amd/csrc/kron.hip
+++ b/montecarlo.jl_amd/csrc/kron.hip
@@ -18,7 +18,7 @@
 constexpr int KR_PF_IMG = 0, KR_PF_X = 20 * KR_PF_TS, KR_PF_R0 = KR_PF_X + 64, KR_PF_RLD = 65;
 constexpr int KR_PF_D = KR_LDS_T, KR_PF_DLD = 257;
 constexpr int KR_LDS_PF = KR_PF_D + KR_COLS * KR_PF_DLD;
-static_assert(KR_PF_R0 + KR_COLS * KR_PF_RLD <= KR_LDS_PF && KR_LDS <= KR_LDS_PF, "pending-chunk LDS layout");
+static_assert(KR_PF_R0 + 2 * KR_COLS * KR_PF_RLD <= KR_LDS_PF && KR_LDS <= KR_LDS_PF, "pending-chunk LDS layout");
 
 #define KR_GLOBAL __attribute__((address_space(1)))
 typedef const KR_GLOBAL double *kr_gcdp;
@@ -59,11 +59,13 @@
     const kr_gcdp img = (kr_gcdp)(a.pf_img + (long)unit * a.pf_img_su);
     const kr_gcdp G = (kr_gcdp)(a.X0 + (long)unit * a.x_su);
     double *limg = lds + KR_PF_IMG, *lx = lds + KR_PF_X, *lr = lds + KR_PF_R0, *ld = lds + KR_PF_D;
-    constexpr int NI = LU_IMG / 2 / 256;
-    static_assert(NI * 512 == LU_IMG, "image staging");
+    constexpr int NI = 20 * LU_TILE / 2 / 256, ND = (LU_OFF_AI - LU_OFF_PT) / LU_TILE;
+    static_assert(NI * 512 == 20 * LU_TILE && ND == 8 && LU_OFF_Q == LU_OFF_PT + 4 * LU_TILE && LU_OFF_AI == LU_IMG + 64 &&
+                  LU_OFF_BI == LU_OFF_AI + 6 * LU_TILE && LU_STRIDE == LU_OFF_BI + 6 * LU_TILE, "image staging");
     kr_d2 iv[NI];
 #pragma unroll
-    for (int i = 0; i < NI; ++i) iv[i] = reinterpret_cast<kr_gcd2p>(img)[tid + 256 * i];
+    for (int i = 0; i < NI; ++i)
+        iv[i] = reinterpret_cast<kr_gcd2p>(img + (2 * i < ND ? LU_OFF_PT : LU_OFF_AI - ND * LU_TILE))[tid + 256 * i];
     const double xin = img[LU_IMG + (tid & 63)];
 #pragma unroll
     for (int i = 0; i < NI; ++i) {
@@ -85,7 +87,7 @@
     KR_STAMP(2);
     auto A = [&](int tl, int q) { return limg[tl * KR_PF_TS + ci * 17 + 4 * q + g]; };
     auto xr = [&](int J, int r) { return lx[16 * J + 4 * r + g]; };
-    constexpr int TU = LU_OFF_U / LU_TILE, TL = LU_OFF_L / LU_TILE, TP = LU_OFF_PT / LU_TILE, TQ = LU_OFF_Q / LU_TILE;
+    constexpr int TP = 0, TQ = 4, TA = 8, TB = 14;
     const kr_gcdp gc = G + 64 * w + ci + (long)KR_N * (site0 + g);
     double ca[2][4][4];
     auto fetch = [&](int J, double (&c)[4][4]) {
@@ -95,18 +97,18 @@
             for (int mm = 0; mm < 4; ++mm) c[mm][q] = gc[16 * mm + (long)KR_N * (16 * J + 4 * q)];
     };
     fetch(0, ca[0]);
-#ifdef KR_PROBE_PRODUCTS
     d4k rh[4];
     {
         double *lw = lr + KR_COLS * KR_PF_RLD, *lh = lr;
-        static_assert(KR_PF_R0 + 2 * KR_COLS * KR_PF_RLD <= KR_LDS_PF, "probe LDS");
         d4k pa[4];
 #pragma unroll
         for (int J = 0; J < 4; ++J) {
             pa[J] = (d4k){0.0, 0.0, 0.0, 0.0};
-            if (J <= w)
-#pragma unroll
-                for (int q = 0; q < 4; ++q) pa[J] = KR_MFMA(A(TL + J, q), lr[ci * KR_PF_RLD + 16 * J + 4 * q + g], pa[J]);
+            if (J <= w) {
+                const int tl = J == w ? TQ + w : TB + lu_pair(J, w);
+#pragma unroll
+                for (int q = 0; q < 4; ++q) pa[J] = KR_MFMA(A(tl, q), lr[ci * KR_PF_RLD + 16 * J + 4 * q + g], pa[J]);
+            }
         }
 #pragma unroll
         for (int r = 0; r < 4; ++r)
@@ -115,9 +117,11 @@
 #pragma unroll
         for (int J = 0; J < 4; ++J) {
             pa[J] = (d4k){0.0, 0.0, 0.0, 0.0};
-            if (J >= w)
-#pragma unroll
-                for (int q = 0; q < 4; ++q) pa[J] = KR_MFMA(A(TU + J, q), lw[ci * KR_PF_RLD + 16 * J + 4 * q + g], pa[J]);
+            if (J >= w) {
+                const int tl = J == w ? TP + w : TA + lu_pair(w, J);
+#pragma unroll
+                for (int q = 0; q < 4; ++q) pa[J] = KR_MFMA(A(tl, q), lw[ci * KR_PF_RLD + 16 * J + 4 * q + g], pa[J]);
+            }
         }
 #pragma unroll
         for (int r = 0; r < 4; ++r) lh[ci * KR_PF_RLD + 16 * w + 4 * r + g] = pa[0][r] + pa[1][r] + pa[2][r] + pa[3][r];
@@ -127,38 +131,6 @@
 #pragma unroll
             for (int q = 0; q < 4; ++q) rh[J][q] = lh[ci * KR_PF_RLD + 16 * J + 4 * q + g];
     }
-#else
-    d4k xv[4], rh[4];
-#pragma unroll
-    for (int J = 0; J < 4; ++J) {
-        d4k acc;
-#pragma unroll
-        for (int r = 0; r < 4; ++r) acc[r] = lr[ci * KR_PF_RLD + 16 * J + 4 * r + g];
-#pragma unroll
-        for (int K = 0; K < J; ++K)
-#pragma unroll
-            for (int q = 0; q < 4; ++q) acc = KR_MFMA(A(TL + lu_pair(K, J), q), xv[K][q], acc);
-        d4k z = (d4k){0.0, 0.0, 0.0, 0.0};
-#pragma unroll
-        for (int q = 0; q < 4; ++q) z = KR_MFMA(A(TQ + J, q), acc[q], z);
-#pragma unroll
-        for (int r = 0; r < 4; ++r) xv[J][r] = z[r] * xr(J, r);
-    }
-#pragma unroll
-    for (int J = 3; J >= 0; --J) {
-        d4k acc = (d4k){0.0, 0.0, 0.0, 0.0};
-#pragma unroll
-        for (int K = J + 1; K < 4; ++K)
-#pragma unroll
-            for (int q = 0; q < 4; ++q) acc = KR_MFMA(A(TU + lu_pair(J, K), q), rh[K][q], acc);
-#pragma unroll
-        for (int r = 0; r < 4; ++r) acc[r] = xv[J][r] + xr(J, r) * acc[r];
-        d4k o = (d4k){0.0, 0.0, 0.0, 0.0};
-#pragma unroll
-        for (int q = 0; q < 4; ++q) o = KR_MFMA(A(TP + J, q), acc[q], o);
-        rh[J] = o;
-    }
-#endif
     KR_STAMP(3);
     d4k dm[4];
 #pragma unroll
diff --git a/montecarlo.jl_amd/csrc/sweep_lu.hip b/montecarlo.jl_amd/csrc/sweep_lu.hip
--- a/montecarlo.jl_amd/csrc/sweep_lu.hip
+++ b/montecarlo.jl_amd/csrc/sweep_lu.hip
@@ -90,14 +90,115 @@
 #else
 #define FL_STAMP(k) do { } while (0)
 #endif
+constexpr int LX_TS = 16 * 17;
+constexpr int LX_PT = 0, LX_Q = 4, LX_U = 8, LX_L = 14, LX_AI = 20, LX_BI = 24, LX_TILES = 28;
+constexpr int LX_FD = 8, LX_FU2 = 12, LX_FU3 = 14, LX_F1 = 17, LX_NFLAG = 24;
+__host__ __device__ constexpr int lx_lo(int I, int J) { return I == 0 ? J - 1 : 2; }
+__device__ __forceinline__ void lx_put(double *t, const d4 &v, int g, int ci)
+{
+#pragma unroll
+    for (int r = 0; r < 4; ++r) t[(4 * r + g) * 17 + ci] = v[r];
+}
+__device__ __forceinline__ void lx_put_t(double *t, const d4 &v, int g, int ci)
+{
+#pragma unroll
+    for (int r = 0; r < 4; ++r) t[ci * 17 + 4 * r + g] = v[r];
+}
+template <int J>
+__device__ __forceinline__ void lx_sums_a(const double *ex, const double *xs, d4 (&T)[3], int g, int ci)
+{
+#pragma unroll
+    for (int I = 0; I < J; ++I) {
+        T[I] = (d4){0.0, 0.0, 0.0, 0.0};
+#pragma unroll
+        for (int K = I; K < J; ++K) {
+            const double *u = ex + (LX_U + lu_pair(K, J)) * LX_TS;
+            const double *ai = ex + (K == I ? LX_PT + I : LX_AI + lx_lo(I, K)) * LX_TS;
+#pragma unroll
+            for (int q = 0; q < 4; ++q)
+                T[I] = MFMA(xs[16 * K + 4 * q + g] * u[(4 * q + g) * 17 + ci], ai[ci * 17 + 4 * q + g], T[I]);
+        }
+    }
+}
+template <int J>
+__device__ __forceinline__ void lx_last_a(const double *ex, const d4 (&T)[3], d4 (&O)[3], int g, int ci)
+{
+    const double *pt = ex + (LX_PT + J) * LX_TS;
+#pragma unroll
+    for (int I = 0; I < J; ++I) O[I] = (d4){0.0, 0.0, 0.0, 0.0};
+#pragma unroll
+    for (int q = 0; q < 4; ++q) {
+        const double p = pt[(4 * q + g) * 17 + ci];
+#pragma unroll
+        for (int I = 0; I < J; ++I) O[I] = MFMA(T[I][q], p, O[I]);
+    }
+}
+template <int J>
+__device__ __forceinline__ void lx_sums_b(const double *ex, const double *xs, d4 (&V)[3], int g, int ci)
+{
+#pragma unroll
+    for (int I = 0; I < J; ++I) {
+        V[I] = (d4){0.0, 0.0, 0.0, 0.0};
+#pragma unroll
+        for (int K = I; K < J; ++K) {
+            const double *l = ex + (LX_L + lu_pair(K, J)) * LX_TS;
+            const double *bi = ex + (K == I ? LX_Q + I : LX_BI + lx_lo(I, K)) * LX_TS;
+#pragma unroll
+            for (int q = 0; q < 4; ++q)
+                V[I] = MFMA(l[ci * 17 + 4 * q + g] * xs[16 * K + 4 * q + g], bi[(4 * q + g) * 17 + ci], V[I]);
+        }
+    }
+}
+template <int J>
+__device__ __forceinline__ void lx_last_b(const double *ex, const d4 (&V)[3], d4 (&O)[3], int g, int ci)
+{
+    const double *qm = ex + (LX_Q + J) * LX_TS;
+#pragma unroll
+    for (int I = 0; I < J; ++I) O[I] = (d4){0.0, 0.0, 0.0, 0.0};
+#pragma unroll
+    for (int q = 0; q < 4; ++q) {
+        const double a = qm[ci * 17 + 4 * q + g];
+#pragma unroll
+        for (int I = 0; I < J; ++I) O[I] = MFMA(a, V[I][q], O[I]);
+    }
+}
+template <int J, bool UPPER>
+__device__ __forceinline__ void lx_store(double *ex, gdp img, const d4 (&O)[3], int lane, int g, int ci)
+{
+#pragma unroll
+    for (int I = 0; I < J; ++I) {
+#pragma unroll
+        for (int r = 0; r < 4; ++r) img[(UPPER ? LU_OFF_AI : LU_OFF_BI) + lu_pair(I, J) * LU_TILE + r * 64 + lane] = O[I][r];
+        if (J < 3) lx_put(ex + ((UPPER ? LX_AI : LX_BI) + lx_lo(I, J < 3 ? J : 2)) * LX_TS, O[I], g, ci);
+    }
+}
+template <int J, bool UPPER>
+__device__ __forceinline__ void lx_level(double *ex, const double *xs, gdp img, int lane, int g, int ci)
+{
+    d4 T[3], O[3];
+    if (UPPER) {
+        lx_sums_a<J>(ex, xs, T, g, ci);
+        lx_last_a<J>(ex, T, O, g, ci);
+    } else {
+        lx_sums_b<J>(ex, xs, T, g, ci);
+        lx_last_b<J>(ex, T, O, g, ci);
+    }
+    lx_store<J, UPPER>(ex, img, O, lane, g, ci);
+}
+
 template <int NB, bool FULL, bool PRO, int J>
 __device__ __noinline__ void lu4_wave(int n, const double *__restrict__ Gall, long strideG, int w, int site0,
                                       int nsites, double *__restrict__ img_all, const SweepConsts &sc,
                                       unsigned long long cbits_v, double uvec, int check_sign, int site0p,
-                                      const double *__restrict__ imgp_all)
+                                      const double *__restrict__ imgp_all, int inv_v)
 {
     Lu4Smem<NB> &sm = *reinterpret_cast<Lu4Smem<NB> *>(lu4_lds);
     const int lane = threadIdx.x & 63, g = lane >> 4, ci = lane & 15;
+    constexpr bool INVW = PRO && FULL && NB == 1;
+    static_assert(!INVW || LX_TILES * LX_TS <= LU_SOLVE + 1536 + 1024, "exchange tiles on the prologue's scratch");
+    const bool inv = INVW && __builtin_amdgcn_readfirstlane(inv_v) != 0;
+    double *const lx = lu4_lds + (sizeof(Lu4Smem<NB>) + 15) / 16 * 2;
+    int *const lxf = reinterpret_cast<int *>(lx + LU_SOLVE + 1536 + 1024);
     const unsigned long long cbits =
         ((unsigned long long)(unsigned)__builtin_amdgcn_readfirstlane((int)(cbits_v >> 32)) << 32) |
         (unsigned)__builtin_amdgcn_readfirstlane((int)(cbits_v & 0xffffffffull));
@@ -124,8 +225,8 @@
     }
     if (PRO) {
         LU4_STAMP(400 + 8 * J + 0);
-        constexpr bool EARLY = (NB == 1) && (sizeof(Lu4Smem<NB>) + LU_STRIDE * sizeof(double) <= 150 * 1024);
-        double *xtra = lu4_lds + (sizeof(Lu4Smem<NB>) + 15) / 16 * 2 + LU_STRIDE;
+        constexpr bool EARLY = (NB == 1) && (sizeof(Lu4Smem<NB>) + LU_SOLVE * sizeof(double) <= 150 * 1024);
+        double *xtra = lu4_lds + (sizeof(Lu4Smem<NB>) + 15) / 16 * 2 + LU_SOLVE;
         double *Rl = EARLY ? reinterpret_cast<double *>(&sm.aST[0][31][0]) : reinterpret_cast<double *>(&sm.aST[0][0][0]);
         double *ttx = EARLY ? xtra : Rl + 64 * 66;
         double *tt0 = xtra + 1536;
@@ -148,19 +249,19 @@
 #pragma unroll
                 for (int i = 0; i < 8; ++i) r0v[i] = q[i];
             }
-            constexpr bool STAGE = sizeof(Lu4Smem<NB>) + LU_STRIDE * sizeof(double) <= 150 * 1024;
+            constexpr bool STAGE = sizeof(Lu4Smem<NB>) + LU_SOLVE * sizeof(double) <= 150 * 1024;
             double *imgl = lu4_lds + (sizeof(Lu4Smem<NB>) + 15) / 16 * 2;
             double opU[STAGE ? 1 : 6][4], opL[STAGE ? 1 : 6][4], opP[STAGE ? 1 : 4][4], opQ[STAGE ? 1 : 4][4], xr[4][4];
             if (STAGE) {
-                constexpr int NI = (LU_STRIDE / 2 + 255) / 256;
+                constexpr int NI = (LU_SOLVE / 2 + 255) / 256;
                 const gcd2p src = reinterpret_cast<gcd2p>(imgp);
                 d2v *dst = reinterpret_cast<d2v *>(imgl);
                 d2v iv[NI];
 #pragma unroll
-                for (int i = 0; i < NI; ++i) iv[i] = src[min(tid + 256 * i, LU_STRIDE / 2 - 1)];
+                for (int i = 0; i < NI; ++i) iv[i] = src[min(tid + 256 * i, LU_SOLVE / 2 - 1)];
 #pragma unroll
                 for (int i = 0; i < NI; ++i)
-                    if (tid + 256 * i < LU_STRIDE / 2) dst[tid + 256 * i] = iv[i];
+                    if (tid + 256 * i < LU_SOLVE / 2) dst[tid + 256 * i] = iv[i];
             } else {
 #pragma unroll
                 for (int pr = 0; pr < (STAGE ? 0 : 6); ++pr)
@@ -337,7 +438,38 @@
     for (int I0 = 0; I0 < 4; ++I0) {
         if (!FULL && 16 * I0 >= nsites) break;
         const bool PIV = (I0 == J), HLP = (J > I0), PTQ = (J == (I0 == 0 ? 3 : (I0 == 3 ? 1 : 0)));
-        if (!PIV && !HLP && !PTQ) continue;
+        if (!PIV && !HLP && !PTQ) {
+            if constexpr (INVW) {
+                if (inv) {
+                    const gdp img = (gdp)(img_all + (long)w * LU_STRIDE);
+                    if (I0 == 2 && J == 1) {
+                        if (lu4_wait(&lxf[LX_FD + 0], &sm.abort) > 0 && lu4_wait(&lxf[LX_FD + 1], &sm.abort) > 0) {
+                            lx_level<1, true>(lx, sm.xs[0], img, lane, g, ci);
+                            lx_level<1, false>(lx, sm.xs[0], img, lane, g, ci);
+                        }
+                        LU4_ORDER();
+                        __hip_atomic_store(&lxf[LX_F1], 1, __ATOMIC_RELAXED, __HIP_MEMORY_SCOPE_WORKGROUP);
+                    }
+                    if (I0 == 3 && (J == 0 || J == 2)) {
+                        constexpr bool UP = J == 0;
+                        if (lu4_wait(&lxf[LX_F1], &sm.abort) > 0 && lu4_wait(&lxf[LX_FU2 + 1], &sm.abort) > 0 &&
+                            lu4_wait(&lxf[LX_FD + 2], &sm.abort) > 0 && lu4_wait(&lxf[LX_FU3 + 2], &sm.abort) > 0) {
+                            lx_level<2, UP>(lx, sm.xs[0], img, lane, g, ci);
+                            d4 T[3], O[3];
+                            if (UP) lx_sums_a<3>(lx, sm.xs[0], T, g, ci);
+                            else lx_sums_b<3>(lx, sm.xs[0], T, g, ci);
+                            LU4_STAMP(320 + 8 * J + 5);
+                            if (lu4_wait(&lxf[LX_FD + 3], &sm.abort) > 0) {
+                                if (UP) lx_last_a<3>(lx, T, O, g, ci);
+                                else lx_last_b<3>(lx, T, O, g, ci);
+                                lx_store<3, UP>(lx, img, O, lane, g, ci);
+                            }
+                        }
+                    }
+                }
+            }
+            continue;
+        }
         d4 PT[NB], Q[NB];
         if (PTQ) {
 #pragma unroll
@@ -355,8 +487,8 @@
         for (int b = 0; b < NB; ++b) { pf_pay[b] = make_double2(0.0, 0.0); pf_xh[b] = 0.0; }
         double dcur[NB];
         if (PIV) {
-            if (PRO && NB == 1 && I0 >= 1 && sizeof(Lu4Smem<NB>) + LU_STRIDE * sizeof(double) <= 150 * 1024) {
-                int *pflag = reinterpret_cast<int *>(lu4_lds + (sizeof(Lu4Smem<NB>) + 15) / 16 * 2 + LU_STRIDE + 1536 + 1024);
+            if (PRO && NB == 1 && I0 >= 1 && sizeof(Lu4Smem<NB>) + LU_SOLVE * sizeof(double) <= 150 * 1024) {
+                int *pflag = reinterpret_cast<int *>(lu4_lds + (sizeof(Lu4Smem<NB>) + 15) / 16 * 2 + LU_SOLVE + 1536 + 1024);
                 (void)lu4_wait(&pflag[5], &sm.abort);
                 (void)lu4_wait(&pflag[6], &sm.abort);
                 (void)lu4_wait(&pflag[7], &sm.abort);
@@ -536,6 +668,26 @@
             }
             if (PIV && (lane >> 4) == I0) img[LU_IMG + lane] = sm.xs[b][lane];
         }
+        if constexpr (INVW) {
+            if (inv && (HLP || PTQ)) {
+                if (I0 == 0) {
+                    (void)lu4_wait(&lxf[5], &sm.abort);
+                    (void)lu4_wait(&lxf[6], &sm.abort);
+                    (void)lu4_wait(&lxf[7], &sm.abort);
+                }
+                if (HLP) {
+                    lx_put(lx + (LX_U + lu_pair(I0, J)) * LX_TS, S[0][I0], g, ci);
+                    lx_put_t(lx + (LX_L + lu_pair(I0, J)) * LX_TS, ST[0][I0], g, ci);
+                }
+                if (PTQ) {
+                    lx_put_t(lx + (LX_PT + I0) * LX_TS, PT[0], g, ci);
+                    lx_put(lx + (LX_Q + I0) * LX_TS, Q[0], g, ci);
+                }
+                LU4_ORDER();
+                if (HLP && J >= 2) __hip_atomic_store(&lxf[(J == 2 ? LX_FU2 : LX_FU3) + I0], 1, __ATOMIC_RELAXED, __HIP_MEMORY_SCOPE_WORKGROUP);
+                if (PTQ) __hip_atomic_store(&lxf[LX_FD + I0], 1, __ATOMIC_RELAXED, __HIP_MEMORY_SCOPE_WORKGROUP);
+            }
+        }
         if (PIV) {
             if (lane == 0) {
                 sm.acc16[I0] = accb;
@@ -554,7 +706,7 @@
                                           int8_t *__restrict__ conf_slice, long conf_stride, int site0, int nsites,
                                           double *__restrict__ img_all, const SweepConsts &sc, WalkerRng *rngs,
                                           DevStats *stats, int check_sign, int *errflag, int site0p,
-                                          const double *__restrict__ imgp_all)
+                                          const double *__restrict__ imgp_all, int inv = 0)
 {
     Lu4Smem<NB> &sm = *reinterpret_cast<Lu4Smem<NB> *>(lu4_lds);
     const int tid = threadIdx.x, lane = tid & 63, wave = tid >> 6;
@@ -577,15 +729,49 @@
 #endif
     if (tid < 4) { sm.acc16[tid] = 0u; sm.neg16[tid] = 0u; sm.ndraw[tid] = 0; sm.exh[tid] = 0; }
     if (tid == 0) sm.abort = 0;
-    if (PRO && NB == 1 && tid < 8)
-        reinterpret_cast<int *>(lu4_lds + (sizeof(Lu4Smem<NB>) + 15) / 16 * 2 + LU_STRIDE + 1536 + 1024)[tid] = 0;
+    if (PRO && NB == 1 && tid < LX_NFLAG)
+        reinterpret_cast<int *>(lu4_lds + (sizeof(Lu4Smem<NB>) + 15) / 16 * 2 + LU_SOLVE + 1536 + 1024)[tid] = 0;
     __syncthreads();
     const int wv = __builtin_amdgcn_readfirstlane(wave);
-    if (wv == 0) lu4_wave<NB, FULL, PRO, 0>(n, Gall, strideG, w, site0, nsites, img_all, sc, cbits, uvec, check_sign, site0p, imgp_all);
-    else if (wv == 1) lu4_wave<NB, FULL, PRO, 1>(n, Gall, strideG, w, site0, nsites, img_all, sc, cbits, uvec, check_sign, site0p, imgp_all);
-    else if (wv == 2) lu4_wave<NB, FULL, PRO, 2>(n, Gall, strideG, w, site0, nsites, img_all, sc, cbits, uvec, check_sign, site0p, imgp_all);
-    else lu4_wave<NB, FULL, PRO, 3>(n, Gall, strideG, w, site0, nsites, img_all, sc, cbits, uvec, check_sign, site0p, imgp_all);
+    if (wv == 0) lu4_wave<NB, FULL, PRO, 0>(n, Gall, strideG, w, site0, nsites, img_all, sc, cbits, uvec, check_sign, site0p, imgp_all, inv);
+    else if (wv == 1) lu4_wave<NB, FULL, PRO, 1>(n, Gall, strideG, w, site0, nsites, img_all, sc, cbits, uvec, check_sign, site0p, imgp_all, inv);
+    else if (wv == 2) lu4_wave<NB, FULL, PRO, 2>(n, Gall, strideG, w, site0, nsites, img_all, sc, cbits, uvec, check_sign, site0p, imgp_all, inv);
+    else lu4_wave<NB, FULL, PRO, 3>(n, Gall, strideG, w, site0, nsites, img_all, sc, cbits, uvec, check_sign, site0p, imgp_all, inv);
     __syncthreads();
+    if constexpr (PRO && FULL && NB == 2) {
+        if (__builtin_amdgcn_readfirstlane(inv) != 0) {
+            static_assert(NB * LX_TILES * LX_TS * sizeof(double) <= sizeof(sm.aST), "exchange tiles on the step ring");
+            constexpr int NI = LU_IMG / 2 / 256;
+            d2v iv[NB][NI];
+#pragma unroll
+            for (int b = 0; b < NB; ++b)
+#pragma unroll
+                for (int i = 0; i < NI; ++i)
+                    iv[b][i] = reinterpret_cast<gcd2p>((gcdp)(img_all + (long)(w * NB + b) * LU_STRIDE))[tid + 256 * i];
+#pragma unroll
+            for (int b = 0; b < NB; ++b)
+#pragma unroll
+                for (int i = 0; i < NI; ++i) {
+                    const int p = 2 * (tid + 256 * i), tl = p >> 8, r = (p >> 6) & 3, ln = p & 63;
+                    double *d = lu4_lds + (b * LX_TILES + (tl < 12 ? tl + LX_U : tl - 12)) * LX_TS + (4 * r + (ln >> 4)) * 17 + (ln & 15);
+                    d[0] = iv[b][i].x;
+                    d[1] = iv[b][i].y;
+                }
+            __syncthreads();
+            const int wu = __builtin_amdgcn_readfirstlane(wave), b = wu >> 1, g = lane >> 4, ci = lane & 15;
+            double *ex = lu4_lds + b * LX_TILES * LX_TS;
+            const gdp img = (gdp)(img_all + (long)(w * NB + b) * LU_STRIDE);
+            if ((wu & 1) == 0) {
+                lx_level<1, true>(ex, sm.xs[b], img, lane, g, ci);
+                lx_level<2, true>(ex, sm.xs[b], img, lane, g, ci);
+                lx_level<3, true>(ex, sm.xs[b], img, lane, g, ci);
+            } else {
+                lx_level<1, false>(ex, sm.xs[b], img, lane, g, ci);
+                lx_level<2, false>(ex, sm.xs[b], img, lane, g, ci);
+                lx_level<3, false>(ex, sm.xs[b], img, lane, g, ci);
+            }
+        }
+    }
     const int nblk = (nsites + 15) / 16;
     if (!FULL) {
         const int I0 = wv, g = lane >> 4, ci = lane & 15;
@@ -672,7 +858,7 @@
     double *fsm = lu4_lds;
     double *img = fsm;
     double *xs = fsm + LU_IMG;
-    double *Rl = fsm + LU_STRIDE;
+    double *Rl = fsm + LU_SOLVE;
     const int xcd = bid & 7, seq = bid >> 3;
     const int T = tiles_m * tiles_n;
     const int unit = (seq / T) * 8 + xcd;
@@ -709,7 +895,7 @@
     {
         const gcd2p src = reinterpret_cast<gcd2p>((gcdp)(img_all + (long)unit * LU_STRIDE));
         d2v *dst = reinterpret_cast<d2v *>(img);
-        for (int i = tid; i < LU_STRIDE / 2; i += 256) dst[i] = src[i];
+        for (int i = tid; i < LU_SOLVE / 2; i += 256) dst[i] = src[i];
     }
 #pragma unroll
     for (int pass = 0; pass < NT / 4; ++pass) {
@@ -894,13 +1080,14 @@
     int check_sign;
     int *errflag;
     int tiles_m, tiles_n;
+    int build_inv;
 };
 template <int NB, int NT, int NCP>
 __global__ __launch_bounds__(256) void sweep_fused_kernel(SweepFusedArgs a)
 {
     if ((int)blockIdx.x < a.n_walkers)
         lu4_block<NB, true, true>(blockIdx.x, a.n, a.Gin, a.strideG, a.conf_slice, a.conf_stride, a.site0, 64, a.img, a.sc,
-                                  a.rngs, a.stats, a.check_sign, a.errflag, a.site0p, a.imgp);
+                                  a.rngs, a.stats, a.check_sign, a.errflag, a.site0p, a.imgp, a.build_inv);
     else
         flush_lu_body<true, NT, NCP>((int)blockIdx.x - a.n_walkers, a.n, a.n_units, a.Gin, a.Gout, a.strideG, a.site0p, 64,
                                      a.imgp, a.tiles_m, a.tiles_n);
@@ -915,13 +1102,13 @@
     const int nt = wide ? 8 : 4;
     const int tm = (n + 63) / 64, tn = (n + 16 * nt - 1) / (16 * nt);
     const int groups = (n_units + 7) / 8;
-    const size_t lds = ((size_t)LU_STRIDE + 16 * nt * FL_LDR) * sizeof(double);
+    const size_t lds = ((size_t)LU_SOLVE + 16 * nt * FL_LDR) * sizeof(double);
     const bool full = (n % 64 == 0) && nsites == 64;
     int dev = 0;
     (void)hipGetDevice(&dev);
     static unsigned attr_mask = 0;
     if (!(attr_mask & (1u << dev))) {
-        const int big = (int)(((size_t)LU_STRIDE + 128 * FL_LDR) * sizeof(double));
+        const int big = (int)(((size_t)LU_SOLVE + 128 * FL_LDR) * sizeof(double));
         (void)hipFuncSetAttribute((const void *)sweep_flush_lu_kernel<true, 8>, hipFuncAttributeMaxDynamicSharedMemorySize, big);
         (void)hipFuncSetAttribute((const void *)sweep_flush_lu_kernel<false, 8>, hipFuncAttributeMaxDynamicSharedMemorySize, big);
         (void)hipFuncSetAttribute((const void *)sweep_flush_lu_kernel<true, 4>, hipFuncAttributeMaxDynamicSharedMemorySize, big);
@@ -939,11 +1126,11 @@
     const bool ncp2 = sw.flush_ncp2 || (dev >= 0 && dev < 32 && groups * 8 * tm * tn > n_cus[dev]);
     if (ncp2 && full && (n + 63) / 64 > 1) {
         const int tn4 = (n + 63) / 64;
-        const size_t lds4 = ((size_t)LU_STRIDE + 64 * FL_LDR) * sizeof(double);
+        const size_t lds4 = ((size_t)LU_SOLVE + 64 * FL_LDR) * sizeof(double);
         static unsigned m0 = 0;
         if (!(m0 & (1u << dev))) {
             (void)hipFuncSetAttribute((const void *)sweep_flush_lu_kernel<true, 4, 0>, hipFuncAttributeMaxDynamicSharedMemorySize,
-                                      (int)(((size_t)LU_STRIDE + 128 * FL_LDR) * sizeof(double)));
+                                      (int)(((size_t)LU_SOLVE + 128 * FL_LDR) * sizeof(double)));
             m0 |= 1u << dev;
         }
         hipExtLaunchKernelGGL((sweep_flush_lu_kernel<true, 4, 0>), dim3(groups * 8 * tm), dim3(256), lds4, s, start, stop, 0, n,
@@ -959,7 +1146,7 @@
 hipError_t launch_sweep_fused(int n, int nb, int n_walkers, const double *Gin, double *Gout, long strideG,
                               int8_t *conf_slice, long conf_stride, int site0, int site0p, double *img,
                               const double *imgp, SweepConsts sc, WalkerRng *rng, DevStats *stats, int check_sign,
-                              int *errflag, hipStream_t s, hipEvent_t start, hipEvent_t stop)
+                              int *errflag, int build_inv, hipStream_t s, hipEvent_t start, hipEvent_t stop)
 {
     if (n % 64 != 0 || site0 % 64 != 0 || site0p % 64 != 0 || site0 + 64 > n || site0p + 64 > n || nb < 1 || nb > 2)
         return hipErrorInvalidValue;
@@ -969,14 +1156,14 @@
     SweepFusedArgs a;
     a.n = n; a.n_walkers = n_walkers; a.n_units = n_units; a.Gin = Gin; a.Gout = Gout; a.strideG = strideG;
     a.conf_slice = conf_slice; a.conf_stride = conf_stride; a.site0 = site0; a.site0p = site0p; a.img = img; a.imgp = imgp;
-    a.sc = sc; a.rngs = rng; a.stats = stats; a.check_sign = check_sign; a.errflag = errflag;
+    a.sc = sc; a.rngs = rng; a.stats = stats; a.check_sign = check_sign; a.errflag = errflag; a.build_inv = build_inv;
     const int ncp = (wide && n % 256 == 0) ? 2 : 1;
     a.tiles_m = n / 64; a.tiles_n = n / (16 * nt * ncp);
     const int groups = (n_units + 7) / 8;
     const int flush_blocks = groups * 8 * a.tiles_m * a.tiles_n;
-    const size_t lds_flush = ((size_t)LU_STRIDE + 16 * nt * FL_LDR) * sizeof(double);
+    const size_t lds_flush = ((size_t)LU_SOLVE + 16 * nt * FL_LDR) * sizeof(double);
     const size_t lds_lu = nb == 1 ? sizeof(Lu4Smem<1>) : sizeof(Lu4Smem<2>);
-    const size_t lds_pro = nb == 1 ? (sizeof(Lu4Smem<1>) + 15) / 16 * 16 + (LU_STRIDE + 1536 + 1024 + 8) * sizeof(double) : lds_lu;
+    const size_t lds_pro = nb == 1 ? (sizeof(Lu4Smem<1>) + 15) / 16 * 16 + (LU_SOLVE + 1536 + 1024 + LX_NFLAG / 2) * sizeof(double) : lds_lu;
     const size_t lds_e = lds_pro > lds_lu ? lds_pro : lds_lu;
     const size_t lds = lds_flush > lds_e ? lds_flush : lds_e;
     int dev = 0;
diff --git a/montecarlo.jl_amd/dqmc.py b/montecarlo.jl_amd/dqmc.py
--- a/montecarlo.jl_amd/dqmc.py
+++ b/montecarlo.jl_amd/dqmc.py
@@ -769,6 +769,12 @@
         self._c(lib().dqmc_device_errors(self._h, C.byref(w)))
         return int(w.value)
 
+    def lu_image(self, unit):
+        out = np.zeros(int(lib().dqmc_lu_image_doubles()))
+        f = C.c_int32(0)
+        self._c(lib().dqmc_lu_image(self._h, int(unit), dptr(out), out.size, C.byref(f)))
+        return out, bool(f.value)
+
     def timing_enable(self, on=True):
         self._c(lib().dqmc_timing_enable(self._h, int(on)))
 
```

Result: no change. 788.4 (-0.1%).
